# tmdt-buw/VQ-VAE-Transformer-Arc-Welding

Measured on AMD Instinct MI355X. Metric: welding windows/sec (train) VQ-VAE+8-blk Transformer at 1/2/4/8 MI355X, higher is better.
Workload: dtype bf16; 1 GPU; VQ-VAE-Patch reconstruction train step (configs[1]); global_batch=1024, per_gpu_batch=1024, seq_len=200, codebook=512x64, hidden=512, n_resblocks=8, patch=25, parallelism=dp1, optimizer=RAdam(lr 1e-3), operands=bf16 (opt-in), fp32 accumulation and master weights

## Files before the change

### include/arcweld_amd.h

```cpp
#ifndef ARCWELD_AMD_H
#define ARCWELD_AMD_H

#include <stdint.h>

#ifdef __cplusplus
extern "C" {
#endif

enum { AW_OK = 0, AW_ERR_ARG = -1, AW_ERR_LAUNCH = -2 };
enum { AW_F32 = 0, AW_BF16 = 1 };
enum { AW_ACT_GELU_ERF = 0, AW_ACT_GELU_TANH = 1, AW_ACT_DERIV = 2 };

const char* aw_last_error(void);
int aw_version(void);

typedef struct {
  int M, N, K;
  int a_dtype;
  const void* A; int64_t lda; int a_trans;
  const void* B; int64_t ldb; int b_trans;
  int conv_cin, conv_seg, conv_dir, conv_operand;
  float alpha, beta;
  const float* bias;
  int act;
  const float* pre; int64_t ld_pre;
  const float* resid; int64_t ld_resid;
  float drop_p; uint64_t drop_seed;
  void* C; int64_t ldc; int c_dtype;
  void* C2; int64_t ldc2; int c2_mode; int c2_dtype;
  float drop2_p; uint64_t drop2_seed;
  double* colstats; int stats_mod;
  float* a_rowsum;
  int bias_mod;
  int accumulate, col_mod, col_mul, col_off;
  const uint64_t* seed_ptr;
  int pre_dtype;
  int store_policy;
  int resid_dtype;
} aw_gemm_args;
#define AW_STORE_NT 0
#define AW_STORE_WT 1

int aw_gemm(const aw_gemm_args* args, void* stream);
int64_t aw_gemm_workspace(const aw_gemm_args* args);
int aw_gemm_ws(const aw_gemm_args* args, float* ws, int64_t ws_elems, void* stream);
#define AW_GEMM_MAX_GROUPS 16
int aw_gemm_grouped(const aw_gemm_args* args, int n, void* stream);
int aw_gemm_set_tile(int bm);
int aw_gemm_describe(const aw_gemm_args* args, int* layout, uint32_t* epi, int* tile_rows, int* specialised,
                     int* ragged, int* splits);
int aw_gemm_set_wgrad_policy(int mode);
#define AW_WGRAD_BATCH_MAX 32
int64_t aw_wgrad_batch_workspace(const aw_gemm_args* args, int n);
int aw_wgrad_batch(const aw_gemm_args* args, int n, void* ws, int64_t ws_bytes, void* stream);
int aw_wgrad_set_spin_limit(int polls);

#define AW_RES_CHAIN_MAX 16
typedef struct {
  int64_t N;
  int H, R;
  int taps, seg;
  const void* a0;
  const void* x0;
  const void* w1[AW_RES_CHAIN_MAX];
  const void* w2[AW_RES_CHAIN_MAX];
  const float* b1[AW_RES_CHAIN_MAX];
  const float* b2[AW_RES_CHAIN_MAX];
  void* dgelu_h[AW_RES_CHAIN_MAX];
  void* a1[AW_RES_CHAIN_MAX];
  void* dgelu_x[AW_RES_CHAIN_MAX];
  void* a[AW_RES_CHAIN_MAX];
  float drop_p;
  uint64_t drop_seed[AW_RES_CHAIN_MAX];
  const uint64_t* seed_ptr;
  int store_policy;
  uint64_t* drop_masks;
} aw_res_chain_fwd_args;
typedef struct {
  int64_t N;
  int H, R;
  int taps, seg;
  const void* gx;
  const void* gxo;
  const void* x0;
  const void* w1t[AW_RES_CHAIN_MAX];
  const void* w2t[AW_RES_CHAIN_MAX];
  const void* dgelu_h[AW_RES_CHAIN_MAX];
  const void* dgelu_x[AW_RES_CHAIN_MAX];
  void* gh[AW_RES_CHAIN_MAX];
  void* gxo_out[AW_RES_CHAIN_MAX];
  float drop_p;
  int store_policy;
  const uint64_t* drop_masks;
} aw_res_chain_bwd_args;
int aw_res_chain_fwd(const aw_res_chain_fwd_args* args, void* stream);
int aw_res_chain_bwd(const aw_res_chain_bwd_args* args, void* stream);
int64_t aw_res_dropout_masks_bytes(int64_t N, int R);
int aw_res_dropout_masks(int64_t N, int R, float drop_p, const uint64_t* drop_seed, const uint64_t* seed_ptr,
                         void* masks, void* stream);
#define AW_RES_PACK_MAX 32
int aw_res_pack_weights(const void* const* src, void* const* fwd, void* const* bwd, int n, int taps, void* stream);

int aw_vq_forward(const float* z, const float* E, int64_t N, int K, int D,
                  float* zq, int64_t* idx, float* counts, double* sqerr, void* stream);
int aw_vq_forward_ex(const float* z, const float* E, int64_t N, int K, int D, float* zq, int64_t* idx, float* counts,
                     double* sqerr, void* zq_copy, int copy_dtype, void* stream);
#define AW_VQ_COUNT_GROUPS_MAX 64
int aw_vq_forward_ex2(const float* z, const float* E, int64_t N, int K, int D, float* zq, int64_t* idx, float* counts,
                      int count_groups, double* sqerr, void* zq_copy, int copy_dtype, void* stream);
int aw_vq_finalize(const float* counts, const double* sqerr, int64_t N, int K, int D, float beta,
                   float* loss, float* perplexity, void* stream);
int aw_vq_finalize_ex(const float* counts, int count_groups, const double* sqerr, int64_t N, int K, int D, float beta,
                      float* loss, float* perplexity, void* stream);
int aw_vq_backward(const float* z, const float* E, const int64_t* idx, const float* g_zq, const float* g_loss,
                   int64_t N, int K, int D, float beta, float* dz, float* dE, void* stream);
int aw_vq_backward_ex(const float* z, const float* E, const int64_t* idx, const float* g_zq, const float* g_loss,
                      int64_t N, int K, int D, float beta, float* dz, float* dE, void* dz_copy, int copy_dtype,
                      void* stream);
int aw_vq_cluster_sums(const float* z, const int64_t* idx, int64_t N, int K, int D, float* sums, void* stream);
int aw_kmeans_update(float* means, const float* sums, const float* counts, int K, int D, float* avg, void* stream);
int aw_rvq_ema_update(float* embed, float* embed_avg, float* cluster_size, const float* counts, const float* sums,
                      const float* z, int64_t N, int K, int D, float decay, float eps, float threshold, uint64_t salt,
                      const uint64_t* seed_ptr, float* ws, void* stream);
int aw_rvq_residual(const float* r, const float* zq, int64_t n, float* out, int first, float* r_next, void* stream);
int aw_rvq_backward(const float* res, const float* q, const float* g_zq, const float* g_loss, int nq, int64_t N,
                    int D, float commitment, float* dz, void* stream);

int aw_vq_onehot(const int64_t* idx, int64_t N, int K, float* onehot, void* stream);
int aw_vq_gather(const float* E, const int64_t* idx, int64_t N, int D, float* out, void* stream);

int aw_patchify(const float* x, int64_t B, int L, int C, int P, void* patches, int64_t ldp, int dtype,
                void* stream);
int aw_weight_relayout(const float* W, int O, int I, int k, int tap, int mode, void* out, int64_t ldo,
                       int dtype, void* stream);
#define AW_RELAYOUT_MAX_JOBS 40
typedef struct {
  const float* W;
  void* out;
  int O, I, k, tap, mode;
  int64_t ldo;
} aw_relayout_job;
int aw_weight_relayout_batch(const aw_relayout_job* jobs, int n, int dtype, void* stream);
int aw_weight_grad_scatter(const float* g, int O, int I, int k, int tap, int mode, int64_t ldg, float* G,
                           void* stream);
int aw_cast(const float* in, int64_t n, void* out, int dtype, void* stream);

int aw_unpatch_head_fwd(const float* y, int64_t R, int H, int Q, const float* stats, const float* w2,
                        const float* b2, float* x_hat, void* stream);
int aw_bn_finalize(const double* colstats, int64_t n, int H, const float* gamma, const float* beta,
                   float* running_mean, float* running_var, int64_t* nbt, float eps, float momentum,
                   int training, float* stats, void* stream);
int aw_unpatch_head_bwd1(const float* y, int64_t R, int H, int Q, const float* stats, const float* w2,
                         const float* g_xhat, double* gsums, float* gw2, float* gb2, float* ggamma, float* gbeta,
                         void* stream);
int aw_unpatch_head_bwd2(const float* y, int64_t R, int H, int Q, const float* stats, const float* w2,
                         const float* g_xhat, const double* gsums, int training, void* g_y, int gy_dtype, float* db_y,
                         void* stream);
int aw_unpatch_head_fwd_ex(const void* y, int y_dtype, int64_t R, int H, int Q, const float* stats, const float* w2,
                           const float* b2, float* x_hat, void* stream);
int aw_unpatch_head_bwd1_ex(const void* y, int y_dtype, int64_t R, int H, int Q, const float* stats, const float* w2,
                            const float* g_xhat, double* gsums, float* gw2, float* gb2, float* ggamma, float* gbeta,
                            void* stream);
int aw_unpatch_head_bwd2_ex(const void* y, int y_dtype, int64_t R, int H, int Q, const float* stats, const float* w2,
                            const float* g_xhat, const double* gsums, int training, void* g_y, int gy_dtype,
                            float* db_y, void* stream);
int aw_unpatch_head_fwd_bwd1(const void* y, int y_dtype, int64_t R, int H, int Q, const float* stats, const float* w2,
                             const float* b2, const float* x, const float* gscale, float* x_hat, float* g_xhat,
                             double* sqerr, double* gsums, float* gw2, float* gb2, float* ggamma, float* gbeta,
                             void* stream);
int aw_bn_group_stats(const float* h, int64_t N, int H, int G, double* sums, void* stream);
int aw_bn_group_finalize(const double* sums, int64_t n, int H, int G, const float* gamma, const float* beta,
                         float* running_mean, float* running_var, int64_t* nbt, float eps, float momentum,
                         int training, float* stats, void* stream);
int aw_bn_apply(const float* h, int64_t N, int H, int G, const float* stats, int mode, const float* resid,
                float drop_p, uint64_t drop_seed, const uint64_t* seed_ptr, float* out, void* op, int op_dtype,
                void* stream);
int aw_bn_bwd_reduce(const float* h, int64_t N, int H, int G, const float* stats, const float* g_in, float drop_p,
                     uint64_t drop_seed, const uint64_t* seed_ptr, double* sums, void* stream);
int aw_bn_bwd_apply(const float* h, int64_t N, int H, int G, const float* stats, const float* g_in, float drop_p,
                    uint64_t drop_seed, const uint64_t* seed_ptr, const double* sums, int64_t n, int training,
                    void* dh, int dh_dtype, float* dgamma, float* dbeta, void* stream);
int aw_mse_fwd(const float* a, const float* b, int64_t n, double* sqerr, void* stream);
int aw_mse_bwd(const float* a, const float* b, int64_t n, const float* g, float* ga, void* stream);

int aw_scalar_add(const float* a, const float* b, float* out, void* stream);
int aw_mse_finalize(const double* sqerr, int64_t numel, float* out, void* stream);
int aw_mse_finalize_add(const double* sqerr, int64_t numel, const float* addend, float* out, float* sum, void* stream);

int aw_radam_step(float* param, float* grad, float* exp_avg, float* exp_avg_sq, const int64_t* seg_off,
                  const int64_t* seg_len, const float* seg_wd, const int* seg_active, int nseg, int64_t total, int64_t step,
                  float lr, float beta1, float beta2, float eps, const float* gscale, const int64_t* step_ptr,
                  int zero_grad, void* stream);
#define AW_OPS_PER_SEG 2
typedef struct {
  void* out;
  int O, I, k, tap, mode, dtype;
  int64_t ldo;
} aw_operand_desc;
int aw_radam_step_ops(float* param, float* grad, float* exp_avg, float* exp_avg_sq, const int64_t* seg_off,
                      const int64_t* seg_len, const float* seg_wd, const int* seg_active, int nseg, int64_t total,
                      int64_t step, float lr, float beta1, float beta2, float eps, const float* gscale,
                      const int64_t* step_ptr, const aw_operand_desc* ops, int zero_grad, void* stream);
int aw_counter_add(int64_t* counter, int64_t v, void* stream);
int aw_counter_add_snapshot(int64_t* counter, int64_t v, int64_t* snapshot, void* stream);
int aw_counter_add_snapshot_zero(int64_t* counter, int64_t v, int64_t* snapshot, double* zero, int64_t nzero,
                                 void* stream);
#define AW_NORM_WS 1024
int aw_grad_norm_clip(const float* grad, const int64_t* seg_off, const int64_t* seg_len, const int* seg_active,
                      int nseg, int64_t total, float max_norm, double* ws, float* out_norm, float* out_coef,
                      void* stream);
int aw_scale(float* x, int64_t n, const float* s, void* stream);

int aw_layernorm_fwd(const float* x, int64_t R, int D, const float* w, const float* b, float eps, void* y,
                     int y_dtype, float* mean, float* rstd, void* stream);
int aw_layernorm_bwd(const float* x, const float* dy, int64_t R, int D, const float* w, const float* mean,
                     const float* rstd, float* dx, int accumulate, float* dw, float* db, void* dx2, int dx2_dtype,
                     float drop_p, uint64_t drop_seed, const uint64_t* seed_ptr, void* stream);
int aw_class_head_fwd(const float* xf, int64_t B, int T, int D, const float* w1, const float* b1, const float* W2,
                      const float* b2, float* s, float* out, void* stream);
int aw_class_head_bwd(const float* xf, const float* s, const float* dout, int64_t B, int T, int D, const float* w1,
                      const float* W2, float* dxf, float* dw1, float* db1, float* dW2, float* db2, void* stream);
int aw_embed_fwd(const int64_t* ids, int64_t B, int T, int D, const float* wtok, const float* pe, float* x,
                 void* stream);
int aw_embed_ln_fwd(const int64_t* ids, int64_t B, int T, int D, const float* wtok, const float* pe, float* x,
                    const float* w, const float* b, float eps, void* y, int y_dtype, float* mean, float* rstd,
                    void* stream);
int aw_embed_bwd(const int64_t* ids, int64_t B, int T, int D, const float* dx, float* dwtok, void* stream);
int aw_embed_bwd_sorted(const int64_t* ids, int64_t B, int T, int D, int V, const float* dx, float* dwtok, int* work,
                        void* stream);
int aw_embed_sort(const int64_t* ids, int64_t R, int V, int* work, void* stream);
int aw_embed_bwd_segsum(const int* work, int V, int D, const float* dx, float* dwtok, void* stream);
int aw_attn_fwd(const void* qkv, int64_t B, int T, int n_head, int d, int dtype, void* y, float* lse,
                void* stream);
int aw_attn_bwd(const void* qkv, const void* y, const void* dy, const float* lse, int64_t B, int T, int n_head,
                int d, int dtype, void* dqkv, float* ws, void* stream);
int aw_attn_fwd_dropout(const void* qkv, int64_t B, int T, int n_head, int d, int dtype, void* y, float* lse,
                        float drop_p, uint64_t drop_seed, const uint64_t* seed_ptr, void* stream);
int aw_attn_bwd_dropout(const void* qkv, const void* y, const void* dy, const float* lse, int64_t B, int T,
                        int n_head, int d, int dtype, void* dqkv, float* ws, float drop_p, uint64_t drop_seed,
                        const uint64_t* seed_ptr, void* stream);
int aw_attn_decode(const void* qkv_new, int64_t B, int n_new, int pos0, int n_head, int d, int dtype,
                   void* kv_cache, int Tmax, void* y, void* stream);
int aw_ce_fwd(const float* logits, int64_t R, int V, int64_t ldl, const int64_t* y, int ignore_index,
              double* loss_sum, double* count, float* lse, void* stream);
int aw_ce_bwd(const float* logits, int64_t R, int V, int64_t ldl, const int64_t* y, int ignore_index,
              const float* lse, const double* count, const float* g, void* dlogits, int64_t ldd, int dtype,
              void* stream);
int aw_ce_finalize(const double* loss_sum, const double* count, float* out, void* stream);

int aw_gru_pack_weights(const float* w_hh, int H, int op_dtype, void* w_fwd, void* w_bwd, void* stream);
int aw_gru_step_fwd(int B, int H, int op_dtype, const void* h_prev_op, const float* h_prev, const void* w_fwd,
                    const float* gi, const float* b_hh, float* h, void* h_op, float* saved, void* stream);
int aw_gru_step_bwd(int B, int H, int op_dtype, const void* dgh_next_op, const float* dh_next,
                    const float* saved_next, const void* w_bwd, const float* dy, const float* saved,
                    const float* h_prev, float* dh, float* dgi, float* dgh, void* dgi_op, void* dgh_op, void* stream);
int aw_gru_bias_grad(const float* dg, int64_t rows, int H, float* db, void* stream);

#ifdef __cplusplus
}
#endif
#endif
```

### vq-vae-transformer-arc-welding_amd/arcweld/_native.py

```python
from __future__ import annotations

import ctypes
import os

import torch

PKG_DIR = os.path.dirname(os.path.dirname(os.path.abspath(__file__)))
LIB_PATH = os.environ.get("ARCWELD_LIB") or os.path.join(PKG_DIR, "lib", "libarcweld_amd.so")
HEADER = os.path.join(os.path.dirname(PKG_DIR), "include", "arcweld_amd.h")

AW_F32, AW_BF16 = 0, 1
AW_ACT_GELU_ERF, AW_ACT_GELU_TANH, AW_ACT_DERIV = 0, 1, 2
AW_STORE_NT, AW_STORE_WT = 0, 1

c_i64 = ctypes.c_int64
c_int = ctypes.c_int
c_f = ctypes.c_float
c_p = ctypes.c_void_p


class GemmArgs(ctypes.Structure):
    _fields_ = [
        ("M", c_int), ("N", c_int), ("K", c_int),
        ("a_dtype", c_int),
        ("A", c_p), ("lda", c_i64), ("a_trans", c_int),
        ("B", c_p), ("ldb", c_i64), ("b_trans", c_int),
        ("conv_cin", c_int), ("conv_seg", c_int), ("conv_dir", c_int), ("conv_operand", c_int),
        ("alpha", c_f), ("beta", c_f),
        ("bias", c_p),
        ("act", c_int),
        ("pre", c_p), ("ld_pre", c_i64),
        ("resid", c_p), ("ld_resid", c_i64),
        ("drop_p", c_f), ("drop_seed", ctypes.c_uint64),
        ("C", c_p), ("ldc", c_i64), ("c_dtype", c_int),
        ("C2", c_p), ("ldc2", c_i64), ("c2_mode", c_int), ("c2_dtype", c_int),
        ("drop2_p", c_f), ("drop2_seed", ctypes.c_uint64),
        ("colstats", c_p), ("stats_mod", c_int),
        ("a_rowsum", c_p),
        ("bias_mod", c_int),
        ("accumulate", c_int), ("col_mod", c_int), ("col_mul", c_int), ("col_off", c_int),
        ("seed_ptr", c_p),
        ("pre_dtype", c_int),
        ("store_policy", c_int),
        ("resid_dtype", c_int),
    ]


class RelayoutJob(ctypes.Structure):
    _fields_ = [("W", c_p), ("out", c_p), ("O", c_int), ("I", c_int), ("k", c_int), ("tap", c_int),
                ("mode", c_int), ("ldo", c_i64)]


class OperandDesc(ctypes.Structure):
    _fields_ = [("out", c_p), ("O", c_int), ("I", c_int), ("k", c_int), ("tap", c_int), ("mode", c_int),
                ("dtype", c_int), ("ldo", c_i64)]


OPS_PER_SEG = 2

RES_CHAIN_MAX = 16
RES_PACK_MAX = 32
_E = RES_CHAIN_MAX


class ResChainFwdArgs(ctypes.Structure):
    _fields_ = [("N", c_i64), ("H", c_int), ("R", c_int), ("taps", c_int), ("seg", c_int), ("a0", c_p), ("x0", c_p),
                ("w1", c_p * _E), ("w2", c_p * _E), ("b1", c_p * _E), ("b2", c_p * _E),
                ("dgelu_h", c_p * _E), ("a1", c_p * _E), ("dgelu_x", c_p * _E), ("a", c_p * _E),
                ("drop_p", c_f), ("drop_seed", ctypes.c_uint64 * _E), ("seed_ptr", c_p), ("store_policy", c_int),
                ("drop_masks", c_p)]


class ResChainBwdArgs(ctypes.Structure):
    _fields_ = [("N", c_i64), ("H", c_int), ("R", c_int), ("taps", c_int), ("seg", c_int), ("gx", c_p), ("gxo", c_p),
                ("x0", c_p), ("w1t", c_p * _E), ("w2t", c_p * _E), ("dgelu_h", c_p * _E), ("dgelu_x", c_p * _E),
                ("gh", c_p * _E), ("gxo_out", c_p * _E),
                ("drop_p", c_f), ("store_policy", c_int), ("drop_masks", c_p)]

SIGNATURES = {
    "aw_version": [],
    "aw_gemm": [ctypes.POINTER(GemmArgs), c_p],
    "aw_gemm_ws": [ctypes.POINTER(GemmArgs), c_p, c_i64, c_p],
    "aw_gemm_workspace": [ctypes.POINTER(GemmArgs)],
    "aw_gemm_grouped": [ctypes.POINTER(GemmArgs), c_int, c_p],
    "aw_gemm_set_tile": [c_int],
    "aw_gemm_describe": [ctypes.POINTER(GemmArgs), ctypes.POINTER(c_int), ctypes.POINTER(ctypes.c_uint32),
                         ctypes.POINTER(c_int), ctypes.POINTER(c_int), ctypes.POINTER(c_int), ctypes.POINTER(c_int)],
    "aw_gemm_set_wgrad_policy": [c_int],
    "aw_wgrad_batch_workspace": [ctypes.POINTER(GemmArgs), c_int],
    "aw_wgrad_batch": [ctypes.POINTER(GemmArgs), c_int, c_p, c_i64, c_p],
    "aw_wgrad_set_spin_limit": [c_int],
    "aw_res_chain_fwd": [ctypes.POINTER(ResChainFwdArgs), c_p],
    "aw_res_chain_bwd": [ctypes.POINTER(ResChainBwdArgs), c_p],
    "aw_res_pack_weights": [ctypes.POINTER(c_p), ctypes.POINTER(c_p), ctypes.POINTER(c_p), c_int, c_int, c_p],
    "aw_res_dropout_masks_bytes": [c_i64, c_int],
    "aw_res_dropout_masks": [c_i64, c_int, c_f, ctypes.POINTER(ctypes.c_uint64), c_p, c_p, c_p],
    "aw_weight_relayout_batch": [ctypes.POINTER(RelayoutJob), c_int, c_int, c_p],
    "aw_vq_forward": [c_p, c_p, c_i64, c_int, c_int, c_p, c_p, c_p, c_p, c_p],
    "aw_vq_forward_ex": [c_p, c_p, c_i64, c_int, c_int, c_p, c_p, c_p, c_p, c_p, c_int, c_p],
    "aw_vq_finalize": [c_p, c_p, c_i64, c_int, c_int, c_f, c_p, c_p, c_p],
    "aw_vq_forward_ex2": [c_p, c_p, c_i64, c_int, c_int, c_p, c_p, c_p, c_int, c_p, c_p, c_int, c_p],
    "aw_vq_finalize_ex": [c_p, c_int, c_p, c_i64, c_int, c_int, c_f, c_p, c_p, c_p],
    "aw_vq_backward": [c_p, c_p, c_p, c_p, c_p, c_i64, c_int, c_int, c_f, c_p, c_p, c_p],
    "aw_vq_backward_ex": [c_p, c_p, c_p, c_p, c_p, c_i64, c_int, c_int, c_f, c_p, c_p, c_p, c_int, c_p],
    "aw_vq_onehot": [c_p, c_i64, c_int, c_p, c_p],
    "aw_vq_gather": [c_p, c_p, c_i64, c_int, c_p, c_p],
    "aw_patchify": [c_p, c_i64, c_int, c_int, c_int, c_p, c_i64, c_int, c_p],
    "aw_weight_relayout": [c_p, c_int, c_int, c_int, c_int, c_int, c_p, c_i64, c_int, c_p],
    "aw_weight_grad_scatter": [c_p, c_int, c_int, c_int, c_int, c_int, c_i64, c_p, c_p],
    "aw_cast": [c_p, c_i64, c_p, c_int, c_p],
    "aw_unpatch_head_fwd": [c_p, c_i64, c_int, c_int, c_p, c_p, c_p, c_p, c_p],
    "aw_bn_finalize": [c_p, c_i64, c_int, c_p, c_p, c_p, c_p, c_p, c_f, c_f, c_int, c_p, c_p],
    "aw_unpatch_head_bwd1": [c_p, c_i64, c_int, c_int, c_p, c_p, c_p, c_p, c_p, c_p, c_p, c_p, c_p],
    "aw_unpatch_head_bwd2": [c_p, c_i64, c_int, c_int, c_p, c_p, c_p, c_p, c_int, c_p, c_int, c_p, c_p],
    "aw_unpatch_head_fwd_ex": [c_p, c_int, c_i64, c_int, c_int, c_p, c_p, c_p, c_p, c_p],
    "aw_unpatch_head_bwd1_ex": [c_p, c_int, c_i64, c_int, c_int, c_p, c_p, c_p, c_p, c_p, c_p, c_p, c_p, c_p],
    "aw_unpatch_head_fwd_bwd1": [c_p, c_int, c_i64, c_int, c_int, c_p, c_p, c_p, c_p, c_p, c_p, c_p, c_p, c_p, c_p,
                                 c_p, c_p, c_p, c_p],
    "aw_unpatch_head_bwd2_ex": [c_p, c_int, c_i64, c_int, c_int, c_p, c_p, c_p, c_p, c_int, c_p, c_int, c_p, c_p],
    "aw_bn_group_stats": [c_p, c_i64, c_int, c_int, c_p, c_p],
    "aw_bn_group_finalize": [c_p, c_i64, c_int, c_int, c_p, c_p, c_p, c_p, c_p, c_f, c_f, c_int, c_p, c_p],
    "aw_bn_apply": [c_p, c_i64, c_int, c_int, c_p, c_int, c_p, c_f, ctypes.c_uint64, c_p, c_p, c_p, c_int, c_p],
    "aw_bn_bwd_reduce": [c_p, c_i64, c_int, c_int, c_p, c_p, c_f, ctypes.c_uint64, c_p, c_p, c_p],
    "aw_bn_bwd_apply": [c_p, c_i64, c_int, c_int, c_p, c_p, c_f, ctypes.c_uint64, c_p, c_p, c_i64, c_int, c_p, c_int,
                        c_p, c_p, c_p],
    "aw_mse_fwd": [c_p, c_p, c_i64, c_p, c_p],
    "aw_mse_bwd": [c_p, c_p, c_i64, c_p, c_p, c_p],
    "aw_scalar_add": [c_p, c_p, c_p, c_p],
    "aw_mse_finalize": [c_p, c_i64, c_p, c_p],
    "aw_mse_finalize_add": [c_p, c_i64, c_p, c_p, c_p, c_p],
    "aw_radam_step": [c_p, c_p, c_p, c_p, c_p, c_p, c_p, c_p, c_int, c_i64, c_i64, c_f, c_f, c_f, c_f, c_p, c_p,
                      c_int, c_p],
    "aw_radam_step_ops": [c_p, c_p, c_p, c_p, c_p, c_p, c_p, c_p, c_int, c_i64, c_i64, c_f, c_f, c_f, c_f, c_p, c_p,
                          c_p, c_int, c_p],
    "aw_counter_add": [c_p, c_i64, c_p],
    "aw_counter_add_snapshot": [c_p, c_i64, c_p, c_p],
    "aw_counter_add_snapshot_zero": [c_p, c_i64, c_p, c_p, c_i64, c_p],
    "aw_grad_norm_clip": [c_p, c_p, c_p, c_p, c_int, c_i64, c_f, c_p, c_p, c_p, c_p],
    "aw_scale": [c_p, c_i64, c_p, c_p],
    "aw_layernorm_fwd": [c_p, c_i64, c_int, c_p, c_p, c_f, c_p, c_int, c_p, c_p, c_p],
    "aw_layernorm_bwd": [c_p, c_p, c_i64, c_int, c_p, c_p, c_p, c_p, c_int, c_p, c_p, c_p, c_int, c_f,
                         ctypes.c_uint64, c_p, c_p],
    "aw_class_head_fwd": [c_p, c_i64, c_int, c_int, c_p, c_p, c_p, c_p, c_p, c_p, c_p],
    "aw_class_head_bwd": [c_p, c_p, c_p, c_i64, c_int, c_int, c_p, c_p, c_p, c_p, c_p, c_p, c_p, c_p],
    "aw_embed_fwd": [c_p, c_i64, c_int, c_int, c_p, c_p, c_p, c_p],
    "aw_embed_ln_fwd": [c_p, c_i64, c_int, c_int, c_p, c_p, c_p, c_p, c_p, c_f, c_p, c_int, c_p, c_p, c_p],
    "aw_embed_bwd": [c_p, c_i64, c_int, c_int, c_p, c_p, c_p],
    "aw_embed_bwd_sorted": [c_p, c_i64, c_int, c_int, c_int, c_p, c_p, c_p, c_p],
    "aw_embed_sort": [c_p, c_i64, c_int, c_p, c_p],
    "aw_embed_bwd_segsum": [c_p, c_int, c_int, c_p, c_p, c_p],
    "aw_attn_fwd": [c_p, c_i64, c_int, c_int, c_int, c_int, c_p, c_p, c_p],
    "aw_attn_bwd": [c_p, c_p, c_p, c_p, c_i64, c_int, c_int, c_int, c_int, c_p, c_p, c_p],
    "aw_attn_fwd_dropout": [c_p, c_i64, c_int, c_int, c_int, c_int, c_p, c_p, c_f, ctypes.c_uint64, c_p, c_p],
    "aw_attn_bwd_dropout": [c_p, c_p, c_p, c_p, c_i64, c_int, c_int, c_int, c_int, c_p, c_p, c_f, ctypes.c_uint64,
                            c_p, c_p],
    "aw_attn_decode": [c_p, c_i64, c_int, c_int, c_int, c_int, c_int, c_p, c_int, c_p, c_p],
    "aw_ce_fwd": [c_p, c_i64, c_int, c_i64, c_p, c_int, c_p, c_p, c_p, c_p],
    "aw_ce_bwd": [c_p, c_i64, c_int, c_i64, c_p, c_int, c_p, c_p, c_p, c_p, c_i64, c_int, c_p],
    "aw_ce_finalize": [c_p, c_p, c_p, c_p],
    "aw_vq_cluster_sums": [c_p, c_p, c_i64, c_int, c_int, c_p, c_p],
    "aw_kmeans_update": [c_p, c_p, c_p, c_int, c_int, c_p, c_p],
    "aw_rvq_ema_update": [c_p, c_p, c_p, c_p, c_p, c_p, c_i64, c_int, c_int, c_f, c_f, c_f, ctypes.c_uint64, c_p, c_p,
                          c_p],
    "aw_rvq_residual": [c_p, c_p, c_i64, c_p, c_int, c_p, c_p],
    "aw_rvq_backward": [c_p, c_p, c_p, c_p, c_int, c_i64, c_int, c_f, c_p, c_p],
    "aw_gru_pack_weights": [c_p, c_int, c_int, c_p, c_p, c_p],
    "aw_gru_step_fwd": [c_int, c_int, c_int, c_p, c_p, c_p, c_p, c_p, c_p, c_p, c_p, c_p],
    "aw_gru_bias_grad": [c_p, c_i64, c_int, c_p, c_p],
    "aw_gru_step_bwd": [c_int, c_int, c_int, c_p, c_p, c_p, c_p, c_p, c_p, c_p, c_p, c_p, c_p, c_p, c_p, c_p],
}

RET_I64 = {"aw_gemm_workspace", "aw_wgrad_batch_workspace", "aw_res_dropout_masks_bytes"}

_lib = None


class NativeError(RuntimeError):
    pass


def load(path: str = LIB_PATH):
    global _lib
    if _lib is not None:
        return _lib
    if not os.path.exists(path):
        raise NativeError(f"HIP library not built: {path} is missing (run `python -c 'import __graft_entry__ as g; "
                          f"g.build()'` or `make -C vq-vae-transformer-arc-welding_amd/csrc`)")
    lib = ctypes.CDLL(path, mode=ctypes.RTLD_GLOBAL)
    lib.aw_last_error.restype = ctypes.c_char_p
    lib.aw_last_error.argtypes = []
    for name, argtypes in SIGNATURES.items():
        fn = getattr(lib, name)
        fn.restype = c_i64 if name in RET_I64 else c_int
        fn.argtypes = argtypes
    _lib = lib
    return lib


def call(name: str, *args) -> None:
    lib = load()
    status = getattr(lib, name)(*args)
    if status != 0:
        raise NativeError(f"{name} failed ({status}): {lib.aw_last_error().decode(errors='replace')}")


def stream_ptr(stream=None) -> int:
    s = stream if stream is not None else torch.cuda.current_stream()
    return s.cuda_stream


def ptr(t):
    if t is None:
        return None
    if not t.is_cuda:
        raise NativeError("arcweld HIP kernels need device tensors (got a CPU tensor); there is no CPU fallback")
    return t.data_ptr()


def dtype_code(dt: torch.dtype) -> int:
    if dt == torch.float32:
        return AW_F32
    if dt == torch.bfloat16:
        return AW_BF16
    raise NativeError(f"unsupported operand dtype {dt}")
```

### vq-vae-transformer-arc-welding_amd/arcweld/kernels.py

```python
from __future__ import annotations

import contextvars
import ctypes

import torch

from . import _native as nat
from ._native import AW_ACT_DERIV, AW_ACT_GELU_ERF, AW_ACT_GELU_TANH, AW_BF16, AW_F32, GemmArgs, call, dtype_code, ptr, stream_ptr

__all__ = ["gemm", "AW_ACT_DERIV", "AW_ACT_GELU_ERF", "AW_ACT_GELU_TANH", "AW_BF16", "AW_F32"]


def _ld(t):
    if t is None:
        return 0
    if t.dim() == 1:
        return t.shape[0]
    if t.stride(-1) != 1:
        raise nat.NativeError("operand rows must be contiguous (stride(-1) == 1)")
    return t.stride(0)


_STORE_POLICY = contextvars.ContextVar("arcweld_store_policy", default=0)


class store_policy:

    def __init__(self, policy):
        self.policy = int(policy)

    def __enter__(self):
        self._tok = _STORE_POLICY.set(self.policy)

    def __exit__(self, *exc):
        _STORE_POLICY.reset(self._tok)
        return False

    def __call__(self, fn):
        import functools

        @functools.wraps(fn)
        def wrapped(*a, **k):
            with store_policy(self.policy):
                return fn(*a, **k)
        return wrapped


PROFILE = None


def _algorithmic_flops(M, N, Kd, conv, flops):
    if flops is not None:
        return float(flops)
    if conv is not None:
        seg = conv[1]
        return 2.0 * M * N * (Kd / 3.0) * (3.0 - 2.0 / seg)
    return 2.0 * M * N * Kd


def _gemm_args(A, B, M, N, K, *, a_trans=False, b_trans=False, conv=None, alpha=1.0, beta=0.0, bias=None,
               act=AW_ACT_GELU_ERF, pre=None, resid=None, drop=(0.0, 0), C=None, C2=None, c2_mode=0, drop2=(0.0, 0),
               colstats=None, stats_mod=0, a_rowsum=None, bias_mod=0, accumulate=False, col_map=(0, 1, 0),
               seed_ptr=None):
    if A.dtype != B.dtype:
        raise nat.NativeError(f"gemm operands must share a dtype ({A.dtype} vs {B.dtype})")
    a = GemmArgs()
    a.M, a.N, a.K = int(M), int(N), int(K)
    a.a_dtype = dtype_code(A.dtype)
    a.A, a.lda, a.a_trans = ptr(A), _ld(A), int(bool(a_trans))
    a.B, a.ldb, a.b_trans = ptr(B), _ld(B), int(bool(b_trans))
    if conv is not None:
        a.conv_cin, a.conv_seg, a.conv_dir, a.conv_operand = (int(v) for v in conv)
    a.alpha, a.beta = float(alpha), float(beta)
    a.bias = ptr(bias)
    a.act = int(act)
    a.store_policy = _STORE_POLICY.get()
    a.pre, a.ld_pre = ptr(pre), _ld(pre)
    if pre is not None:
        if pre.dtype not in (torch.float32, torch.bfloat16):
            raise nat.NativeError("pre must be float32 or bfloat16")
        a.pre_dtype = dtype_code(pre.dtype)
    a.resid, a.ld_resid = ptr(resid), _ld(resid)
    if resid is not None:
        if resid.dtype not in (torch.float32, torch.bfloat16):
            raise nat.NativeError("resid must be float32 or bfloat16")
        a.resid_dtype = dtype_code(resid.dtype)
    a.drop_p, a.drop_seed = float(drop[0]), int(drop[1]) & 0xFFFFFFFFFFFFFFFF
    if C is not None:
        a.C, a.ldc, a.c_dtype = ptr(C), _ld(C), dtype_code(C.dtype)
    if C2 is not None:
        a.C2, a.ldc2, a.c2_dtype = ptr(C2), _ld(C2), dtype_code(C2.dtype)
    a.c2_mode = int(c2_mode)
    a.drop2_p, a.drop2_seed = float(drop2[0]), int(drop2[1]) & 0xFFFFFFFFFFFFFFFF
    if colstats is not None:
        if colstats.dtype != torch.float64:
            raise nat.NativeError("colstats must be float64")
        a.colstats, a.stats_mod = ptr(colstats), int(stats_mod)
    a.a_rowsum = ptr(a_rowsum)
    a.bias_mod = int(bias_mod)
    a.accumulate = int(bool(accumulate))
    a.col_mod, a.col_mul, a.col_off = (int(v) for v in col_map)
    a.seed_ptr = ptr(seed_ptr)
    return a


def _timed(s, fn, flops, tag, name=None, nbytes=None):
    e0, e1 = torch.cuda.Event(enable_timing=True), torch.cuda.Event(enable_timing=True)
    e0.record(s)
    fn(s.cuda_stream)
    e1.record(s)
    PROFILE.append((e0, e1, flops, tag, name or tag, nbytes))


def _gemm_tag(A):
    return "gemm_bf16" if A.dtype == torch.bfloat16 else "gemm_f32"


def gemm(A, B, M, N, K, *, stream=None, flops=None, **kw):
    a = _gemm_args(A, B, M, N, K, **kw)
    lib = nat.load()
    wsn = lib.aw_gemm_workspace(ctypes.byref(a))
    ws = torch.empty(wsn, device=A.device, dtype=torch.float32) if wsn > 0 else None
    if PROFILE is None:
        call("aw_gemm_ws", ctypes.byref(a), ptr(ws), wsn, stream_ptr(stream))
        return kw.get("C")
    s = stream if stream is not None else torch.cuda.current_stream()
    _timed(s, lambda sp: call("aw_gemm_ws", ctypes.byref(a), ptr(ws), wsn, sp),
           _algorithmic_flops(M, N, K, kw.get("conv"), flops), _gemm_tag(A), "gemm_kernel")
    return kw.get("C")


MAX_GROUPS = 16


def gemm_grouped(problems, stream=None):
    for c0 in range(0, len(problems), MAX_GROUPS):
        chunk = problems[c0:c0 + MAX_GROUPS]
        arr = (GemmArgs * len(chunk))(*[_gemm_args(A, B, M, N, K, **kw) for (A, B, M, N, K, kw) in chunk])
        if PROFILE is None:
            call("aw_gemm_grouped", arr, len(chunk), stream_ptr(stream))
            continue
        s = stream if stream is not None else torch.cuda.current_stream()
        fl = sum(_algorithmic_flops(M, N, K, kw.get("conv"), None) for (_, _, M, N, K, kw) in chunk)
        c0_ = chunk[0]
        nm = "wgrad_conv3_kernel" if (c0_[5].get("conv") is not None and c0_[0].dtype == torch.bfloat16) \
            else "gemm_kernel (grouped)"
        _timed(s, lambda sp: call("aw_gemm_grouped", arr, len(chunk), sp), fl, _gemm_tag(chunk[0][0]), nm)


WGRAD_BATCH_MAX = 32


def wgrad_batch_ok(problems):
    import os
    mode = os.environ.get("ARCWELD_WGRAD_BATCH", "auto")
    if mode == "0" or not problems or len(problems) > WGRAD_BATCH_MAX:
        return False
    arr = (GemmArgs * len(problems))(*[_gemm_args(A, B, M, N, K, **kw) for (A, B, M, N, K, kw) in problems])
    if nat.load().aw_wgrad_batch_workspace(arr, len(problems)) <= 0:
        return False
    tiles = sum((M // 256) * (N // 256) for (_, _, M, N, _, _) in problems)
    return mode == "1" or tiles >= 128


def wgrad_batch(problems, stream=None):
    arr = (GemmArgs * len(problems))(*[_gemm_args(A, B, M, N, K, **kw) for (A, B, M, N, K, kw) in problems])
    lib = nat.load()
    wsb = lib.aw_wgrad_batch_workspace(arr, len(problems))
    if wsb < 0:
        raise nat.NativeError(f"aw_wgrad_batch: batch not eligible ({lib.aw_last_error().decode(errors='replace')})")
    ws = torch.empty((wsb + 3) // 4, device=problems[0][0].device, dtype=torch.float32)
    if PROFILE is None:
        call("aw_wgrad_batch", arr, len(problems), ptr(ws), wsb, stream_ptr(stream))
        return
    s = stream if stream is not None else torch.cuda.current_stream()
    fl = sum(_algorithmic_flops(M, N, K, None, None) for (_, _, M, N, K, _) in problems)
    _timed(s, lambda sp: call("aw_wgrad_batch", arr, len(problems), ptr(ws), wsb, sp), fl, _gemm_tag(problems[0][0]),
           "wgrad_tt_kernel")


def wgrad_issue(problems, stream=None):
    if not problems:
        return
    nch = (len(problems) + WGRAD_BATCH_MAX - 1) // WGRAD_BATCH_MAX
    per = (len(problems) + nch - 1) // nch
    chunks = [problems[i:i + per] for i in range(0, len(problems), per)]
    if all(wgrad_batch_ok(c) for c in chunks):
        for c in chunks:
            wgrad_batch(c, stream)
        return
    by_shape = {}
    for pb in problems:
        by_shape.setdefault((pb[2], pb[3]), []).append(pb)
    for grp in by_shape.values():
        gemm_grouped(grp, stream)


RES_CHAIN_MAX = nat.RES_CHAIN_MAX


def res_chain_ok(H, R, T, RT, taps=1, seg=16, which="ENC"):
    import os
    if os.environ.get(f"ARCWELD_{which}_CHAIN", "1") == "0":
        return False
    return (H == 512 and 1 <= R <= RES_CHAIN_MAX and T == torch.bfloat16 and RT == torch.bfloat16
            and (taps == 1 or (taps == 3 and seg == 16)))


def _chain_store_policy():
    import os
    return nat.AW_STORE_WT if os.environ.get("ARCWELD_CHAIN_STORE", "nt") == "wt" else nat.AW_STORE_NT


def _chk_rows(ts, N, H, who):
    for t in ts:
        if t is None:
            continue
        if t.dtype != torch.bfloat16 or t.dim() != 2 or tuple(t.shape) != (N, H) or not t.is_contiguous():
            raise nat.NativeError(f"{who}: activations must be contiguous ({N}, {H}) bfloat16 tensors")


def res_dropout_masks_empty(N, R, device):
    nb = nat.load().aw_res_dropout_masks_bytes(int(N), int(R))
    if nb <= 0:
        raise nat.NativeError("res_dropout_masks: bad N / R")
    return torch.empty(nb, device=device, dtype=torch.uint8)


def res_dropout_masks(N, drop, seed_ptr=None, stream=None):
    p, seeds = float(drop[0]), list(drop[1] or [])
    if p <= 0.0:
        return None
    R = len(seeds)
    out = res_dropout_masks_empty(N, R, torch.cuda.current_device() if seed_ptr is None else seed_ptr.device)
    sd = (ctypes.c_uint64 * R)(*[int(v) & 0xFFFFFFFFFFFFFFFF for v in seeds])
    call("aw_res_dropout_masks", int(N), R, p, sd, ptr(seed_ptr), ptr(out), stream_ptr(stream))
    return out


def _nbytes(ts):
    seen, n = set(), 0
    for t in ts:
        if t is not None and t.data_ptr() not in seen:
            seen.add(t.data_ptr())
            n += t.numel() * t.element_size()
    return n


def _chain_flops(R, N, H, taps, seg):
    if taps == 1:
        return 4.0 * R * N * H * H
    return 4.0 * R * N * H * H * (3 - 2.0 / seg)


def res_chain_fwd(a0, x0, w1, w2, b1, b2, dh, a1, dx, a, drop=(0.0, None), seed_ptr=None, masks=None, taps=1, seg=16,
                  stream=None):
    N, H = a0.shape
    R = len(w1)
    if not (1 <= R <= RES_CHAIN_MAX) or not all(len(v) == R for v in (w2, b1, b2, dh, a1, dx, a)):
        raise nat.NativeError("res_chain_fwd: need R (1..16) entries in every per-block list")
    _chk_rows([a0, x0] + list(dh) + list(a1) + list(dx) + list(a), N, H, "res_chain_fwd")
    g = nat.ResChainFwdArgs()
    g.N, g.H, g.R, g.taps, g.seg = N, H, R, int(taps), int(seg)
    g.a0, g.x0 = ptr(a0), ptr(x0)
    for r in range(R):
        g.w1[r], g.w2[r], g.b1[r], g.b2[r] = ptr(w1[r]), ptr(w2[r]), ptr(b1[r]), ptr(b2[r])
        g.dgelu_h[r], g.a1[r], g.dgelu_x[r], g.a[r] = ptr(dh[r]), ptr(a1[r]), ptr(dx[r]), ptr(a[r])
        g.drop_seed[r] = int(drop[1][r]) & 0xFFFFFFFFFFFFFFFF if drop[0] > 0 else 0
    g.drop_p = float(drop[0])
    g.seed_ptr = ptr(seed_ptr)
    g.store_policy = _chain_store_policy()
    g.drop_masks = ptr(masks)
    _maybe_timed(stream, "gemm_bf16", _chain_flops(R, N, H, taps, seg),
                 lambda sp: call("aw_res_chain_fwd", ctypes.byref(g), sp),
                 lambda: (f"res_chain_fwd_kernel<{int(taps)}>",
                          _nbytes([a0, x0, masks] + list(w1) + list(w2) + list(b1) + list(b2) + list(dh) + list(a1) +
                                  list(dx)[:-1] + list(a))))


def res_chain_bwd(gx, gxo, w1t, w2t, dh, x0, dx, gh, gxo_out, drop_p=0.0, masks=None, taps=1, seg=16, stream=None):
    N, H = gx.shape
    R = len(w1t)
    if not (1 <= R <= RES_CHAIN_MAX) or not all(len(v) == R for v in (w2t, dh, dx, gh, gxo_out)):
        raise nat.NativeError("res_chain_bwd: need R (1..16) entries in every per-block list")
    _chk_rows([gx, gxo, x0] + list(dh) + list(dx[1:]) + list(gh) + list(gxo_out), N, H, "res_chain_bwd")
    g = nat.ResChainBwdArgs()
    g.N, g.H, g.R, g.taps, g.seg = N, H, R, int(taps), int(seg)
    g.gx, g.gxo, g.x0 = ptr(gx), ptr(gxo), ptr(x0)
    for r in range(R):
        g.w1t[r], g.w2t[r], g.dgelu_h[r] = ptr(w1t[r]), ptr(w2t[r]), ptr(dh[r])
        g.dgelu_x[r] = ptr(dx[r]) if r > 0 else None
        g.gh[r], g.gxo_out[r] = ptr(gh[r]), ptr(gxo_out[r])
    g.drop_p = float(drop_p)
    g.store_policy = _chain_store_policy()
    g.drop_masks = ptr(masks)
    _maybe_timed(stream, "gemm_bf16", _chain_flops(R, N, H, taps, seg),
                 lambda sp: call("aw_res_chain_bwd", ctypes.byref(g), sp),
                 lambda: (f"res_chain_bwd_kernel<{int(taps)}>",
                          _nbytes([gx, gxo, x0, masks] + list(w1t) + list(w2t) + list(dh) + list(dx[1:]) + list(gh) +
                                  list(gxo_out))))


def res_pack_weights(src, fwd=None, bwd=None, taps=1, stream=None):
    n = len(src)
    fwd = fwd if fwd is not None else [None] * n
    bwd = bwd if bwd is not None else [None] * n
    if len(fwd) != n or len(bwd) != n:
        raise nat.NativeError("res_pack_weights: list lengths differ")
    for t in list(src) + [t for t in fwd + bwd if t is not None]:
        if t.dtype != torch.bfloat16 or t.numel() != 512 * 512 * taps or not t.is_contiguous():
            raise nat.NativeError(f"res_pack_weights: need contiguous 512 x {512 * taps} bfloat16 tensors")
    for c0 in range(0, n, nat.RES_PACK_MAX):
        sl = slice(c0, c0 + nat.RES_PACK_MAX)
        m = len(src[sl])
        arr = lambda ts: (ctypes.c_void_p * m)(*[ptr(t) for t in ts])
        call("aw_res_pack_weights", arr(src[sl]), arr(fwd[sl]), arr(bwd[sl]), m, int(taps), stream_ptr(stream))


def vq_forward(z2d, E, zq, idx, counts, sqerr, stream=None, zq_copy=None, count_groups=1):
    N, D = z2d.shape
    Kc = E.shape[0]
    assert counts.numel() >= count_groups * Kc, "counts: count_groups x K floats"
    _maybe_timed(stream, "vq_fwd", 2.0 * N * Kc * D, lambda sp: call(
        "aw_vq_forward_ex2", ptr(z2d), ptr(E), N, Kc, D, ptr(zq), ptr(idx), ptr(counts), int(count_groups),
        ptr(sqerr), ptr(zq_copy), dtype_code(zq_copy.dtype) if zq_copy is not None else 0, sp),
        lambda: ("vq_fwd_pinned_kernel" if Kc <= 512 and D in (16, 32, 64) else "vq_fwd_kernel",
                 _nbytes([z2d, E, zq, idx, zq_copy]) + 4 * Kc * count_groups))


def vq_finalize(counts, sqerr, N, K, D, beta, loss, perplexity, stream=None, count_groups=1):
    call("aw_vq_finalize_ex", ptr(counts), int(count_groups), ptr(sqerr), N, K, D, float(beta), ptr(loss),
         ptr(perplexity), stream_ptr(stream))


def vq_backward(z2d, E, idx, g_zq, g_loss, beta, dz, dE, stream=None, dz_copy=None):
    N, D = z2d.shape
    if dz_copy is None:
        call("aw_vq_backward", ptr(z2d), ptr(E), ptr(idx), ptr(g_zq), ptr(g_loss), N, E.shape[0], D, float(beta),
             ptr(dz), ptr(dE), stream_ptr(stream))
    else:
        call("aw_vq_backward_ex", ptr(z2d), ptr(E), ptr(idx), ptr(g_zq), ptr(g_loss), N, E.shape[0], D, float(beta),
             ptr(dz), ptr(dE), ptr(dz_copy), dtype_code(dz_copy.dtype), stream_ptr(stream))


def vq_cluster_sums(z2d, idx, K, sums, stream=None):
    _dense(z2d, "vq_cluster_sums")
    call("aw_vq_cluster_sums", ptr(z2d), ptr(idx), z2d.shape[0], K, z2d.shape[1], ptr(sums), stream_ptr(stream))


def kmeans_update(means, sums, counts, avg=None, stream=None):
    call("aw_kmeans_update", ptr(means), ptr(sums), ptr(counts), means.shape[0], means.shape[1], ptr(avg),
         stream_ptr(stream))


def rvq_ema_update(embed, embed_avg, cluster_size, counts, sums, z2d, decay, eps, threshold, salt, seed_ptr, ws,
                   stream=None):
    K, D = embed.shape
    call("aw_rvq_ema_update", ptr(embed), ptr(embed_avg), ptr(cluster_size), ptr(counts), ptr(sums), ptr(z2d),
         z2d.shape[0], K, D, float(decay), float(eps), float(threshold), int(salt) & 0xFFFFFFFFFFFFFFFF,
         ptr(seed_ptr), ptr(ws), stream_ptr(stream))


def rvq_residual(r, zq, out, first, r_next=None, stream=None):
    call("aw_rvq_residual", ptr(r), ptr(zq), zq.numel(), ptr(out), int(bool(first)), ptr(r_next), stream_ptr(stream))


def rvq_backward(res, q, g_zq, g_loss, dz, commitment=1.0, stream=None):
    nq, N, D = res.shape
    call("aw_rvq_backward", ptr(res), ptr(q), ptr(g_zq), ptr(g_loss), nq, N, D, float(commitment), ptr(dz),
         stream_ptr(stream))


def vq_onehot(idx, K, out, stream=None):
    call("aw_vq_onehot", ptr(idx), idx.numel(), K, ptr(out), stream_ptr(stream))


def vq_gather(E, idx, out, stream=None):
    call("aw_vq_gather", ptr(E), ptr(idx), idx.numel(), E.shape[1], ptr(out), stream_ptr(stream))


def patchify(x, P, out, stream=None):
    B, L, C = x.shape
    call("aw_patchify", ptr(x), B, L, C, P, ptr(out), out.stride(0), dtype_code(out.dtype), stream_ptr(stream))


def weight_relayout(W, O, I, k, tap, mode, out, ldo=0, stream=None):
    _dense(W, "weight_relayout")
    call("aw_weight_relayout", ptr(W), O, I, k, tap, mode, ptr(out), ldo, dtype_code(out.dtype), stream_ptr(stream))


RELAYOUT_MAX_JOBS = 40


def _dense(W, who):
    if not W.is_contiguous():
        raise nat.NativeError(f"{who}: the source weight must be contiguous (got strides {tuple(W.stride())})")


def weight_relayout_batch(jobs, stream=None):
    by_dtype = {}
    for jb in jobs:
        by_dtype.setdefault(jb[6].dtype, []).append(jb)
    for dt, js in by_dtype.items():
        for c0 in range(0, len(js), RELAYOUT_MAX_JOBS):
            chunk = js[c0:c0 + RELAYOUT_MAX_JOBS]
            arr = (nat.RelayoutJob * len(chunk))()
            for r, jb in zip(arr, chunk):
                W, O, I, k, tap, mode, out = jb[:7]
                _dense(W, "weight_relayout_batch")
                r.W, r.out = ptr(W), ptr(out)
                r.O, r.I, r.k, r.tap, r.mode = int(O), int(I), int(k), int(tap), int(mode)
                r.ldo = int(jb[7]) if len(jb) > 7 else 0
            call("aw_weight_relayout_batch", arr, len(chunk), dtype_code(dt), stream_ptr(stream))


def weight_grad_scatter(g, O, I, k, tap, mode, G, stream=None):
    call("aw_weight_grad_scatter", ptr(g), O, I, k, tap, mode, g.stride(0), ptr(G), stream_ptr(stream))


def cast(x, out, stream=None):
    call("aw_cast", ptr(x), x.numel(), ptr(out), dtype_code(out.dtype), stream_ptr(stream))


def bn_finalize(colstats, n, H, gamma, beta, rm, rv, nbt, eps, momentum, training, stats, stream=None):
    call("aw_bn_finalize", ptr(colstats), n, H, ptr(gamma), ptr(beta), ptr(rm), ptr(rv), ptr(nbt), float(eps),
         float(momentum), int(training), ptr(stats), stream_ptr(stream))


def unpatch_head_fwd(y, Q, stats, w2, b2, x_hat, stream=None):
    R, H = y.shape
    call("aw_unpatch_head_fwd_ex", ptr(y), dtype_code(y.dtype), R, H, Q, ptr(stats), ptr(w2), ptr(b2), ptr(x_hat),
         stream_ptr(stream))


def unpatch_head_bwd1(y, Q, stats, w2, g_xhat, gsums, gw2, gb2, ggamma, gbeta, stream=None):
    R, H = y.shape
    call("aw_unpatch_head_bwd1_ex", ptr(y), dtype_code(y.dtype), R, H, Q, ptr(stats), ptr(w2), ptr(g_xhat), ptr(gsums),
         ptr(gw2), ptr(gb2), ptr(ggamma), ptr(gbeta), stream_ptr(stream))


def unpatch_head_bwd2(y, Q, stats, w2, g_xhat, gsums, training, g_y, db_y, stream=None):
    R, H = y.shape
    call("aw_unpatch_head_bwd2_ex", ptr(y), dtype_code(y.dtype), R, H, Q, ptr(stats), ptr(w2), ptr(g_xhat),
         ptr(gsums), int(training), ptr(g_y), dtype_code(g_y.dtype), ptr(db_y), stream_ptr(stream))


def unpatch_head_fwd_bwd1(y, Q, stats, w2, b2, x, gscale, x_hat, g_xhat, sqerr, gsums, gw2, gb2, ggamma, gbeta,
                          stream=None):
    R, H = y.shape
    for nm, t in (("x", x), ("x_hat", x_hat), ("g_xhat", g_xhat)):
        if t.dtype != torch.float32 or not t.is_contiguous() or t.numel() != R * 5:
            raise nat.NativeError(f"unpatch_head_fwd_bwd1: {nm} must be a contiguous float32 tensor of R*5 = {R * 5} "
                                  f"elements (got {tuple(t.shape)} {t.dtype}, contiguous={t.is_contiguous()})")
    call("aw_unpatch_head_fwd_bwd1", ptr(y), dtype_code(y.dtype), R, H, Q, ptr(stats), ptr(w2), ptr(b2), ptr(x),
         ptr(gscale), ptr(x_hat), ptr(g_xhat), ptr(sqerr), ptr(gsums), ptr(gw2), ptr(gb2), ptr(ggamma), ptr(gbeta),
         stream_ptr(stream))


def head_bf16_ok(H):
    return 64 <= H <= 2048 and H & (H - 1) == 0


def mse_fwd(a, b, sqerr, stream=None):
    call("aw_mse_fwd", ptr(a), ptr(b), a.numel(), ptr(sqerr), stream_ptr(stream))


def mse_bwd(a, b, g, ga, stream=None):
    call("aw_mse_bwd", ptr(a), ptr(b), a.numel(), ptr(g), ptr(ga), stream_ptr(stream))


def scalar_add(a, b, out, stream=None):
    call("aw_scalar_add", ptr(a), ptr(b), ptr(out), stream_ptr(stream))


def mse_finalize(sqerr, numel, out, stream=None):
    call("aw_mse_finalize", ptr(sqerr), int(numel), ptr(out), stream_ptr(stream))


def mse_finalize_add(sqerr, numel, addend, out, total, stream=None):
    call("aw_mse_finalize_add", ptr(sqerr), int(numel), ptr(addend), ptr(out), ptr(total), stream_ptr(stream))


def radam_step(param, grad, m, v, seg_off, seg_len, seg_wd, seg_active, nseg, total, step, lr, beta1, beta2, eps,
               gscale=None, stream=None, step_ptr=None, ops=None, zero_grad=False):
    args = (ptr(param), ptr(grad), ptr(m), ptr(v), ptr(seg_off), ptr(seg_len), ptr(seg_wd), ptr(seg_active), int(nseg),
            int(total), int(step), float(lr), float(beta1), float(beta2), float(eps), ptr(gscale), ptr(step_ptr))
    if ops is None:
        call("aw_radam_step", *args, int(bool(zero_grad)), stream_ptr(stream))
    else:
        call("aw_radam_step_ops", *args, ptr(ops), int(bool(zero_grad)), stream_ptr(stream))


def counter_add_snapshot(counter, snapshot, v=1, stream=None, zero=None):
    if zero is None:
        call("aw_counter_add_snapshot", ptr(counter), int(v), ptr(snapshot), stream_ptr(stream))
        return
    if zero.dtype != torch.float64 or not zero.is_contiguous():
        raise nat.NativeError("counter_add_snapshot: zero must be a contiguous float64 tensor")
    call("aw_counter_add_snapshot_zero", ptr(counter), int(v), ptr(snapshot), ptr(zero), zero.numel(),
         stream_ptr(stream))


def counter_add(counter, v=1, stream=None):
    call("aw_counter_add", ptr(counter), int(v), stream_ptr(stream))


NORM_WS = 1024


def grad_norm_clip(grad, seg_off, seg_len, seg_active, nseg, max_norm, ws, out_norm, out_coef, stream=None):
    if ws.numel() < NORM_WS or ws.dtype != torch.float64:
        raise nat.NativeError(f"grad_norm_clip: ws must hold {NORM_WS} float64")
    call("aw_grad_norm_clip", ptr(grad), ptr(seg_off), ptr(seg_len), ptr(seg_active), int(nseg), grad.numel(),
         float(max_norm), ptr(ws), ptr(out_norm), ptr(out_coef), stream_ptr(stream))


def scale_(x, s, stream=None):
    call("aw_scale", ptr(x), x.numel(), ptr(s), stream_ptr(stream))


def layernorm_fwd(x, w, b, eps, y, mean, rstd, stream=None):
    R, D = x.shape
    call("aw_layernorm_fwd", ptr(x), R, D, ptr(w), ptr(b), float(eps), ptr(y), dtype_code(y.dtype), ptr(mean),
         ptr(rstd), stream_ptr(stream))


def layernorm_bwd(x, dy, w, mean, rstd, dx, accumulate, dw, db, dx2=None, drop=(0.0, 0), stream=None,
                  seed_ptr=None):
    R, D = x.shape
    call("aw_layernorm_bwd", ptr(x), ptr(dy), R, D, ptr(w), ptr(mean), ptr(rstd), ptr(dx), int(accumulate), ptr(dw),
         ptr(db), ptr(dx2), dtype_code(dx2.dtype) if dx2 is not None else AW_F32, float(drop[0]),
         int(drop[1]) & 0xFFFFFFFFFFFFFFFF, ptr(seed_ptr), stream_ptr(stream))


def class_head_fwd(xf, B, T, w1, b1, W2, b2, s, out, stream=None):
    call("aw_class_head_fwd", ptr(xf), B, T, xf.shape[-1], ptr(w1), ptr(b1), ptr(W2), ptr(b2), ptr(s), ptr(out),
         stream_ptr(stream))


def class_head_bwd(xf, s, dout, B, T, w1, W2, dxf, dw1, db1, dW2, db2, stream=None):
    call("aw_class_head_bwd", ptr(xf), ptr(s), ptr(dout), B, T, xf.shape[-1], ptr(w1), ptr(W2), ptr(dxf), ptr(dw1),
         ptr(db1), ptr(dW2), ptr(db2), stream_ptr(stream))


def embed_fwd(ids, wtok, pe, x, stream=None):
    B, T = ids.shape
    call("aw_embed_fwd", ptr(ids), B, T, wtok.shape[1], ptr(wtok), ptr(pe), ptr(x), stream_ptr(stream))


def embed_ln_fwd(ids, wtok, pe, x, w, b, eps, y, mean, rstd, stream=None):
    B, T = ids.shape
    call("aw_embed_ln_fwd", ptr(ids), B, T, wtok.shape[1], ptr(wtok), ptr(pe), ptr(x), ptr(w), ptr(b), float(eps),
         ptr(y), dtype_code(y.dtype), ptr(mean), ptr(rstd), stream_ptr(stream))


def embed_bwd(ids, dx, dwtok, stream=None, sort=True):
    B, T = ids.shape
    if not sort:
        call("aw_embed_bwd", ptr(ids), B, T, dwtok.shape[1], ptr(dx), ptr(dwtok), stream_ptr(stream))
        return
    V = dwtok.shape[0]
    work = torch.empty(V + 1 + B * T, device=dx.device, dtype=torch.int32)
    call("aw_embed_bwd_sorted", ptr(ids), B, T, dwtok.shape[1], V, ptr(dx), ptr(dwtok), ptr(work),
         stream_ptr(stream))


EMBED_SORT_MAX_V = 15360


def embed_sort(ids, V, work, stream=None):
    call("aw_embed_sort", ptr(ids), ids.numel(), V, ptr(work), stream_ptr(stream))


def embed_bwd_segsum(work, dx, dwtok, stream=None):
    call("aw_embed_bwd_segsum", ptr(work), dwtok.shape[0], dwtok.shape[1], ptr(dx), ptr(dwtok), stream_ptr(stream))


def attn_flops(B, T, n_head, d):
    return 4.0 * B * n_head * (T * (T + 1) / 2) * (d // n_head)


def _maybe_timed(stream, tag, flops, fn, info=None):
    if PROFILE is None:
        fn(stream_ptr(stream))
        return
    s = stream if stream is not None else torch.cuda.current_stream()
    _timed(s, fn, flops, tag, *(info() if info is not None else ()))


def attn_fwd(qkv, B, T, n_head, d, y, lse, drop=(0.0, 0), seed_ptr=None, stream=None):
    if drop[0] > 0:
        _maybe_timed(stream, "attn_fwd", attn_flops(B, T, n_head, d), lambda sp: call(
            "aw_attn_fwd_dropout", ptr(qkv), B, T, n_head, d, dtype_code(qkv.dtype), ptr(y), ptr(lse),
            float(drop[0]), int(drop[1]) & 0xFFFFFFFFFFFFFFFF, ptr(seed_ptr), sp))
        return
    _maybe_timed(stream, "attn_fwd", attn_flops(B, T, n_head, d), lambda sp: call(
        "aw_attn_fwd", ptr(qkv), B, T, n_head, d, dtype_code(qkv.dtype), ptr(y), ptr(lse), sp))


def attn_bwd(qkv, y, dy, lse, B, T, n_head, d, dqkv, ws, drop=(0.0, 0), seed_ptr=None, stream=None):
    fl = 2.0 * attn_flops(B, T, n_head, d)
    if drop[0] > 0:
        _maybe_timed(stream, "attn_bwd", fl, lambda sp: call(
            "aw_attn_bwd_dropout", ptr(qkv), ptr(y), ptr(dy), ptr(lse), B, T, n_head, d, dtype_code(qkv.dtype),
            ptr(dqkv), ptr(ws), float(drop[0]), int(drop[1]) & 0xFFFFFFFFFFFFFFFF, ptr(seed_ptr), sp))
        return
    _maybe_timed(stream, "attn_bwd", fl, lambda sp: call(
        "aw_attn_bwd", ptr(qkv), ptr(y), ptr(dy), ptr(lse), B, T, n_head, d, dtype_code(qkv.dtype), ptr(dqkv),
        ptr(ws), sp))


def bn_group_stats(h, G, sums, stream=None):
    N, H = h.shape
    call("aw_bn_group_stats", ptr(h), N, H, int(G), ptr(sums), stream_ptr(stream))


def bn_group_finalize(sums, n, H, G, bn, training, stats, stream=None):
    mom = bn.momentum if bn.momentum is not None else 0.1
    call("aw_bn_group_finalize", ptr(sums) if training else None, int(n), int(H), int(G), ptr(bn.weight),
         ptr(bn.bias), ptr(bn.running_mean), ptr(bn.running_var), ptr(bn.num_batches_tracked) if training else None,
         float(bn.eps), float(mom), int(bool(training)), ptr(stats), stream_ptr(stream))


def bn_apply(h, G, stats, mode, out, op=None, resid=None, drop=(0.0, 0), seed_ptr=None, stream=None):
    N, H = h.shape
    call("aw_bn_apply", ptr(h), N, H, int(G), ptr(stats), int(mode), ptr(resid), float(drop[0]), int(drop[1]),
         ptr(seed_ptr), ptr(out), ptr(op), dtype_code(op.dtype) if op is not None else AW_F32, stream_ptr(stream))


def bn_bwd_reduce(h, G, stats, g_in, sums, drop=(0.0, 0), seed_ptr=None, stream=None):
    N, H = h.shape
    call("aw_bn_bwd_reduce", ptr(h), N, H, int(G), ptr(stats), ptr(g_in), float(drop[0]), int(drop[1]),
         ptr(seed_ptr), ptr(sums), stream_ptr(stream))


def bn_bwd_apply(h, G, stats, g_in, sums, n, training, dh, dgamma=None, dbeta=None, drop=(0.0, 0), seed_ptr=None,
                 stream=None):
    N, H = h.shape
    call("aw_bn_bwd_apply", ptr(h), N, H, int(G), ptr(stats), ptr(g_in), float(drop[0]), int(drop[1]),
         ptr(seed_ptr), ptr(sums), int(n), int(bool(training)), ptr(dh), dtype_code(dh.dtype), ptr(dgamma),
         ptr(dbeta), stream_ptr(stream))


def attn_decode(qkv_new, B, n_new, pos0, n_head, d, kv_cache, y, stream=None):
    if kv_cache.dtype != qkv_new.dtype or y.dtype != qkv_new.dtype or kv_cache.shape[-1] != 2 * d:
        raise nat.NativeError("attn_decode: qkv, cache and y share a dtype; cache rows are [K | V] (2d)")
    call("aw_attn_decode", ptr(qkv_new), B, n_new, pos0, n_head, d, dtype_code(qkv_new.dtype), ptr(kv_cache),
         kv_cache.shape[1], ptr(y), stream_ptr(stream))


def ce_fwd(logits, V, y, ignore_index, loss_sum, count, lse, stream=None):
    R = y.numel()
    call("aw_ce_fwd", ptr(logits), R, V, logits.stride(0), ptr(y), int(ignore_index), ptr(loss_sum), ptr(count),
         ptr(lse), stream_ptr(stream))


def ce_bwd(logits, V, y, ignore_index, lse, count, g, dlogits, stream=None):
    R = y.numel()
    call("aw_ce_bwd", ptr(logits), R, V, logits.stride(0), ptr(y), int(ignore_index), ptr(lse), ptr(count), ptr(g),
         ptr(dlogits), dlogits.stride(0), dtype_code(dlogits.dtype), stream_ptr(stream))


def ce_finalize(loss_sum, count, out, stream=None):
    call("aw_ce_finalize", ptr(loss_sum), ptr(count), ptr(out), stream_ptr(stream))


def gru_padded(H):
    return (int(H) + 31) // 32 * 32


def _chk_gru(name, t, shape, dtype):
    if t is None:
        return
    if t.dtype != dtype or tuple(t.shape) != tuple(shape) or not t.is_contiguous():
        raise nat.NativeError(f"gru: {name} must be a contiguous {dtype} tensor of shape {tuple(shape)}, got "
                              f"{t.dtype} {tuple(t.shape)}")


def gru_pack_weights(w_hh, H, w_fwd=None, w_bwd=None, stream=None):
    Hp = gru_padded(H)
    T = (w_fwd if w_fwd is not None else w_bwd).dtype
    _chk_gru("w_hh", w_hh, (3 * H, H), torch.float32)
    _chk_gru("w_fwd", w_fwd, (3, Hp, Hp), T)
    _chk_gru("w_bwd", w_bwd, (Hp, 3 * Hp), T)
    call("aw_gru_pack_weights", ptr(w_hh), int(H), dtype_code(T), ptr(w_fwd), ptr(w_bwd), stream_ptr(stream))


def gru_step_fwd(H, T, gi, b_hh, h, saved, w_fwd=None, h_prev_op=None, h_prev=None, h_op=None, stream=None):
    B, Hp = gi.shape[0], gru_padded(H)
    _chk_gru("gi", gi, (B, 3 * Hp), torch.float32)
    _chk_gru("b_hh", b_hh, (3 * H,), torch.float32)
    _chk_gru("h", h, (B, Hp), torch.float32)
    _chk_gru("saved", saved, (B, 4 * Hp), torch.float32)
    _chk_gru("h_prev_op", h_prev_op, (B, Hp), T)
    _chk_gru("h_prev", h_prev, (B, Hp), torch.float32)
    _chk_gru("h_op", h_op, (B, Hp), torch.bfloat16)
    _chk_gru("w_fwd", w_fwd, (3, Hp, Hp), T)
    call("aw_gru_step_fwd", B, int(H), dtype_code(T), ptr(h_prev_op), ptr(h_prev), ptr(w_fwd), ptr(gi), ptr(b_hh),
         ptr(h), ptr(h_op), ptr(saved), stream_ptr(stream))


def gru_step_bwd(H, T, saved, dh, dgi, dgh, w_bwd=None, dgh_next_op=None, dh_next=None, saved_next=None, dy=None,
                 h_prev=None, dgi_op=None, dgh_op=None, stream=None):
    B, Hp = saved.shape[0], gru_padded(H)
    f32 = torch.float32
    _chk_gru("saved", saved, (B, 4 * Hp), f32)
    _chk_gru("saved_next", saved_next, (B, 4 * Hp), f32)
    for name, t in (("dh", dh), ("dh_next", dh_next), ("dy", dy), ("h_prev", h_prev)):
        _chk_gru(name, t, (B, Hp), f32)
    for name, t in (("dgi", dgi), ("dgh", dgh)):
        _chk_gru(name, t, (B, 3 * Hp), f32)
    for name, t in (("dgi_op", dgi_op), ("dgh_op", dgh_op)):
        _chk_gru(name, t, (B, 3 * Hp), torch.bfloat16)
    _chk_gru("dgh_next_op", dgh_next_op, (B, 3 * Hp), T)
    _chk_gru("w_bwd", w_bwd, (Hp, 3 * Hp), T)
    call("aw_gru_step_bwd", B, int(H), dtype_code(T), ptr(dgh_next_op), ptr(dh_next), ptr(saved_next), ptr(w_bwd),
         ptr(dy), ptr(saved), ptr(h_prev), ptr(dh), ptr(dgi), ptr(dgh), ptr(dgi_op), ptr(dgh_op), stream_ptr(stream))


def gru_bias_grad(dg, H, db, stream=None):
    rows = dg.shape[0]
    _chk_gru("dg", dg, (rows, 3 * gru_padded(H)), torch.float32)
    _chk_gru("db", db, (3 * H,), torch.float32)
    call("aw_gru_bias_grad", ptr(dg), rows, int(H), ptr(db), stream_ptr(stream))
```

### vq-vae-transformer-arc-welding_amd/arcweld/resstack.py

```python
from __future__ import annotations

import torch

from . import kernels as K

F32 = torch.float32


def _centre_job(w, out):
    O, I = w.shape[0], w.shape[1]
    c = w[:, :, 1]
    if w.is_contiguous():
        return (w, O, I, 3, 1, 0, out)
    if not c.is_contiguous():
        raise ValueError("encoder conv weight: unsupported layout")
    return (c, O, I, 1, 0, 0, out)


def _centre_grad(g):
    O, I = g.shape[0], g.shape[1]
    if g.is_contiguous():
        return g.view(O, 3 * I), (0, 3, 1)
    c = g[:, :, 1]
    if not c.is_contiguous():
        raise ValueError("encoder conv gradient: unsupported layout")
    return c, (0, 1, 0)


def _conv3_job(w, mode, out):
    from .operands import OperandJob
    return OperandJob("", w, w.shape[0], w.shape[1], 3, 0, mode, out).relayout_job()


def _conv3_grad(g):
    O, I = g.shape[0], g.shape[1]
    if g.is_contiguous():
        return g.view(O, 3 * I), (I, 3, 0)
    st = g.permute(0, 2, 1)
    if not st.is_contiguous():
        raise ValueError("decoder conv gradient: unsupported layout")
    return st.reshape(O, 3 * I), (0, 1, 0)


class Geometry:

    def __init__(self, taps, H, S):
        self.taps, self.H, self.S, self.Kd = taps, H, S, taps * H
        conv = lambda d, operand: dict(conv=(H, S, d, operand)) if taps == 3 else {}
        self.fwd, self.dgrad, self.wgrad = conv(1, 0), conv(-1, 0), conv(1, 1)
        self.G = S if taps == 1 else 1
        self.grad_target = _centre_grad if taps == 1 else _conv3_grad

    def fwd_job(self, w, out):
        return _centre_job(w, out) if self.taps == 1 else _conv3_job(w, 1, out)

    def dgrad_job(self, w, out):
        return _conv3_job(w, 2, out)

    def wgrad_problem(self, A, B, gw, gb):
        Cw, cm = self.grad_target(gw)
        return (A, B, self.H, self.Kd, A.shape[0], dict(a_trans=True, b_trans=True, C=Cw, accumulate=True, col_map=cm,
                                                        a_rowsum=gb, **self.wgrad))


class Saved:

    def __init__(self, geo, route, T, p_drop, seeds, ctr, training, x0, a0):
        self.geo = geo
        self.route, self.T, self.p_drop, self.seeds, self.ctr, self.training = route, T, p_drop, seeds, ctr, training
        self.xs, self.a0s, self.hs, self.a1s, self.bs, self.ws = [x0], [a0], [], [], [], []
        self.masks = self.pk_bwd = None


def _bn_stats(h, G, bn, training):
    N, H = h.shape
    sums = None
    if training and N // G <= 1:
        raise ValueError(f"Expected more than 1 value per channel when training, got input size "
                         f"torch.Size([{N // G}, {H}])")
    if training:
        sums = torch.zeros(2, G, H, device=h.device, dtype=torch.float64)
        K.bn_group_stats(h, G, sums)
    st = torch.empty(4, G, H, device=h.device)
    K.bn_group_finalize(sums, N // G, H, G, bn, training, st)
    return st


def _bn_block_fwd(geo, a0, x, w1, w2, b1, b2, bns, training, p_drop, seed, ctr, T, last):
    N, H = x.shape
    G = geo.G
    bn1, bn2 = bns
    e = lambda *s, dt=F32: torch.empty(*s, device=x.device, dtype=dt)
    h1 = e(N, H)
    K.gemm(a0, w1, N, H, geo.Kd, bias=b1, C=h1, **geo.fwd)
    st1 = _bn_stats(h1, G, bn1, training)
    hn1, a1 = e(N, H), e(N, H, dt=T)
    K.bn_apply(h1, G, st1, 0, hn1, op=a1)
    h2 = e(N, H)
    K.gemm(a1, w2, N, H, geo.Kd, bias=b2, C=h2, **geo.fwd)
    st2 = _bn_stats(h2, G, bn2, training)
    y, an = e(N, H), e(N, H, dt=T)
    K.bn_apply(h2, G, st2, 2 if last else 1, y, op=an, resid=x, drop=(p_drop, seed), seed_ptr=ctr)
    return y, an, dict(h1=h1, hn1=hn1, a1=a1, h2=h2, st1=st1, st2=st2)


def _bn_block_bwd(sv, r, gy, w1d, w2d, grads, bns, slot, wgrads, need_copy):
    N, H = gy.shape
    geo = sv.geo
    G, T, training = geo.G, sv.T, sv.training
    bs, drop = sv.bs[r], dict(drop=(sv.p_drop, sv.seeds[r]), seed_ptr=sv.ctr)
    bn1, bn2 = bns
    dev = gy.device
    e = lambda *s, dt=F32: torch.empty(*s, device=dev, dtype=dt)
    n = N // G
    sums2 = torch.zeros(2, G, H, device=dev, dtype=torch.float64)
    K.bn_bwd_reduce(bs["h2"], G, bs["st2"], gy, sums2, **drop)
    dh2 = e(N, H, dt=T)
    K.bn_bwd_apply(bs["h2"], G, bs["st2"], gy, sums2, n, training, dh2, slot(bn2.weight), slot(bn2.bias), **drop)
    t1 = e(N, H)
    K.gemm(dh2, w2d, N, H, geo.Kd, b_trans=True, pre=bs["hn1"], C=t1, **geo.dgrad)
    wgrads.append(geo.wgrad_problem(dh2, bs["a1"], *grads(r, 1)))
    sums1 = torch.zeros(2, G, H, device=dev, dtype=torch.float64)
    K.bn_bwd_reduce(bs["h1"], G, bs["st1"], t1, sums1)
    dh1 = e(N, H, dt=T)
    K.bn_bwd_apply(bs["h1"], G, bs["st1"], t1, sums1, n, training, dh1, slot(bn1.weight), slot(bn1.bias))
    gx = e(N, H)
    gxo = e(N, H, dt=T) if need_copy else None
    K.gemm(dh1, w1d, N, H, geo.Kd, b_trans=True, pre=sv.xs[r], resid=gy, C=gx, C2=gxo, c2_mode=2 if need_copy else 0,
           **geo.dgrad)
    wgrads.append(geo.wgrad_problem(dh1, sv.a0s[r], *grads(r, 0)))
    return gx, gxo


def _chain_fwd(sv, weights, biases, RT, save):
    geo = sv.geo
    R, H, taps, T = len(biases), geo.H, geo.taps, sv.T
    x0, a0 = sv.xs[0], sv.a0s[0]
    N, dev = a0.shape[0], a0.device
    e = lambda dt: torch.empty(N, H, device=dev, dtype=dt)
    sv.hs = [e(T) if save else None for _ in range(R)]
    sv.a1s = [e(T) if save else None for _ in range(R)]
    sv.xs += [e(RT) if save and r < R - 1 else None for r in range(R)]
    sv.a0s += [e(T) for _ in range(R)]
    wsrc = [w for r in range(R) for w in weights[r]]
    pk = [torch.empty(H, geo.Kd, device=dev, dtype=T) for _ in wsrc]
    K.res_pack_weights(wsrc, pk, None, taps=taps)
    if save:
        sv.pk_bwd = wsrc
        if sv.p_drop > 0 and R > 1:
            sv.masks = K.res_dropout_masks_empty(N, R, dev)
    K.res_chain_fwd(a0, x0, pk[0::2], pk[1::2], [b1 for b1, _ in biases], [b2 for _, b2 in biases], sv.hs, sv.a1s,
                    sv.xs[1:], sv.a0s[1:], drop=(sv.p_drop, sv.seeds), seed_ptr=sv.ctr, masks=sv.masks, taps=taps,
                    seg=geo.S)


def _chain_bwd(sv, gx, gxo, grads):
    N, H = gx.shape
    geo = sv.geo
    R, taps, dev, T = len(sv.hs), geo.taps, gx.device, gxo.dtype
    gh = [torch.empty(N, H, device=dev, dtype=T) for _ in range(R)]
    go = [torch.empty(N, H, device=dev, dtype=T) for _ in range(R)]
    pk_bwd = [torch.empty(H, geo.Kd, device=dev, dtype=T) for _ in sv.pk_bwd]
    K.res_pack_weights(sv.pk_bwd, None, pk_bwd, taps=taps)
    K.res_chain_bwd(gx, gxo, pk_bwd[0::2], pk_bwd[1::2], sv.hs, sv.xs[0], [None] + list(sv.xs[1:R]), gh, go,
                    drop_p=sv.p_drop, masks=sv.masks, taps=taps, seg=geo.S)
    sv.pk_bwd = sv.masks = None
    wgrads = []
    for r in reversed(range(R)):
        gin = gxo if r == R - 1 else go[r + 1]
        wgrads.append(geo.wgrad_problem(gin, sv.a1s[r], *grads(r, 1)))
        wgrads.append(geo.wgrad_problem(gh[r], sv.a0s[r], *grads(r, 0)))
    return go[0], wgrads


def forward(geo, x0, a0, weights, biases, bns=None, *, T, RT, p_drop=0.0, seeds=None, ctr=None, training=False,
            chain=False, last_operand_only=True, in_place=False, save=True):
    R, H, Kd = len(biases), geo.H, geo.Kd
    N, dev = a0.shape[0], a0.device
    seeds = [0] * R if seeds is None else seeds
    route = "bn" if bns is not None else "chain" if chain else "conv"
    sv = Saved(geo, route, T, p_drop, seeds, ctr, training, x0, a0)
    e = lambda dt: torch.empty(N, H, device=dev, dtype=dt)
    if route == "chain":
        _chain_fwd(sv, weights, biases, RT, save)
        return sv.xs[R], sv.a0s[R], sv
    x, a, h, a1 = x0, a0, None, None
    for r in range(R):
        (w1, w2), (b1, b2) = weights[r], biases[r]
        last = last_operand_only and r == R - 1
        if route == "bn":
            xn, an, bs = _bn_block_fwd(geo, a, x, w1, w2, b1, b2, bns[r], training, p_drop, seeds[r], ctr, T, last)
        else:
            if h is None or not in_place:
                h, a1 = e(T), e(T)
            K.gemm(a, w1, N, H, Kd, bias=b1, C=h, C2=a1, c2_mode=1, **geo.fwd)
            xn = None if last else x if in_place else e(RT)
            an = a if in_place else e(T)
            out = dict(C=an) if last else dict(C=xn, C2=an, c2_mode=1)
            K.gemm(a1, w2, N, H, Kd, bias=b2, drop=(p_drop, seeds[r]), seed_ptr=ctr, resid=x, **out, **geo.fwd)
            bs = None
        if save:
            sv.xs.append(xn)
            sv.a0s.append(an)
            sv.hs.append(h)
            sv.a1s.append(a1)
            sv.bs.append(bs)
            sv.ws.append((w1, w2))
        x, a = xn, an
    return x, a, sv


def backward(sv, gy, go, dweights, grads, bns=None, slot=None, r0_copy=True):
    if sv.route == "chain":
        gxo, wgrads = _chain_bwd(sv, gy, go, grads)
        return gxo, gxo, wgrads
    N, H = gy.shape
    geo, RT, T, p = sv.geo, gy.dtype, sv.T, sv.p_drop
    e = lambda dt: torch.empty(N, H, device=gy.device, dtype=dt)
    wgrads = []
    for r in reversed(range(len(sv.hs))):
        W1d, W2d = dweights[r]
        if sv.route == "bn":
            gy, go = _bn_block_bwd(sv, r, gy, W1d, W2d, grads, bns[r], slot, wgrads, r0_copy and r == 0)
            continue
        gh = e(T)
        K.gemm(go, W2d, N, H, geo.Kd, b_trans=True, pre=sv.hs[r], C=gh, **geo.dgrad)
        wgrads.append(geo.wgrad_problem(go, sv.a1s[r], *grads(r, 1)))
        gyn = e(RT)
        gon = e(T) if r > 0 or r0_copy else None
        K.gemm(gh, W1d, N, H, geo.Kd, b_trans=True, pre=sv.xs[r], resid=gy, C=gyn, C2=gon,
               c2_mode=3 if r > 0 else 2 if r0_copy else 0, drop2=(p, sv.seeds[r - 1] if r > 0 else 0),
               seed_ptr=sv.ctr, **geo.dgrad)
        wgrads.append(geo.wgrad_problem(gh, sv.a0s[r], *grads(r, 0)))
        gy, go = gyn, gon
    return gy, go, wgrads
```

### vq-vae-transformer-arc-welding_amd/arcweld/vqvae.py

```python
from __future__ import annotations

import os
import weakref

import torch

from . import _native as nat
from . import kernels as K
from . import operands
from . import resstack
from .precision import operand_dtype

F32 = torch.float32


def _mix(seed: int, salt: int) -> int:
    z = (seed * 0x9E3779B97F4A7C15 + salt * 0xBF58476D1CE4E5B9 + 0x94D049BB133111EB) & 0xFFFFFFFFFFFFFFFF
    z ^= z >> 31
    z = (z * 0xD6E8FEB86659FD93) & 0xFFFFFFFFFFFFFFFF
    return z ^ (z >> 32)


def rng_snapshot(m, dev, p_drop, zero=None):
    if p_drop <= 0.0:
        if zero is not None:
            zero.zero_()
        return None
    ctr = getattr(m, "_rng_counter", None)
    if ctr is None or ctr.device != dev:
        ctr = torch.zeros(1, dtype=torch.int64, device=dev)
        m._rng_counter = ctr
    snap = torch.empty(1, dtype=torch.int64, device=dev)
    K.counter_add_snapshot(ctr, snap, zero=zero)
    return snap


VQ_COUNT_GROUPS = 8


def accumulators(m, dev, K, H, zero=True):
    key = (dev, K, H)
    st = m.__dict__.get("_acc_block")
    if st is None or st[0] != key:
        st = (key, torch.empty(2 + 4 * H + (VQ_COUNT_GROUPS * K + 1) // 2, dtype=torch.float64, device=dev))
        m.__dict__["_acc_block"] = st
    buf = st[1]
    if zero:
        buf.zero_()
    return dict(block=buf, vq_sq=buf[0:1], mse_sq=buf[1:2], colstats=buf[2:2 + 2 * H], head_gsums=buf[2 + 2 * H:2 + 4 * H],
                counts=buf[2 + 4 * H:].view(torch.float32)[:VQ_COUNT_GROUPS * K])


def resid_dtype(m, T):
    if T == F32 or m.batch_norm or os.environ.get("ARCWELD_RESID_F32", "0") == "1":
        return F32
    return T


class VQVAEShapes:
    def __init__(self, m, B):
        self.B = B
        self.H, self.D, self.K = m.hidden_dim, m.embedding_dim, m.num_embeddings
        self.R = m.n_resblocks
        self.P, self.L, self.C = m.patch_size, m.seq_len, m.input_dim
        self.S = self.L * self.C // self.P
        self.N = B * self.S
        self.k1 = m.reverse_patch_embed.k1
        self.Q = self.S * self.k1
        self.ldp = (self.P + 7) // 8 * 8


def _params(m):
    enc = [(blk.block[1], blk.block[4]) for blk in m.encoder[0].shared_conv]
    dec = [(blk.block[1], blk.block[4]) for blk in m.decoder[1].shared_conv]
    enc_bn = [(blk.block[2], blk.block[5]) for blk in m.encoder[0].shared_conv] if m.batch_norm else None
    dec_bn = [(blk.block[2], blk.block[5]) for blk in m.decoder[1].shared_conv] if m.batch_norm else None
    rp = m.reverse_patch_embed.proj
    E = None if getattr(m, "use_improved_vq", False) else m.vector_quantization.embedding.weight
    return dict(pe=m.patch_embed.proj, enc=enc, sep=m.encoder[1].shared_conv, E=E,
                dec0=m.decoder[0], dec=dec, t1=rp[0], bn=rp[1], t2=rp[3], enc_bn=enc_bn, dec_bn=dec_bn)


class Saved:
    pass


def _operand_jobs(m, T):
    from .operands import OperandJob as J
    sh = VQVAEShapes(m, 1)
    H, D, R, P, k1 = sh.H, sh.D, sh.R, sh.P, sh.k1
    pr = _params(m)
    dev = pr["pe"].weight.device
    e = lambda *s: torch.empty(*s, device=dev, dtype=T)
    jobs = [J("Wp", pr["pe"].weight, H, 1, P, 0, 4, torch.zeros(H, sh.ldp, device=dev, dtype=T),
              sh.ldp)]
    centre = lambda w: resstack._centre_job(w, None)[:6]
    for r, (c1, c2) in enumerate(pr["enc"]):
        for nm, c in (("1", c1), ("2", c2)):
            jobs.append(J(f"enc{r}_{nm}", c.weight, H, H, 1, 0, 0, e(H, H), derive=centre))
    jobs.append(J("Ws", pr["sep"].weight, D, H, 1, 0, 0, e(D, H)))
    jobs.append(J("Wd0", pr["dec0"].weight, H, D, 1, 0, 0, e(H, D)))
    for r, (c1, c2) in enumerate(pr["dec"]):
        for nm, c in (("1", c1), ("2", c2)):
            jobs.append(J(f"dec{r}_{nm}", c.weight, H, H, 3, 0, 1, e(H, 3 * H)))
            jobs.append(J(f"dgw{r}_{nm}", c.weight, H, H, 3, 0, 2, e(3 * H, H)))
    jobs.append(J("Wt1", pr["t1"].weight, H, H, k1, 0, 3, e(k1 * H, H)))
    return jobs


def operand_set(m, T=None):
    T = operand_dtype(T)
    return operands.peek(m, ("vqvae", T), lambda: _operand_jobs(m, T))


@K.store_policy(nat.AW_STORE_WT)
def forward(m, x, training: bool, need_backward: bool, dtype=None, seed: int = 0, head=True):
    T = operand_dtype(dtype)
    if x.dtype != F32 or x.dim() != 3:
        raise ValueError("VQVAEPatch expects float32 windows of shape (B, seq_len, input_dim)")
    x = x.contiguous()
    sh = VQVAEShapes(m, x.shape[0])
    H, D, N, S, R, P, k1 = sh.H, sh.D, sh.N, sh.S, sh.R, sh.P, sh.k1
    if x.shape[1] != sh.L or x.shape[2] != sh.C:
        raise ValueError(f"expected windows (B, {sh.L}, {sh.C}), got {tuple(x.shape)}")
    pr = _params(m)
    dev = x.device
    p_drop = float(m.dropout_p) if training else 0.0
    e = lambda *s, dt=F32: torch.empty(*s, device=dev, dtype=dt)
    sv = Saved()
    sv.sh, sv.T, sv.p_drop, sv.training = sh, T, p_drop, training
    RT = sv.RT = resid_dtype(m, T)
    acc = accumulators(m, dev, sh.K, H, zero=False)
    sv.ctr = rng_snapshot(m, dev, p_drop, zero=acc["block"])
    sv.acc = acc
    owner = m.__dict__.get("_acc_owner")
    owned = owner is not None and owner() is not None
    sv.head_gsums = acc["head_gsums"] if not owned else torch.zeros(2 * H, device=dev, dtype=torch.float64)
    if need_backward and not owned:
        m.__dict__["_acc_owner"] = weakref.ref(sv)

    ops = operands.get(m, ("vqvae", T), lambda: _operand_jobs(m, T))
    Wp, Ws, Wd0, Wt1 = ops["Wp"], ops["Ws"], ops["Wd0"], ops["Wt1"]
    enc_w = [(ops[f"enc{r}_1"], ops[f"enc{r}_2"]) for r in range(R)]
    dec_w = [(ops[f"dec{r}_1"], ops[f"dec{r}_2"]) for r in range(R)]
    sv.ops = ops

    patches = e(N, sh.ldp, dt=T)
    K.patchify(x, P, patches)
    x0, a0 = e(N, H, dt=RT), e(N, H, dt=T)
    K.gemm(patches, Wp, N, H, sh.ldp, bias=pr["pe"].bias, C=x0, C2=a0, c2_mode=1, flops=2 * N * H * P)

    stack = dict(T=T, RT=RT, p_drop=p_drop, ctr=sv.ctr, training=training, save=need_backward)
    _, xR_T, sv.enc = resstack.forward(resstack.Geometry(1, H, S), x0, a0, enc_w, _biases(pr["enc"]), pr["enc_bn"],
                                       seeds=[_mix(seed, 100 + r) for r in range(R)],
                                       chain=K.res_chain_ok(H, R, T, RT), **stack)
    if R == 0:
        xR_T = _operand(x0, T)

    z = e(N, D)
    K.gemm(xR_T, Ws, N, D, H, bias=pr["sep"].bias, C=z)

    Kc = sh.K
    if pr["E"] is None:
        rvq = m.vector_quantization.vq
        zq, idx2, losses, sv.rvq = rvq.quantize_rows(z, training, save=need_backward)
        idx = idx2[:, 0] if rvq.num_quantizers == 1 else idx2
        emb_loss = losses.view(()) if rvq.num_quantizers == 1 else losses.sum()
        perplexity = None
    else:
        zq = e(N, D)
        idx = e(N, dt=torch.int64)
        counts, sq = acc["counts"], acc["vq_sq"]
        zq_T = None if T == F32 else e(N, D, dt=T)
        K.vq_forward(z, pr["E"], zq, idx, counts, sq, zq_copy=zq_T, count_groups=VQ_COUNT_GROUPS)
        emb_loss, perplexity = e(()), e(())
        K.vq_finalize(counts, sq, N, Kc, D, m.vector_quantization.beta, emb_loss, perplexity,
                      count_groups=VQ_COUNT_GROUPS)
    if pr["E"] is None or T == F32:
        zq_T = zq if T == F32 else _cast(zq, T)

    y0, ya0 = e(N, H, dt=RT), e(N, H, dt=T)
    K.gemm(zq_T, Wd0, N, H, D, bias=pr["dec0"].bias, C=y0, C2=ya0, c2_mode=1)
    _, yR_T, sv.dec = resstack.forward(resstack.Geometry(3, H, S), y0, ya0, dec_w, _biases(pr["dec"]), pr["dec_bn"],
                                       seeds=[_mix(seed, 200 + r) for r in range(R)],
                                       chain=K.res_chain_ok(H, R, T, RT, 3, S, "DEC"), **stack)
    if R == 0:
        yR_T = _operand(y0, T)

    bn = pr["bn"]
    bf_y = T != F32 and K.head_bf16_ok(H) and os.environ.get("ARCWELD_HEAD_BF16", "1") == "1"
    Y = e(N, k1 * H, dt=T if bf_y else F32)
    colstats = acc["colstats"] if training else None
    K.gemm(yR_T, Wt1, N, k1 * H, H, bias=pr["t1"].bias, bias_mod=H, C=Y, colstats=colstats, stats_mod=H)
    stats = e(4 * H)
    K.bn_finalize(colstats, N * k1, H, bn.weight, bn.bias, bn.running_mean, bn.running_var,
                  bn.num_batches_tracked if training else None, bn.eps,
                  bn.momentum if bn.momentum is not None else 0.1, training, stats)
    x_hat = e(sh.B, sh.L, sh.C)
    Y2 = Y.view(N * k1, H)
    sv.head_fused = not head and need_backward and fused_head_ok(H)
    if not sv.head_fused:
        K.unpatch_head_fwd(Y2, sh.Q, stats, pr["t2"].weight.view(H, 5), pr["t2"].bias, x_hat)

    if not need_backward:
        return emb_loss, x_hat, perplexity, idx, None
    sv.patches, sv.xR_T, sv.z, sv.idx, sv.zq_T, sv.yR_T = patches, xR_T, z, idx, zq_T, yR_T
    sv.Y2, sv.stats = Y2, stats
    sv.Ws, sv.Wd0, sv.Wt1 = Ws, Wd0, Wt1
    return emb_loss, x_hat, perplexity, idx, sv


def fused_head_ok(H):
    return H == 512


def head_train(m, sv, x, gscale, x_hat, sqerr, slot):
    sh, H = sv.sh, sv.sh.H
    pr = _params(m)
    bn = pr["bn"]
    g_xhat = torch.empty_like(x_hat)
    K.unpatch_head_fwd_bwd1(sv.Y2, sh.Q, sv.stats, pr["t2"].weight.view(H, 5), pr["t2"].bias, x, gscale, x_hat,
                            g_xhat, sqerr, sv.head_gsums, slot(pr["t2"].weight).view(H, 5), slot(pr["t2"].bias),
                            slot(bn.weight), slot(bn.bias))
    sv.head_pass1_done = True
    return g_xhat


@torch.no_grad()
def encode(m, x, dtype=F32):
    T = F32 if dtype is None else operand_dtype(dtype)
    if x.dtype != F32 or x.dim() != 3:
        raise ValueError("expected float32 windows of shape (W, seq_len, input_dim)")
    x = x.contiguous()
    sh = VQVAEShapes(m, x.shape[0])
    H, D, N, R, P = sh.H, sh.D, sh.N, sh.R, sh.P
    if x.shape[1] != sh.L or x.shape[2] != sh.C:
        raise ValueError(f"expected windows (W, {sh.L}, {sh.C}), got {tuple(x.shape)}")
    pr = _params(m)
    e = lambda *s, dt=F32: torch.empty(*s, device=x.device, dtype=dt)
    Wp = e(H, sh.ldp, dt=T)
    K.weight_relayout(pr["pe"].weight, H, 1, P, 0, 4, Wp, ldo=sh.ldp)
    patches = e(N, sh.ldp, dt=T)
    K.patchify(x, P, patches)
    xr, a = e(N, H), e(N, H, dt=T)
    K.gemm(patches, Wp, N, H, sh.ldp, bias=pr["pe"].bias, C=xr, C2=a, c2_mode=1, flops=2 * N * H * P)
    ew = [(e(H, H, dt=T), e(H, H, dt=T)) for _ in range(R)]
    Ws = e(D, H, dt=T)
    geo = resstack.Geometry(1, H, sh.S)
    K.weight_relayout_batch([geo.fwd_job(c.weight, w) for cs, ws in zip(pr["enc"], ew) for c, w in zip(cs, ws)]
                            + [(pr["sep"].weight, D, H, 1, 0, 0, Ws)])
    _, xR_T, _ = resstack.forward(geo, xr, a, ew, _biases(pr["enc"]), pr["enc_bn"], T=T, RT=F32, training=m.training,
                                  in_place=True, save=False)
    if R == 0:
        xR_T = _operand(xr, T)
    z = e(N, D)
    K.gemm(xR_T, Ws, N, D, H, bias=pr["sep"].bias, C=z)
    if pr["E"] is None:
        rvq = m.vector_quantization.vq
        if rvq.num_quantizers != 1:
            raise ValueError("tokenization needs a single quantizer (ResidualVQ num_quantizers == 1)")
        _, idx2, _, _ = rvq.quantize_rows(z, False)
        return idx2[:, 0].contiguous(), z
    zq, idx = e(N, D), e(N, dt=torch.int64)
    counts = torch.zeros(sh.K, device=x.device)
    sq = torch.zeros(1, device=x.device, dtype=torch.float64)
    K.vq_forward(z, pr["E"], zq, idx, counts, sq)
    return idx, z


def _cast(t, T):
    out = torch.empty(t.shape, device=t.device, dtype=T)
    K.cast(t, out)
    return out


def _operand(x, T):
    return x if x.dtype == T else _cast(x, T)


def _biases(convs):
    return [(c1.bias, c2.bias) for c1, c2 in convs]


def _grads(convs, slot):
    return lambda r, i: (slot(convs[r][i].weight), slot(convs[r][i].bias))


@K.store_policy(nat.AW_STORE_WT)
def backward(m, sv, g_emb, g_xhat, slot, mid_hook=None):
    sh, T, p_drop = sv.sh, sv.T, sv.p_drop
    H, D, N, S, R, P, k1 = sh.H, sh.D, sh.N, sh.S, sh.R, sh.P, sh.k1
    pr = _params(m)
    dev = g_xhat.device
    e = lambda *s, dt=F32: torch.empty(*s, device=dev, dtype=dt)
    g_xhat = g_xhat.contiguous()
    bn = pr["bn"]

    gsums = sv.head_gsums
    owner = m.__dict__.get("_acc_owner")
    if owner is not None and owner() is sv:
        m.__dict__["_acc_owner"] = None
    if not getattr(sv, "head_pass1_done", False):
        K.unpatch_head_bwd1(sv.Y2, sh.Q, sv.stats, pr["t2"].weight.view(H, 5), g_xhat, gsums,
                            slot(pr["t2"].weight).view(H, 5), slot(pr["t2"].bias), slot(bn.weight), slot(bn.bias))
    gY = e(N * k1, H, dt=T)
    K.unpatch_head_bwd2(sv.Y2, sh.Q, sv.stats, pr["t2"].weight.view(H, 5), g_xhat, gsums, sv.training, gY,
                        slot(pr["t1"].bias))
    gY2 = gY.view(N, k1 * H)
    K.gemm(sv.yR_T, gY2, H, k1 * H, N, a_trans=True, b_trans=True, C=slot(pr["t1"].weight).view(H, H * k1),
           accumulate=True, col_map=(H, k1, 0))
    RT = sv.RT
    gy, go = e(N, H, dt=RT), e(N, H, dt=T)
    bnm = m.batch_norm and R > 0
    K.gemm(gY2, sv.Wt1, N, H, k1 * H, b_trans=True, C=gy, C2=None if bnm else go, c2_mode=0 if bnm else
           (3 if R > 0 else 2), drop2=(p_drop, sv.dec.seeds[-1] if R > 0 else 0), seed_ptr=sv.ctr)

    dgw = [(sv.ops[f"dgw{r}_1"], sv.ops[f"dgw{r}_2"]) for r in range(R)]
    gy, go, wgrads = resstack.backward(sv.dec, gy, go, dgw, _grads(pr["dec"], slot), pr["dec_bn"], slot)
    K.gemm_grouped(wgrads)

    K.gemm(go, sv.zq_T, H, D, N, a_trans=True, b_trans=True, C=slot(pr["dec0"].weight).view(H, D), accumulate=True,
           a_rowsum=slot(pr["dec0"].bias))
    gzq = e(N, D)
    K.gemm(go, sv.Wd0, N, D, H, b_trans=True, C=gzq)

    dz = e(N, D)
    dz_T = dz if T == F32 else None
    if pr["E"] is None:
        res, qs = sv.rvq
        nq = res.shape[0]
        K.rvq_backward(res, qs, gzq, g_emb if nq == 1 else g_emb.expand(nq).contiguous(), dz)
    else:
        dz_T = dz if T == F32 else e(N, D, dt=T)
        K.vq_backward(sv.z, pr["E"], sv.idx, gzq, g_emb, m.vector_quantization.beta, dz, slot(pr["E"]),
                      dz_copy=None if T == F32 else dz_T)
    if mid_hook is not None:
        with K.store_policy(nat.AW_STORE_NT):
            mid_hook()
    if dz_T is None:
        dz_T = _cast(dz, T)

    K.gemm(dz_T, sv.xR_T, D, H, N, a_trans=True, b_trans=True, C=slot(pr["sep"].weight).view(D, H), accumulate=True,
           a_rowsum=slot(pr["sep"].bias))
    gx, gxo = e(N, H, dt=RT), e(N, H, dt=T)
    K.gemm(dz_T, sv.Ws, N, H, D, b_trans=True, C=gx, C2=None if bnm else gxo, c2_mode=0 if bnm else
           (3 if R > 0 else 2), drop2=(p_drop, sv.enc.seeds[-1] if R > 0 else 0), seed_ptr=sv.ctr)

    gx, gxo, wgrads = resstack.backward(sv.enc, gx, gxo, sv.enc.ws, _grads(pr["enc"], slot), pr["enc_bn"], slot)
    K.wgrad_issue(wgrads)

    K.gemm(gxo, sv.patches, H, P, N, a_trans=True, b_trans=True, C=slot(pr["pe"].weight).view(H, P),
           accumulate=True, a_rowsum=slot(pr["pe"].bias))


class VQVAEPatchFunction(torch.autograd.Function):

    @staticmethod
    def forward(ctx, m, x, seed, *params):
        training = m.training
        need = torch.is_grad_enabled() or any(p.requires_grad for p in params)
        emb, x_hat, perp, idx, sv = forward(m, x, training, need_backward=True, seed=seed)
        ctx.m, ctx.sv, ctx.params = m, sv, params
        if perp is not None:
            ctx.mark_non_differentiable(perp)
        m._last_indices = idx
        return emb, x_hat, perp

    @staticmethod
    def backward(ctx, g_emb, g_xhat, g_perp):
        m, sv = ctx.m, ctx.sv
        sink = getattr(m, "_grad_sink", None)
        grads = {}

        def slot(p):
            if sink is not None and p in sink:
                return sink[p]
            g = grads.get(p)
            if g is None:
                g = torch.zeros_like(p, dtype=F32)
                grads[p] = g
            return g

        if g_emb is None:
            g_emb = torch.zeros(1, device=g_xhat.device)
        if g_xhat is None:
            g_xhat = torch.zeros(sv.sh.B, sv.sh.L, sv.sh.C, device=g_emb.device)
        backward(m, sv, g_emb.reshape(1).contiguous(), g_xhat, slot)
        ctx.sv = None
        return (None, None, None) + tuple(grads.get(p) for p in ctx.params)
```

### vq-vae-transformer-arc-welding_amd/csrc/gemm_core.h

```cpp
#pragma once
#include "common.h"

#pragma clang diagnostic ignored "-Winline-asm"

namespace awg {

constexpr int BN = 128;
constexpr int ROWB = 128;
constexpr int CPITCH = BN + 4;

template <int BMT> struct Cfg;
#ifndef AW_W8
#define AW_W8 1
#endif
#if AW_W8
template <> struct Cfg<128> { static constexpr int NTH = 512, NSTAGE = 2, MINB = 4; };
#else
template <> struct Cfg<128> { static constexpr int NTH = 256, NSTAGE = 2, MINB = 2; };
#endif
template <> struct Cfg<256> { static constexpr int NTH = 512, NSTAGE = 3, MINB = 1; };
template <int BMT> constexpr int stage_bytes() { return (BMT + BN) * ROWB; }
template <int BMT> constexpr int smem_bytes() {
  return Cfg<BMT>::NSTAGE * stage_bytes<BMT>() > BMT * CPITCH * 4 ? Cfg<BMT>::NSTAGE * stage_bytes<BMT>()
                                                                   : BMT * CPITCH * 4;
}

template <typename T> struct TT;
template <> struct TT<bf16> {
  static constexpr int EPC = 8, BK = 64;
  __device__ static constexpr int rot(int k) { return 32 * ((k & 3) + 4 * ((k >> 3) & 1)); }
};
template <> struct TT<float> {
  static constexpr int EPC = 4, BK = 32;
  __device__ static constexpr int rot(int k) { return 64 * ((k >> 2) & 1); }
};

__device__ __forceinline__ int nt_off(int row, int chunk) { return row * ROWB + ((chunk ^ ((row >> 1) & 7)) << 4); }
template <typename T, int MPB>
__device__ __forceinline__ int tr_off(int krow, int byte_in_row) {
  return krow * MPB + ((byte_in_row + TT<T>::rot(krow)) & (MPB - 1));
}

struct GemmP {
  aw_gemm_args a;
  int tiles_n, nblocks, splits, ksplit;
  int vec;
  int a_bytes, b_bytes;
  float* ws;
  int ngroups, tiles_per_group;
  int bm;
  const void* gA[AW_GEMM_MAX_GROUPS];
  const void* gB[AW_GEMM_MAX_GROUPS];
  void* gC[AW_GEMM_MAX_GROUPS];
  float* gRow[AW_GEMM_MAX_GROUPS];
};

enum { CONV_NONE = 0, CONV_ROWSHIFT = 1, CONV_KSHIFT = 2 };

enum EpiBits : uint32_t {
  EP_BIAS = 1u << 0, EP_BIASMOD = 1u << 1, EP_PRE = 1u << 2, EP_TANH = 1u << 3, EP_DROP = 1u << 4,
  EP_RESID = 1u << 5, EP_BETA = 1u << 6, EP_C = 1u << 7, EP_CBF = 1u << 8, EP_C2ACT = 1u << 9,
  EP_C2COPY = 1u << 10, EP_C2DROP = 1u << 11, EP_C2BF = 1u << 12, EP_STATS = 1u << 13, EP_ACCUM = 1u << 14,
  EP_PREBF = 1u << 15, EP_RESIDBF = 1u << 16, EP_DERIV = 1u << 17, EP_C2DACT = 1u << 18, EP_GENERIC = 1u << 31
};

#ifdef AW_GEMM_STAMPS
static __device__ uint64_t g_gemm_stamps[8192 * 8];
#define AW_STAMP(i) do { if (threadIdx.x == 0 && blockIdx.y == 0 && blockIdx.x < 8192) \
    g_gemm_stamps[blockIdx.x * 8 + (i)] = __builtin_amdgcn_s_memrealtime(); } while (0)
#define AW_STAMP_EXPORT(name)                                                                                   \
  extern "C" int name(uint64_t* out, int n) {                                                                  \
    if (hipMemcpyFromSymbol(out, HIP_SYMBOL(awg::g_gemm_stamps), (size_t)n * 8) != hipSuccess) return -1;     \
    static uint64_t zeros[8192 * 8];                                                                            \
    return hipMemcpyToSymbol(HIP_SYMBOL(awg::g_gemm_stamps), zeros, sizeof(zeros)) == hipSuccess ? n : -1;    \
  }
#else
#define AW_STAMP(i) do { } while (0)
#define AW_STAMP_EXPORT(name)
#endif

constexpr int OOB = 0x7FFFFFF0;
typedef int v4i32 __attribute__((ext_vector_type(4)));

template <typename T, bool TR, int CONV, bool RAGGED, int ROWS, int NTH>
struct Stager {
  static constexpr int EPC = TT<T>::EPC, BK = TT<T>::BK;
  static constexpr int CPR = ROWS / EPC;
  static constexpr int CPK = BK / EPC;
  static constexpr int MPB = ROWS * (int)sizeof(T);
  static constexpr int NCH = ROWS * 8 / NTH;
  const T* base;
  int64_t ld;
  int rows_total, row0, kend, cin, seg, dir;
  __amdgpu_buffer_rsrc_t rsrc;
  v4i32 desc;
  int wpos[NCH];
  int tapoff[NCH];
  int colin[NCH];

  __device__ __forceinline__ static int tr_logical_m(int c, bool dma) {
    if (!dma) return (c % CPR) * EPC;
    const int pb = (c % CPR) * 16;
    return ((pb - TT<T>::rot(c / CPR)) & (MPB - 1)) / (int)sizeof(T);
  }

  __device__ __forceinline__ void init(int kbeg, int tid, int nbytes, bool dma) {
    rsrc = __builtin_amdgcn_make_buffer_rsrc((void*)base, (short)0, nbytes, 0x00020000);
    const uint64_t b = (uint64_t)(uintptr_t)base;
    desc = v4i32{(int)__builtin_amdgcn_readfirstlane((uint32_t)b),
                 (int)__builtin_amdgcn_readfirstlane((uint32_t)(b >> 32) & 0xFFFFu),
                 (int)__builtin_amdgcn_readfirstlane((uint32_t)nbytes), 0x00020000};
#pragma unroll
    for (int i = 0; i < NCH; ++i) {
      const int c = tid + i * NTH;
      if constexpr (CONV == CONV_ROWSHIFT) {
        wpos[i] = (row0 + c / CPK) % seg;
      } else if constexpr (CONV == CONV_KSHIFT) {
        const int m = row0 + tr_logical_m(c, dma);
        const int j = m / cin;
        tapoff[i] = j - 1;
        colin[i] = m - j * cin;
        wpos[i] = (kbeg + c / CPR) % seg;
      }
    }
  }

  __device__ __forceinline__ uint4 bload(int off) const {
    auto r = __builtin_amdgcn_raw_buffer_load_b128(rsrc, off, 0, 0);
    uint4 u;
    memcpy(&u, &r, 16);
    return u;
  }

  __device__ __forceinline__ int64_t src_nt(int i, int jrow, int row, int k, bool& ok) const {
    ok = row < rows_total && k < kend;
    int src = row, kk = k;
    if constexpr (CONV == CONV_ROWSHIFT) {
      kk = k - jrow * cin;
      const int sft = dir * (jrow - 1);
      ok = ok && (wpos[i] + sft >= 0) && (wpos[i] + sft < seg);
      src = row + sft;
    }
    return (int64_t)src * ld + kk;
  }
  __device__ __forceinline__ int64_t src_tr(int i, int k, int m, bool& ok) {
    ok = k < kend && m < rows_total;
    int srck = k, mm = m;
    if constexpr (CONV == CONV_KSHIFT) {
      mm = colin[i];
      const int sft = tapoff[i];
      ok = ok && (wpos[i] + sft >= 0) && (wpos[i] + sft < seg);
      srck = k + sft;
      wpos[i] += BK % seg;
      if (wpos[i] >= seg) wpos[i] -= seg;
    }
    return (int64_t)srck * ld + mm;
  }

  __device__ __forceinline__ void load(int k0, int tid, uint4 (&v)[NCH]) {
    const int jrow = (CONV == CONV_ROWSHIFT) ? k0 / cin : 0;
#pragma unroll
    for (int i = 0; i < NCH; ++i) {
      const int c = tid + i * NTH;
      bool ok;
      if constexpr (!TR) {
        const int k = k0 + (c % CPK) * EPC;
        const int64_t e = src_nt(i, jrow, row0 + c / CPK, k, ok);
        if constexpr (RAGGED) {
          if (ok && k + EPC > kend) {
            T tmp[EPC];
#pragma unroll
            for (int q = 0; q < EPC; ++q) tmp[q] = (k + q < kend) ? base[e + q] : from_f32<T>(0.f);
            memcpy(&v[i], tmp, 16);
            continue;
          }
        }
        v[i] = bload(ok ? (int)(e * (int)sizeof(T)) : OOB);
      } else {
        const int m = row0 + (c % CPR) * EPC;
        const int64_t e = src_tr(i, k0 + c / CPR, m, ok);
        if constexpr (RAGGED) {
          if (ok && m + EPC > rows_total) {
            T tmp[EPC];
#pragma unroll
            for (int q = 0; q < EPC; ++q) tmp[q] = (m + q < rows_total) ? base[e + q] : from_f32<T>(0.f);
            memcpy(&v[i], tmp, 16);
            continue;
          }
        }
        v[i] = bload(ok ? (int)(e * (int)sizeof(T)) : OOB);
      }
    }
  }

  __device__ __forceinline__ void store(char* lds, int tid, const uint4 (&v)[NCH]) const {
#pragma unroll
    for (int i = 0; i < NCH; ++i) {
      const int c = tid + i * NTH;
      if constexpr (!TR)
        *reinterpret_cast<uint4*>(lds + nt_off(c / CPK, c % CPK)) = v[i];
      else
        *reinterpret_cast<uint4*>(lds + tr_off<T, MPB>(c / CPR, (c % CPR) * 16)) = v[i];
    }
  }

  int doff[NCH];
  int rbase[NCH];
  int dpos[NCH];
  bool rok[NCH];
  uint32_t lds0;
  int dj, dkc;
  static constexpr uint32_t OOB_F = 0x80000000u;

  __device__ __forceinline__ void retap() {
    const int sft = dir * (dj - 1);
#pragma unroll
    for (int i = 0; i < NCH; ++i) {
      const bool ok = rok[i] && (unsigned)(wpos[i] + sft) < (unsigned)seg;
      doff[i] = ok ? rbase[i] + (int)((int64_t)sft * ld * (int)sizeof(T)) : (int)OOB_F;
    }
  }

  __device__ __forceinline__ void dma_init(int tid, uint32_t img_lds, int kbeg) {
    lds0 = img_lds + __builtin_amdgcn_readfirstlane((uint32_t)(tid & ~63)) * 16u;
#pragma unroll
    for (int i = 0; i < NCH; ++i) {
      const int c = tid + i * NTH;
      if constexpr (!TR) {
        const int r = c / CPK;
        const int lc = (c % CPK) ^ ((r >> 1) & 7);
        const int row = row0 + r;
        rok[i] = row < rows_total;
        dpos[i] = lc * EPC;
        rbase[i] = rok[i] ? (int)(((int64_t)row * ld + lc * EPC) * (int)sizeof(T)) : 0;
        doff[i] = rok[i] ? rbase[i] : (int)OOB_F;
      } else {
        const int kr = c / CPR;
        const int m = row0 + tr_logical_m(c, true);
        rok[i] = m < rows_total;
        dpos[i] = kr;
        if constexpr (CONV == CONV_KSHIFT)
          doff[i] = (int)(((int64_t)(kr + tapoff[i]) * ld + colin[i]) * (int)sizeof(T));
        else
          doff[i] = rok[i] ? (int)(((int64_t)kr * ld + m) * (int)sizeof(T)) : (int)OOB_F;
      }
    }
    if constexpr (CONV == CONV_ROWSHIFT) {
      dj = kbeg / cin;
      dkc = kbeg - dj * cin;
      retap();
    }
  }

  __device__ __forceinline__ void dma(int k0, uint32_t stage_off) {
    int delta;
    if constexpr (!TR)
      delta = (CONV == CONV_ROWSHIFT ? dkc : k0) * (int)sizeof(T);
    else
      delta = (int)((int64_t)k0 * ld * (int)sizeof(T));
    const bool full = k0 + BK <= kend;
#pragma unroll
    for (int i = 0; i < NCH; ++i) {
      int off;
      if constexpr (CONV == CONV_KSHIFT) {
        bool ok = rok[i] & (k0 + dpos[i] < kend);
        ok = ok & ((unsigned)(wpos[i] + tapoff[i]) < (unsigned)seg);
        wpos[i] += BK % seg;
        if (wpos[i] >= seg) wpos[i] -= seg;
        off = ok ? doff[i] + delta : OOB;
      } else {
        off = doff[i] + delta;
        if (!full) off = (k0 + dpos[i] < kend) ? off : OOB;
      }
      const uint32_t m0 = lds0 + stage_off + (uint32_t)(i * NTH * 16);
      asm volatile("s_mov_b32 m0, %0\n\tbuffer_load_dwordx4 %1, %2, 0 offen lds" ::"s"(m0), "v"(off), "s"(desc)
                   : "memory", "m0");
    }
    if constexpr (CONV == CONV_ROWSHIFT) {
      dkc += BK;
      if (dkc >= cin) {
        dkc = 0;
        ++dj;
        retap();
      }
    }
  }
};

typedef short v4i16 __attribute__((ext_vector_type(4)));
typedef __attribute__((address_space(3))) v4i16 lds_v4i16;

template <typename T, bool TR, int MPB>
__device__ __forceinline__ uint4 frag(const char* lds, int rbase, int lane, int u) {
  const int g = lane >> 4, i = lane & 15;
  if constexpr (!TR) {
    return *reinterpret_cast<const uint4*>(lds + nt_off(rbase + i, 4 * u + g));
  } else if constexpr (sizeof(T) == 2) {
    const int q = i >> 2, p = i & 3;
    const int k0 = 32 * u + 8 * g + q;
    const v4i16 lo = __builtin_amdgcn_ds_read_tr16_b64_v4i16(
        (lds_v4i16*)(uintptr_t)(lds + tr_off<T, MPB>(k0, 2 * (rbase + 4 * p))));
    const v4i16 hi = __builtin_amdgcn_ds_read_tr16_b64_v4i16(
        (lds_v4i16*)(uintptr_t)(lds + tr_off<T, MPB>(k0 + 4, 2 * (rbase + 4 * p))));
    uint4 out;
    memcpy(&out, &lo, 8);
    memcpy(reinterpret_cast<char*>(&out) + 8, &hi, 8);
    return out;
  } else {
    float f[4];
#pragma unroll
    for (int s = 0; s < 4; ++s)
      f[s] = *reinterpret_cast<const float*>(lds + tr_off<T, MPB>(16 * u + 4 * g + s, 4 * (rbase + i)));
    uint4 out;
    memcpy(&out, f, 16);
    return out;
  }
}

template <typename T> struct Mfma;
template <> struct Mfma<bf16> {
  __device__ __forceinline__ static void run(f32x4& acc, const uint4& a, const uint4& b) {
    acc = __builtin_amdgcn_mfma_f32_16x16x32_bf16(__builtin_bit_cast(bf16x8, a), __builtin_bit_cast(bf16x8, b), acc,
                                                  0, 0, 0);
  }
};
template <> struct Mfma<float> {
  __device__ __forceinline__ static void run(f32x4& acc, const uint4& a, const uint4& b) {
    f32x4 av, bv;
    memcpy(&av, &a, 16);
    memcpy(&bv, &b, 16);
#pragma unroll
    for (int s = 0; s < 4; ++s) acc = __builtin_amdgcn_mfma_f32_16x16x4f32(av[s], bv[s], acc, 0, 0, 0);
  }
};

#ifndef AW_GEMM_NT
#define AW_GEMM_NT 1
#endif
__device__ __forceinline__ void store4(void* base, bool is_bf16, int64_t e, const float (&v)[4], bool wt) {
  if (is_bf16) {
    bf16 h[4] = {(bf16)v[0], (bf16)v[1], (bf16)v[2], (bf16)v[3]};
    u32x2 u;
    memcpy(&u, h, 8);
    u32x2* d = reinterpret_cast<u32x2*>(reinterpret_cast<bf16*>(base) + e);
    if (wt) aw_st_wt(d, u);
    else if (AW_GEMM_NT) __builtin_nontemporal_store(u, d);
    else *d = u;
  } else {
    f32x4 u = {v[0], v[1], v[2], v[3]};
    f32x4* d = reinterpret_cast<f32x4*>(reinterpret_cast<float*>(base) + e);
    if (wt) aw_st_wt(d, u);
    else if (AW_GEMM_NT) __builtin_nontemporal_store(u, d);
    else *d = u;
  }
}

__device__ __forceinline__ int xcd_remap(int bid, int nblocks) {
  const int q = nblocks / 8, r = nblocks % 8;
  const int xcd = bid % 8, slot = bid / 8;
  return (xcd < r ? xcd * (q + 1) : r * (q + 1) + (xcd - r) * q) + slot;
}

template <typename T>
__device__ __forceinline__ float frag_sum(const uint4& v) {
  const uint32_t w[4] = {v.x, v.y, v.z, v.w};
  if constexpr (sizeof(T) == 2) {
    const bf16x8 h = __builtin_bit_cast(bf16x8, v);
    float s0 = 0.f, s1 = 0.f;
#pragma unroll
    for (int i = 0; i < 4; ++i) {
      s0 += (float)h[2 * i];
      s1 += (float)h[2 * i + 1];
    }
    return s0 + s1;
  } else {
    return (__uint_as_float(w[0]) + __uint_as_float(w[1])) + (__uint_as_float(w[2]) + __uint_as_float(w[3]));
  }
}

template <int N> __device__ __forceinline__ void wait_vmcnt() { asm volatile("s_waitcnt vmcnt(%0)" ::"n"(N) : "memory"); }

template <typename T, bool ATR, bool BTR, int ACONV, int BCONV, bool RAGGED, uint32_t EPI, int BMT>
__global__ __launch_bounds__(Cfg<BMT>::NTH, RAGGED ? 1 : Cfg<BMT>::MINB) void gemm_kernel(GemmP P) {
  constexpr int NTH = Cfg<BMT>::NTH;
  constexpr int BK = TT<T>::BK;
  constexpr int A_IMG = BMT * ROWB;
  constexpr int STAGE = stage_bytes<BMT>();
  static_assert(!(RAGGED && BMT != 128), "ragged shapes use the 128-row register-staged tile");
  using SA = Stager<T, ATR, ACONV, RAGGED, BMT, NTH>;
  using SB = Stager<T, BTR, BCONV, RAGGED, BN, NTH>;
  const aw_gemm_args& p = P.a;
  __shared__ __attribute__((aligned(16))) char smem[smem_bytes<BMT>()];

  AW_STAMP(0);
  const int tid = threadIdx.x;
  const int lane = tid & 63, wid = tid >> 6;
  const int wm = wid >> 1, wn = wid & 1;
  constexpr int WR = BMT / (NTH / 128);
  constexpr int FM = WR / 16;
  int tile = xcd_remap(blockIdx.x, P.nblocks);
  const void* Aptr = p.A;
  const void* Bptr = p.B;
  void* Cptr = p.C;
  float* rowptr = p.a_rowsum;
  if (P.ngroups > 1) {
    const int g = tile / P.tiles_per_group;
    tile -= g * P.tiles_per_group;
    Aptr = P.gA[g];
    Bptr = P.gB[g];
    Cptr = P.gC[g];
    rowptr = P.gRow[g];
  }
  const int tm = tile / P.tiles_n, tn = tile % P.tiles_n;
  const int m0 = tm * BMT, n0 = tn * BN;
  const int M = p.M, N = p.N;
  const int kbeg = blockIdx.y * P.ksplit;
  const int kend = min(p.K, kbeg + P.ksplit);

  SA sa{reinterpret_cast<const T*>(Aptr), p.lda, M, m0, kend, p.conv_cin, p.conv_seg, p.conv_dir};
  SB sb{reinterpret_cast<const T*>(Bptr), p.ldb, N, n0, kend, p.conv_cin, p.conv_seg, 1};
  constexpr bool use_dma = !RAGGED;
  sa.init(kbeg, tid, P.a_bytes, use_dma);
  sb.init(kbeg, tid, P.b_bytes, use_dma);
  if constexpr (use_dma) {
    const uint32_t smem_lds = (uint32_t)(uintptr_t)(__attribute__((address_space(3))) char*)smem;
    sa.dma_init(tid, smem_lds, kbeg);
    sb.dma_init(tid, smem_lds + A_IMG, kbeg);
  }
  const bool do_rowsum = rowptr != nullptr && tn == 0;

  f32x4 acc[FM][4];
#pragma unroll
  for (int i = 0; i < FM; ++i)
#pragma unroll
    for (int j = 0; j < 4; ++j) acc[i][j] = f32x4{0.f, 0.f, 0.f, 0.f};
  constexpr bool ROWSUM_OK = (EPI & EP_GENERIC) || (EPI & EP_ACCUM);
  const bool wave_rowsum = ROWSUM_OK && do_rowsum && wn == 0;
  float rowacc[FM] = {};

  auto compute = [&](const char* a_l) {
    const char* b_l = a_l + A_IMG;
#pragma unroll
    for (int u = 0; u < 2; ++u) {
      uint4 af[FM], bfr[4];
#pragma unroll
      for (int f = 0; f < FM; ++f) af[f] = frag<T, ATR, BMT * (int)sizeof(T)>(a_l, wm * WR + f * 16, lane, u);
#pragma unroll
      for (int f = 0; f < 4; ++f) bfr[f] = frag<T, BTR, BN * (int)sizeof(T)>(b_l, wn * 64 + f * 16, lane, u);
#pragma unroll
      for (int i = 0; i < FM; ++i)
#pragma unroll
        for (int j = 0; j < 4; ++j) Mfma<T>::run(acc[i][j], af[i], bfr[j]);
      if (wave_rowsum) {
#pragma unroll
        for (int f = 0; f < FM; ++f) rowacc[f] += frag_sum<T>(af[f]);
      }
    }
  };

  const int nk = kend > kbeg ? (kend - kbeg + BK - 1) / BK : 0;
  if constexpr (use_dma && Cfg<BMT>::NSTAGE == 2) {
    char* L0 = smem;
    char* L1 = smem + STAGE;
    sa.dma(kbeg, 0u);
    sb.dma(kbeg, 0u);
    wait_vmcnt<0>();
    __syncthreads();
    AW_STAMP(1);
    for (int kt = 0; kt < nk; ++kt) {
      char* cur = (kt & 1) ? L1 : L0;
      const uint32_t nxt = (kt & 1) ? 0u : (uint32_t)STAGE;
      if (kt + 1 < nk) {
        sa.dma(kbeg + (kt + 1) * BK, nxt);
        sb.dma(kbeg + (kt + 1) * BK, nxt);
      }
      compute(cur);
      wait_vmcnt<0>();
      __syncthreads();
    }
  } else if constexpr (use_dma) {
    constexpr int PER_STEP = SA::NCH + SB::NCH;
    const int grp = wid >> 2;
    auto stage_of = [](int t) { return (uint32_t)((t % 3) * STAGE); };
    sa.dma(kbeg, 0u);
    sb.dma(kbeg, 0u);
    if (nk > 1) {
      sa.dma(kbeg + BK, stage_of(1));
      sb.dma(kbeg + BK, stage_of(1));
      wait_vmcnt<PER_STEP>();
    } else {
      wait_vmcnt<0>();
    }
    __builtin_amdgcn_sched_barrier(0);
    __builtin_amdgcn_s_barrier();
    __builtin_amdgcn_sched_barrier(0);
    if (grp == 1) __builtin_amdgcn_s_barrier();
    AW_STAMP(1);
    uint4 af[2][FM], bfr[2][4];
    for (int kt = 0; kt < nk; ++kt) {
      const char* a_l = smem + stage_of(kt);
      const char* b_l = a_l + A_IMG;
#pragma unroll
      for (int u = 0; u < 2; ++u) {
#pragma unroll
        for (int f = 0; f < FM; ++f) af[u][f] = frag<T, ATR, BMT * (int)sizeof(T)>(a_l, wm * WR + f * 16, lane, u);
#pragma unroll
        for (int f = 0; f < 4; ++f) bfr[u][f] = frag<T, BTR, BN * (int)sizeof(T)>(b_l, wn * 64 + f * 16, lane, u);
      }
      if (kt + 2 < nk) {
        sa.dma(kbeg + (kt + 2) * BK, stage_of(kt + 2));
        sb.dma(kbeg + (kt + 2) * BK, stage_of(kt + 2));
        wait_vmcnt<PER_STEP>();
      } else {
        wait_vmcnt<0>();
      }
      asm volatile("s_waitcnt lgkmcnt(0)" ::: "memory");
      __builtin_amdgcn_sched_barrier(0);
      __builtin_amdgcn_s_barrier();
      __builtin_amdgcn_sched_barrier(0);
      __builtin_amdgcn_s_setprio(1);
#pragma unroll
      for (int u = 0; u < 2; ++u)
#pragma unroll
        for (int i = 0; i < FM; ++i)
#pragma unroll
          for (int j = 0; j < 4; ++j) Mfma<T>::run(acc[i][j], af[u][i], bfr[u][j]);
      __builtin_amdgcn_s_setprio(0);
      if (wave_rowsum) {
#pragma unroll
        for (int u = 0; u < 2; ++u)
#pragma unroll
          for (int f = 0; f < FM; ++f) rowacc[f] += frag_sum<T>(af[u][f]);
      }
      __builtin_amdgcn_sched_barrier(0);
      __builtin_amdgcn_s_barrier();
      __builtin_amdgcn_sched_barrier(0);
    }
    if (grp == 0) __builtin_amdgcn_s_barrier();
  } else {
    char* L0 = smem;
    char* L1 = smem + STAGE;
    uint4 ra0[SA::NCH], rb0[SB::NCH], ra1[SA::NCH], rb1[SB::NCH];
    sa.load(kbeg, tid, ra0);
    sb.load(kbeg, tid, rb0);
    sa.load(kbeg + BK, tid, ra1);
    sb.load(kbeg + BK, tid, rb1);
    sa.store(L0, tid, ra0);
    sb.store(L0 + A_IMG, tid, rb0);
    __syncthreads();
    AW_STAMP(1);
    for (int kt = 0; kt < nk; kt += 2) {
      sa.load(kbeg + (kt + 2) * BK, tid, ra0);
      sb.load(kbeg + (kt + 2) * BK, tid, rb0);
      compute(L0);
      sa.store(L1, tid, ra1);
      sb.store(L1 + A_IMG, tid, rb1);
      __syncthreads();
      if (kt + 1 >= nk) break;
      sa.load(kbeg + (kt + 3) * BK, tid, ra1);
      sb.load(kbeg + (kt + 3) * BK, tid, rb1);
      compute(L1);
      sa.store(L0, tid, ra0);
      sb.store(L0 + A_IMG, tid, rb0);
      __syncthreads();
    }
  }

  AW_STAMP(2);
  if (wave_rowsum) {
#pragma unroll
    for (int f = 0; f < FM; ++f) {
      float v = rowacc[f];
      v += __shfl_xor(v, 16, 64);
      v += __shfl_xor(v, 32, 64);
      const int r = m0 + wm * WR + f * 16 + lane;
      if (lane < 16 && r < M) atomicAdd(rowptr + r, v);
    }
  }

#define EPF(bit, rt) ((EPI & EP_GENERIC) ? (rt) : ((EPI & (bit)) != 0))
  constexpr bool GEN = (EPI & EP_GENERIC) != 0;
  constexpr int NR = NTH / 32;
  float* Cs = reinterpret_cast<float*>(smem);
  {
    const int cq = lane & 15, rq = (lane >> 4) * 4;
#pragma unroll
    for (int i = 0; i < FM; ++i)
#pragma unroll
      for (int j = 0; j < 4; ++j)
#pragma unroll
        for (int r = 0; r < 4; ++r)
          Cs[(wm * WR + i * 16 + rq + r) * CPITCH + wn * 64 + j * 16 + cq] = acc[i][j][r];
  }
  __syncthreads();
  AW_STAMP(3);
  const int rows_here = min(BMT, M - m0);
  if (EPF(EP_ACCUM, P.splits > 1 || p.accumulate)) {
    if (P.splits > 1 && P.ws) {
      const int lc = tid & 127, col = n0 + lc;
      if (col >= N) return;
      float* slab = P.ws + (int64_t)blockIdx.y * M * N;
      for (int lr = tid >> 7; lr < rows_here; lr += NTH / 128)
        slab[(int64_t)(m0 + lr) * N + col] = Cs[lr * CPITCH + lc];
      return;
    }
    const int lc = tid & 127, col = n0 + lc;
    if (col >= N) return;
    const int64_t oc = p.col_mod > 0 ? (int64_t)(col % p.col_mod) * p.col_mul + col / p.col_mod + p.col_off
                                     : (int64_t)col * (p.col_mul > 0 ? p.col_mul : 1) + p.col_off;
    float* C = reinterpret_cast<float*>(Cptr);
    for (int lr = tid >> 7; lr < rows_here; lr += NTH / 128)
      atomicAdd(C + (int64_t)(m0 + lr) * p.ldc + oc, p.alpha * Cs[lr * CPITCH + lc]);
    return;
  }
  if constexpr (!GEN && (EPI & EP_ACCUM)) return;
  else {
  const bool f_bias = EPF(EP_BIAS, p.bias != nullptr);
  const bool f_bmod = EPF(EP_BIASMOD, p.bias_mod > 0);
  const bool f_pre = EPF(EP_PRE, p.pre != nullptr);
  const bool f_prebf = EPF(EP_PREBF, p.pre_dtype == AW_BF16);
  const bool f_tanh = EPF(EP_TANH, p.act == AW_ACT_GELU_TANH);
  const bool f_deriv = EPF(EP_DERIV, p.act == AW_ACT_DERIV);
  const bool f_drop = EPF(EP_DROP, p.drop_p > 0.f);
  const bool f_resid = EPF(EP_RESID, p.resid != nullptr);
  const bool f_residbf = EPF(EP_RESIDBF, p.resid_dtype == AW_BF16);
  const bool f_beta = EPF(EP_BETA, p.beta != 0.f);
  const bool f_c = EPF(EP_C, Cptr != nullptr);
  const bool f_cbf = EPF(EP_CBF, p.c_dtype == AW_BF16);
  const int c2m = GEN ? p.c2_mode
                      : ((EPI & EP_C2ACT) ? 1 : (EPI & EP_C2COPY) ? 2 : (EPI & EP_C2DROP) ? 3 : (EPI & EP_C2DACT) ? 4 : 0);
  const bool f_c2bf = EPF(EP_C2BF, p.c2_dtype == AW_BF16);
  const bool f_stats = EPF(EP_STATS, p.colstats != nullptr);
  const float alpha = GEN ? p.alpha : 1.f;
  const bool wt = p.store_policy == AW_STORE_WT;
  constexpr bool FASTGELU = sizeof(T) == 2;
  const uint64_t dseed = f_drop ? aw_seed_mix(p.drop_seed, p.seed_ptr) : 0ull;
  const uint64_t dseed2 = c2m == 3 ? aw_seed_mix(p.drop2_seed, p.seed_ptr) : 0ull;
  const int c4 = (tid & 31) * 4, r0 = tid >> 5;
  const int col = n0 + c4;
  const bool vec = GEN ? (P.vec && col + 4 <= N) : (col < N);
  float bias[4], csum[4] = {0.f, 0.f, 0.f, 0.f}, csq[4] = {0.f, 0.f, 0.f, 0.f};
#pragma unroll
  for (int e = 0; e < 4; ++e) {
    const int c = col + e;
    bias[e] = (f_bias && c < N) ? p.bias[f_bmod ? c % p.bias_mod : c] : 0.f;
  }
  if (col < N) {
    for (int lr0 = r0; lr0 < rows_here; lr0 += 4 * NR) {
      float4 pre4[4], res4[4], old4[4];
#pragma unroll
      for (int u = 0; u < 4; ++u) {
        const int lr = lr0 + NR * u;
        if (lr >= rows_here) break;
        const int64_t row = m0 + lr;
        if (vec) {
          if (f_pre) {
            if (f_prebf) {
              const uint2 h = *reinterpret_cast<const uint2*>(reinterpret_cast<const bf16*>(p.pre) + row * p.ld_pre + col);
              pre4[u] = make_float4(__uint_as_float(h.x << 16), __uint_as_float(h.x & 0xFFFF0000u),
                                    __uint_as_float(h.y << 16), __uint_as_float(h.y & 0xFFFF0000u));
            } else {
              pre4[u] = *reinterpret_cast<const float4*>(p.pre + row * p.ld_pre + col);
            }
          }
          if (f_resid) {
            if (f_residbf) {
              const uint2 h = *reinterpret_cast<const uint2*>(reinterpret_cast<const bf16*>(p.resid) + row * p.ld_resid + col);
              res4[u] = make_float4(__uint_as_float(h.x << 16), __uint_as_float(h.x & 0xFFFF0000u),
                                    __uint_as_float(h.y << 16), __uint_as_float(h.y & 0xFFFF0000u));
            } else {
              res4[u] = *reinterpret_cast<const float4*>(p.resid + row * p.ld_resid + col);
            }
          }
          if (f_beta) old4[u] = *reinterpret_cast<const float4*>(reinterpret_cast<const float*>(Cptr) + row * p.ldc + col);
        } else if constexpr (GEN) {
          float a[4] = {0.f, 0.f, 0.f, 0.f}, b[4] = {0.f, 0.f, 0.f, 0.f}, c[4] = {0.f, 0.f, 0.f, 0.f};
#pragma unroll
          for (int e = 0; e < 4; ++e) {
            if (col + e >= N) break;
            if (f_pre) a[e] = load_as_f32(p.pre, p.pre_dtype, row * p.ld_pre + col + e);
            if (f_resid) b[e] = load_as_f32(p.resid, p.resid_dtype, row * p.ld_resid + col + e);
            if (f_beta) c[e] = reinterpret_cast<const float*>(Cptr)[row * p.ldc + col + e];
          }
          pre4[u] = make_float4(a[0], a[1], a[2], a[3]);
          res4[u] = make_float4(b[0], b[1], b[2], b[3]);
          old4[u] = make_float4(c[0], c[1], c[2], c[3]);
        }
      }
#pragma unroll
      for (int u = 0; u < 4; ++u) {
        const int lr = lr0 + NR * u;
        if (lr >= rows_here) break;
        const int64_t row = m0 + lr;
        const float4 a4 = *reinterpret_cast<const float4*>(Cs + lr * CPITCH + c4);
        const float av[4] = {a4.x, a4.y, a4.z, a4.w};
        const float pv[4] = {pre4[u].x, pre4[u].y, pre4[u].z, pre4[u].w};
        const float rv[4] = {res4[u].x, res4[u].y, res4[u].z, res4[u].w};
        const float ov[4] = {old4[u].x, old4[u].y, old4[u].z, old4[u].w};
        const uint64_t e0 = (uint64_t)row * N + col;
        float ds[4] = {1.f, 1.f, 1.f, 1.f}, ds2[4] = {1.f, 1.f, 1.f, 1.f};
        if (f_drop) aw_dropout_scale4(dseed, e0, p.drop_p, ds);
        if (c2m == 3) aw_dropout_scale4(dseed2, e0, p.drop2_p, ds2);
        float v[4], w[4], ag[4];
        if (FASTGELU && f_pre && !f_tanh && !f_deriv) aw_gelu_grad4(pv, ag);
#pragma unroll
        for (int e = 0; e < 4; ++e) {
          float x = alpha * av[e] + bias[e];
          float m = 1.f;
          bool has_m = false;
          if (f_pre) {
            const float a = f_deriv ? pv[e] : f_tanh ? gelu_tanh_grad(pv[e]) : (FASTGELU ? ag[e] : gelu_erf_grad(pv[e]));
            if (f_drop) x *= a;
            else m = a, has_m = true;
          }
          if (f_drop) m = ds[e], has_m = true;
          x = aw_epi_mad(x, m, has_m, f_resid ? rv[e] : 0.f, f_resid);
          if (f_beta) x += p.beta * ov[e];
          v[e] = x;
          float y = x;
          if (c2m == 1 && (f_tanh || !FASTGELU)) y = f_tanh ? gelu_tanh(x) : gelu_erf(x);
          else if (c2m == 3) y = x * ds2[e];
          w[e] = y;
          if (f_stats && col + e < N) {
            csum[e] += x;
            csq[e] += x * x;
          }
        }
        if (FASTGELU && c2m == 1 && !f_tanh) aw_gelu4(v, w);
        if (c2m == 4 && f_tanh && FASTGELU) {
#pragma unroll
          for (int e = 0; e < 4; e += 2) {
            f32x2 g, dg;
            gelu_tanh_and_grad2((f32x2){v[e], v[e + 1]}, g, dg);
            v[e] = g.x, v[e + 1] = g.y, w[e] = dg.x, w[e + 1] = dg.y;
          }
        } else if (c2m == 4) {
#pragma unroll
          for (int e = 0; e < 4; ++e) {
            float g, dg;
            if (f_tanh) {
              gelu_tanh_and_grad(v[e], g, dg);
            } else {
              float ex;
              const float phi = FASTGELU ? aw_phi_e(v[e], ex) : 0.f;
              g = FASTGELU ? v[e] * phi : gelu_erf(v[e]);
              dg = FASTGELU ? fmaf(v[e] * AW_INV_SQRT2PI, ex, phi) : gelu_erf_grad(v[e]);
            }
            v[e] = g;
            w[e] = dg;
          }
        }
        if (vec) {
          if (f_c) store4(Cptr, f_cbf, row * p.ldc + col, v, wt);
          if (c2m) store4(p.C2, f_c2bf, row * p.ldc2 + col, w, wt);
        } else if constexpr (GEN) {
#pragma unroll
          for (int e = 0; e < 4; ++e) {
            if (col + e >= N) break;
            if (f_c) store_from_f32(Cptr, p.c_dtype, row * p.ldc + col + e, v[e]);
            if (c2m) store_from_f32(p.C2, p.c2_dtype, row * p.ldc2 + col + e, w[e]);
          }
        }
      }
    }
  }
  AW_STAMP(4);
  if (f_stats) {
    __syncthreads();
    float* red = Cs;
#pragma unroll
    for (int e = 0; e < 4; ++e) {
      red[(r0 * 2 + 0) * 128 + c4 + e] = csum[e];
      red[(r0 * 2 + 1) * 128 + c4 + e] = csq[e];
    }
    __syncthreads();
    if (tid < 128 && n0 + tid < N) {
      float a = 0.f, b = 0.f;
#pragma unroll
      for (int g = 0; g < NR; ++g) {
        a += red[(g * 2 + 0) * 128 + tid];
        b += red[(g * 2 + 1) * 128 + tid];
      }
      const int sl = (n0 + tid) % p.stats_mod;
      atomicAdd(p.colstats + sl, (double)a);
      atomicAdd(p.colstats + p.stats_mod + sl, (double)b);
    }
  }
  }
#undef EPF
}

enum Layout { L_NN = 0, L_NN_CONV = 1, L_NT = 2, L_NT_CONV = 3, L_TN = 4, L_TT = 5, L_TT_KCONV = 6 };

template <Layout LY> struct LayoutArgs;
template <> struct LayoutArgs<L_NN> { static constexpr bool ATR = false, BTR = false; static constexpr int AC = CONV_NONE, BC = CONV_NONE; };
template <> struct LayoutArgs<L_NN_CONV> { static constexpr bool ATR = false, BTR = false; static constexpr int AC = CONV_ROWSHIFT, BC = CONV_NONE; };
template <> struct LayoutArgs<L_NT> { static constexpr bool ATR = false, BTR = true; static constexpr int AC = CONV_NONE, BC = CONV_NONE; };
template <> struct LayoutArgs<L_NT_CONV> { static constexpr bool ATR = false, BTR = true; static constexpr int AC = CONV_ROWSHIFT, BC = CONV_NONE; };
template <> struct LayoutArgs<L_TN> { static constexpr bool ATR = true, BTR = false; static constexpr int AC = CONV_NONE, BC = CONV_NONE; };
template <> struct LayoutArgs<L_TT> { static constexpr bool ATR = true, BTR = true; static constexpr int AC = CONV_NONE, BC = CONV_NONE; };
template <> struct LayoutArgs<L_TT_KCONV> { static constexpr bool ATR = true, BTR = true; static constexpr int AC = CONV_NONE, BC = CONV_KSHIFT; };

template <typename T, Layout LY, bool RAGGED, uint32_t EPI, int BMT>
inline void launch_kernel(const GemmP& P, hipStream_t s) {
  using LA = LayoutArgs<LY>;
  hipLaunchKernelGGL((gemm_kernel<T, LA::ATR, LA::BTR, LA::AC, LA::BC, RAGGED, EPI, BMT>), dim3(P.nblocks, P.splits),
                     dim3(Cfg<BMT>::NTH), 0, s, P);
}

template <typename T, Layout LY, uint32_t EPI>
inline void launch_tiled(const GemmP& P, hipStream_t s) {
  if constexpr (sizeof(T) == 2 && (EPI == EP_GENERIC || EPI == EP_ACCUM)) {
    if (P.bm == 256) {
      launch_kernel<T, LY, false, EPI, 256>(P, s);
      return;
    }
  }
  launch_kernel<T, LY, false, EPI, 128>(P, s);
}

bool launch_fast_fwd(const GemmP& P, hipStream_t s, bool is_bf16, Layout ly, uint32_t code, bool launch);
bool launch_fast_bwd(const GemmP& P, hipStream_t s, bool is_bf16, Layout ly, uint32_t code, bool launch);
bool launch_fast_256(const GemmP& P, hipStream_t s, Layout ly, uint32_t code, bool launch);
bool wgrad_conv3_try(const aw_gemm_args* args, int n, hipStream_t s);


}
```

### vq-vae-transformer-arc-welding_amd/csrc/reschain.hip

```cpp
#include "common.h"

#include <type_traits>

#pragma clang diagnostic ignored "-Winline-asm"


namespace {

constexpr int EC_H = 512;
constexpr int EC_ROWS = 64;
constexpr int EC_NTH = 512;
constexpr int EC_ROWB = EC_H * 2;
constexpr int EC_SCR = 2048;
constexpr int EC_SEG = 16;

template <int TAPS> struct EcGeo {
  static constexpr int KS = 16 * TAPS;
  static constexpr int JS = (TAPS == 1 ? 16 : 17) * EC_ROWB;
  static constexpr int R0 = TAPS == 1 ? 0 : EC_ROWB;
  static constexpr int IMG = (TAPS == 1 ? 64 : 69) * EC_ROWB;
  static constexpr int SCR = 2 * IMG;
  static constexpr int FLAGS = SCR + 8 * EC_SCR;
  static constexpr int BIAS = FLAGS + 64;
  static constexpr int LDS = BIAS + 8 * 256;
  static constexpr uint32_t WBYTES = (uint32_t)EC_H * EC_H * 2 * TAPS;
  static constexpr int WWAVE = 4 * KS * 1024;
  static constexpr uint64_t KEYS = TAPS == 1 ? 0xfe76dc54ba329810ull : 0xf53ac739685ace10ull;
  __device__ static int key(int u) { return u < 0 ? 15 : u > 15 ? 0 : (int)((KEYS >> (4 * u)) & 15); }
};
static_assert(EcGeo<3>::LDS <= 160 * 1024, "decoder chain LDS");

typedef __amdgpu_buffer_rsrc_t rsrc_t;
__device__ __forceinline__ rsrc_t ec_rsrc(const void* p, uint32_t nbytes) {
  return __builtin_amdgcn_make_buffer_rsrc((void*)p, (short)0, p ? nbytes : 0u, 0x00020000);
}
__device__ __forceinline__ u32x2 ec_load8(rsrc_t r, uint32_t voff, int soff) {
  return __builtin_amdgcn_raw_buffer_load_b64(r, voff, soff, 0);
}
template <bool WT> __device__ __forceinline__ void ec_store16(rsrc_t r, uint32_t voff, int soff, uint4 v) {
  aw_v4i32 u;
  memcpy(&u, &v, 16);
  __builtin_amdgcn_raw_buffer_store_b128(u, r, voff, soff, WT ? 16 : 2);
  asm volatile("s_nop 1" ::"v"(u));
}
__device__ __forceinline__ void ec_store8(rsrc_t r, uint32_t voff, u32x2 v) {
  __builtin_amdgcn_raw_buffer_store_b64(v, r, voff, 0, 2);
}
typedef __attribute__((ext_vector_type(2))) __bf16 bf16x2;
__device__ __forceinline__ u32x2 ec_pack(const float (&v)[4]) {
  const bf16x2 lo = __builtin_convertvector((f32x2){v[0], v[1]}, bf16x2);
  const bf16x2 hi = __builtin_convertvector((f32x2){v[2], v[3]}, bf16x2);
  return u32x2{__builtin_bit_cast(uint32_t, lo), __builtin_bit_cast(uint32_t, hi)};
}
__device__ __forceinline__ void ec_unpack(u32x2 u, float (&v)[4]) {
  v[0] = __uint_as_float(u.x << 16);
  v[1] = __uint_as_float(u.x & 0xFFFF0000u);
  v[2] = __uint_as_float(u.y << 16);
  v[3] = __uint_as_float(u.y & 0xFFFF0000u);
}
__device__ __forceinline__ uint4 ec_wload(rsrc_t r, int voff, int soff) {
  const auto v = __builtin_amdgcn_raw_buffer_load_b128(r, voff, soff, 0);
  uint4 u;
  memcpy(&u, &v, 16);
  return u;
}
__device__ __forceinline__ void ec_lds_w8(char* smem, int off, u32x2 v) { *reinterpret_cast<u32x2*>(smem + off) = v; }
__device__ __forceinline__ uint4 ec_lds_r16(const char* smem, int off) {
  return *reinterpret_cast<const uint4*>(smem + off);
}

template <class G> __device__ __forceinline__ int ec_off(int tok, int chunk) {
  return G::R0 + (tok >> 4) * G::JS + (tok & 15) * EC_ROWB + ((chunk ^ G::key(tok & 15)) << 4);
}

template <class G>
__device__ __forceinline__ void ec_load_image(char* img, const void* src, int64_t row0, uint32_t nbytes, int tid) {
  const rsrc_t rs = ec_rsrc(src, nbytes);
#pragma unroll
  for (int q = 0; q < (EC_ROWS * EC_ROWB / 16) / EC_NTH; ++q) {
    const int c = tid + q * EC_NTH, tok = c >> 6, ch = c & 63;
    const uint32_t off = (uint32_t)((row0 + tok) * EC_ROWB + ch * 16);
    const auto v = __builtin_amdgcn_raw_buffer_load_b128(rs, off, 0, 0);
    uint4 u;
    memcpy(&u, &v, 16);
    *reinterpret_cast<uint4*>(img + ec_off<G>(tok, ch)) = u;
  }
  if constexpr (G::R0 != 0) {
    for (int c = tid; c < 2 * 5 * 64; c += EC_NTH) {
      const int im = c / 320, row = (c % 320) >> 6, ch = c & 63;
      *reinterpret_cast<uint4*>(img + im * G::IMG + row * G::JS + ch * 16) = uint4{0u, 0u, 0u, 0u};
    }
  }
}

typedef __attribute__((address_space(3))) volatile int lds_vint;
template <class G> __device__ __forceinline__ lds_vint* ec_flag(char* smem, int wv) {
  return (lds_vint*)(smem + G::FLAGS) + wv;
}
template <class G> __device__ __forceinline__ void ec_wait(char* smem, int wv, int target) {
  while (__builtin_amdgcn_readfirstlane(*ec_flag<G>(smem, wv)) < target) __builtin_amdgcn_s_sleep(1);
  asm volatile("" ::: "memory");
}
template <class G> __device__ __forceinline__ void ec_publish(char* smem, int w, int lane, int count) {
  asm volatile("s_waitcnt lgkmcnt(0)" ::: "memory");
  if (lane == 0) *ec_flag<G>(smem, w) = count;
}

__device__ __forceinline__ void ec_frag_fence(int) { __builtin_amdgcn_sched_barrier(0); }

__device__ __forceinline__ void ec_gelu_grad4(const float (&v)[4], float (&y)[4]) {
#pragma unroll
  for (int e = 0; e < 4; ++e) y[e] = gelu_erf_grad_fast(v[e]);
}
__device__ __forceinline__ void ec_gelu_and_grad4(const float (&v)[4], float (&y)[4], float (&d)[4]) {
#pragma unroll
  for (int e = 0; e < 4; ++e) {
    float ex;
    const float phi = aw_phi_e(v[e], ex);
    y[e] = v[e] * phi;
    d[e] = fmaf(v[e] * AW_INV_SQRT2PI, ex, phi);
  }
}

template <class G> __device__ __forceinline__ constexpr int ec_woff(int i, int s) { return (i * G::KS + s) * 1024; }

__device__ __forceinline__ size_t ec_keep_idx(int r, int tid) {
  return ((size_t)r * gridDim.x + blockIdx.x) * EC_NTH + tid;
}
__device__ __forceinline__ u32x2 ec_keep(const uint64_t* masks, int r, int tid) {
  return __builtin_bit_cast(u32x2, masks[ec_keep_idx(r, tid)]);
}
__device__ __forceinline__ uint32_t ec_keep_bits(uint64_t seed, uint64_t grp0, int f, uint32_t thr) {
  uint32_t lo = (uint32_t)grp0, hi = (uint32_t)(grp0 >> 32);
  asm volatile("" : "+v"(lo), "+v"(hi));
  const uint64_t h = aw_hash_group(seed, (((uint64_t)hi << 32) | lo) + 2048u * (f & 3) + 4u * (f >> 2));
  uint32_t k = 0;
#pragma unroll
  for (int e = 0; e < 4; ++e) k |= (((uint32_t)(h >> (16 * e)) & 0xFFFFu) >= thr ? 1u : 0u) << (4 * (f & 7) + e);
  return k;
}
__device__ __forceinline__ void ec_scales(u32x2 keep, int i, int j, float k, float (&ds)[4]) {
  const int f = 4 * i + j;
  const uint32_t b = ((f >> 3) ? keep.y : keep.x) >> (4 * (f & 7));
#pragma unroll
  for (int e = 0; e < 4; ++e) ds[e] = (b >> e) & 1u ? k : 0.f;
}

template <class G, typename Tail, typename Step>
__device__ __forceinline__ void ec_conv(f32x4 (&acc)[4][4], uint4 (&wf)[2][4], char* smem, const int (&rb)[G::KS / 16],
                                        int io, rsrc_t rc, rsrc_t rn, bool has_next, int wl, int w, int target,
                                        Tail tail, Step step) {
  constexpr int T = G::KS / 16;
#pragma unroll
  for (int i = 0; i < 4; ++i)
#pragma unroll
    for (int j = 0; j < 4; ++j) acc[i][j] = f32x4{0.f, 0.f, 0.f, 0.f};
  int rbi[T];
#pragma unroll
  for (int t = 0; t < T; ++t) rbi[t] = rb[t] + io;
#pragma unroll
  for (int s = 0; s < G::KS; ++s) {
    const int t = s >> 4, kk = s & 15;
    if (t == 0 && (kk & 1) == 0 && (kk >> 1) != w) ec_wait<G>(smem, kk >> 1, target);
    uint4 bf[4];
#pragma unroll
    for (int j = 0; j < 4; ++j) bf[j] = ec_lds_r16(smem, (rbi[t] ^ (64 * (kk & 3))) + (kk >> 2) * 256 + j * G::JS);
#pragma unroll
    for (int i = 0; i < 4; ++i)
#pragma unroll
      for (int j = 0; j < 4; ++j)
        acc[i][j] = __builtin_amdgcn_mfma_f32_16x16x32_bf16(__builtin_bit_cast(bf16x8, wf[s & 1][i]),
                                                            __builtin_bit_cast(bf16x8, bf[j]), acc[i][j], 0, 0, 0);
    if (s + 2 < G::KS) {
#pragma unroll
      for (int i = 0; i < 4; ++i) wf[s & 1][i] = ec_wload(rc, wl, ec_woff<G>(i, s + 2));
    } else if (has_next) {
#pragma unroll
      for (int i = 0; i < 4; ++i) wf[s & 1][i] = ec_wload(rn, wl, ec_woff<G>(i, s + 2 - G::KS));
    }
    step(s);
    if (s == G::KS - 1) tail();
    __builtin_amdgcn_sched_barrier(0);
  }
}

template <class G, int DIR> struct EcLane {
  static constexpr int T = G::KS / 16;
  int lane, li, g, w;
  int wl;
  int rb[T];
  int wb0;
  __device__ __forceinline__ EcLane(int tid) {
    lane = tid & 63;
    w = tid >> 6, g = lane >> 4, li = lane & 15;
    wl = w * G::WWAVE + lane * 16;
#pragma unroll
    for (int t = 0; t < T; ++t) {
      const int tp = li + (T == 1 ? 0 : DIR * (t - 1)), key = G::key(tp);
      rb[t] = G::R0 + tp * EC_ROWB + ((4 * (key >> 2) + (g ^ (key & 3))) << 4);
    }
    wb0 = G::R0 + li * EC_ROWB + (((8 * w + (g >> 1)) ^ G::key(li)) << 4) + (g & 1) * 8;
  }
  __device__ __forceinline__ int wb(int i) const { return wb0 ^ (32 * i); }
};
template <class G> struct EcStore {
  int ir[2];
  int sw[4];
  int sr;
  __device__ __forceinline__ int srq(int q) const { return q ? (sr ^ 64) + 1024 : sr; }
  uint32_t gs;
  __device__ __forceinline__ EcStore(int tid, int64_t row0) {
    const int lane = tid & 63, w = tid >> 6, g = lane >> 4, li = lane & 15;
    const int t8 = lane >> 3, c8 = lane & 7;
#pragma unroll
    for (int p = 0; p < 2; ++p) ir[p] = G::R0 + (8 * p + t8) * EC_ROWB + (((8 * w + c8) ^ G::key(8 * p + t8)) << 4);
    const int sbase = G::SCR + w * EC_SCR;
#pragma unroll
    for (int i = 0; i < 4; ++i) sw[i] = sbase + li * 128 + (((2 * i + (g >> 1)) ^ (li >> 1)) << 4) + (g & 1) * 8;
    sr = sbase + t8 * 128 + ((c8 ^ (t8 >> 1)) << 4);
    gs = (uint32_t)(((row0 + t8) * EC_H + 64 * w + 8 * c8) * 2);
  }
};

__device__ __forceinline__ void ec_load_frags(u32x2 (&d)[4][4], rsrc_t r, uint32_t go) {
#pragma unroll
  for (int i = 0; i < 4; ++i)
#pragma unroll
    for (int j = 0; j < 4; ++j) d[i][j] = ec_load8(r, go, 16384 * j + 32 * i);
}
__device__ __forceinline__ uint32_t ec_frag_off(int64_t row0, int li, int w, int g) {
  return (uint32_t)(((row0 + li) * EC_H + 64 * w + 4 * g) * 2);
}
template <class G, bool WT>
__device__ __forceinline__ void ec_store_slice(const char* smem, int img, const EcStore<G>& S, rsrc_t r) {
  const int b0 = img + S.ir[0], b1 = img + S.ir[1];
#pragma unroll
  for (int q = 0; q < 8; ++q)
    ec_store16<WT>(r, S.gs, 8192 * q, ec_lds_r16(smem, ((q & 1) ? b1 : b0) + G::JS * (q >> 1)));
}
template <class G, bool WT>
__device__ __forceinline__ void ec_store_scratch(const char* smem, int j, const EcStore<G>& S, rsrc_t r) {
#pragma unroll
  for (int q = 0; q < 2; ++q) ec_store16<WT>(r, S.gs, 8192 * (2 * j + q), ec_lds_r16(smem, S.srq(q)));
}

template <class G> __device__ __forceinline__ void ec_init(char* smem, int tid) {
  if (tid < 8) *ec_flag<G>(smem, tid) = 0;
}

template <int TAPS, bool DROP, bool WT>
__global__ __launch_bounds__(EC_NTH) void res_chain_fwd_kernel(aw_res_chain_fwd_args P) {
  using G = EcGeo<TAPS>;
  __shared__ __attribute__((aligned(16))) char smem[G::LDS];
  const int tid = threadIdx.x;
  const int64_t row0 = (int64_t)blockIdx.x * EC_ROWS;
  const EcLane<G, 1> L(tid);
  const uint32_t nbytes = (uint32_t)(P.N * EC_ROWB);
  const int R = P.R, NC = 2 * R;

  ec_init<G>(smem, tid);
  ec_load_image<G>(smem, P.a0, row0, nbytes, tid);
  u32x2 xr[4][4];
  ec_load_frags(xr, ec_rsrc(P.x0, nbytes), ec_frag_off(row0, L.li, L.w, L.g));
  uint4 wf[2][4];
  {
    const rsrc_t r0 = ec_rsrc(P.w1[0], G::WBYTES);
#pragma unroll
    for (int i = 0; i < 4; ++i) {
      wf[0][i] = ec_wload(r0, L.wl, ec_woff<G>(i, 0));
      wf[1][i] = ec_wload(r0, L.wl, ec_woff<G>(i, 1));
    }
  }
  const rsrc_t rmask = ec_rsrc(DROP ? P.drop_masks : nullptr, (uint32_t)(R * gridDim.x * EC_NTH * 8));
  const uint32_t thr = aw_drop_threshold(P.drop_p);
  const uint64_t grp0 = (uint64_t)(row0 + L.li) * (EC_H / 4) + 16 * L.w + L.g;
  asm volatile("s_waitcnt lgkmcnt(0)" ::: "memory");
  __syncthreads();

  for (int c = 0; c < NC; ++c) {
    const int r = c >> 1;
    const bool second = (c & 1) != 0;
    const rsrc_t rc = ec_rsrc(second ? P.w2[r] : P.w1[r], G::WBYTES);
    const bool has_next = c + 1 < NC;
    const rsrc_t rn = ec_rsrc(has_next ? (second ? P.w1[r + 1] : P.w2[r]) : nullptr, G::WBYTES);
    const int io = (c & 1) * G::IMG, no = ((c + 1) & 1) * G::IMG;
    f32x4 acc[4][4];
    const float bias_l = (second ? P.b2[r] : P.b1[r])[64 * L.w + L.lane];
    const uint64_t seed = DROP && second ? aw_seed_mix(P.drop_seed[r], P.seed_ptr) : 0;
    uint32_t kb[2] = {0u, 0u};
    auto hash = [&](int s) {
      if (DROP && second && s < 16) kb[s >> 3] |= ec_keep_bits(seed, grp0, s, thr);
    };
    auto park = [&] {
      *reinterpret_cast<float*>(smem + G::BIAS + 256 * L.w + 4 * L.lane) = bias_l;
      if (DROP && second) ec_store8(rmask, (uint32_t)(ec_keep_idx(r, tid) * 8), u32x2{kb[0], kb[1]});
    };
    ec_conv<G>(acc, wf, smem, L.rb, io, rc, rn, has_next, L.wl, L.w, c, park, hash);
    const u32x2 keep = {kb[0], kb[1]};
    int nwb[4];
#pragma unroll
    for (int i = 0; i < 4; ++i) nwb[i] = L.wb(i) + no;

    auto bias = [&](int i, float (&bv)[4]) {
      const float4 b4 = *reinterpret_cast<const float4*>(smem + G::BIAS + 256 * L.w + 64 * i + 16 * L.g);
      bv[0] = b4.x, bv[1] = b4.y, bv[2] = b4.z, bv[3] = b4.w;
    };
    const EcStore<G> S(tid, row0);
    if (!second) {
      const rsrc_t rh = ec_rsrc(P.dgelu_h[r], nbytes);
#pragma unroll
      for (int j = 0; j < 4; ++j) {
#pragma unroll
        for (int i = 0; i < 4; ++i) {
          float v[4], y[4], d[4], bv[4];
          bias(i, bv);
#pragma unroll
          for (int e = 0; e < 4; ++e) v[e] = acc[i][j][e] + bv[e];
          ec_gelu_and_grad4(v, y, d);
          ec_lds_w8(smem, nwb[i] + G::JS * j, ec_pack(y));
          ec_lds_w8(smem, S.sw[i], ec_pack(d));
          ec_frag_fence(4 * j + i);
        }
        ec_store_scratch<G, WT>(smem, j, S, rh);
        __builtin_amdgcn_sched_barrier(0);
      }
      ec_publish<G>(smem, L.w, L.lane, c + 1);
      ec_store_slice<G, WT>(smem, no, S, ec_rsrc(P.a1[r], nbytes));
    } else {
      const bool last = r == R - 1;
      const float dk = DROP ? 1.f / (1.f - P.drop_p) : 1.f;
      auto resid = [&](int i, int j, float (&v)[4]) {
        float ds[4] = {1.f, 1.f, 1.f, 1.f}, xv[4], bv[4];
        bias(i, bv);
        if constexpr (DROP) ec_scales(keep, i, j, dk, ds);
        ec_unpack(xr[i][j], xv);
#pragma unroll
        for (int e = 0; e < 4; ++e) v[e] = aw_epi_mad(acc[i][j][e] + bv[e], ds[e], DROP, xv[e], true);
        xr[i][j] = ec_pack(v);
      };
      if (!last) {
        const rsrc_t rx = ec_rsrc(P.dgelu_x[r], nbytes);
#pragma unroll
        for (int j = 0; j < 4; ++j) {
#pragma unroll
          for (int i = 0; i < 4; ++i) {
            float v[4], y[4], d[4];
            resid(i, j, v);
            ec_gelu_and_grad4(v, y, d);
            ec_lds_w8(smem, nwb[i] + G::JS * j, ec_pack(y));
            ec_lds_w8(smem, S.sw[i], ec_pack(d));
            ec_frag_fence(4 * j + i);
          }
          ec_store_scratch<G, WT>(smem, j, S, rx);
          __builtin_amdgcn_sched_barrier(0);
        }
        ec_publish<G>(smem, L.w, L.lane, c + 1);
      } else {
#pragma unroll
        for (int i = 0; i < 4; ++i)
#pragma unroll
          for (int j = 0; j < 4; ++j) {
            float v[4];
            resid(i, j, v);
            ec_lds_w8(smem, nwb[i] + G::JS * j, xr[i][j]);
            ec_frag_fence(4 * i + j);
          }
      }
      ec_store_slice<G, WT>(smem, no, S, ec_rsrc(P.a[r], nbytes));
    }
  }
}

template <int TAPS, bool DROP, bool WT>
__global__ __launch_bounds__(EC_NTH) void res_chain_bwd_kernel(aw_res_chain_bwd_args P) {
  using G = EcGeo<TAPS>;
  __shared__ __attribute__((aligned(16))) char smem[G::LDS];
  const int tid = threadIdx.x;
  const int64_t row0 = (int64_t)blockIdx.x * EC_ROWS;
  const EcLane<G, -1> L(tid);
  const uint32_t nbytes = (uint32_t)(P.N * EC_ROWB);
  const int R = P.R, NC = 2 * R;
  const uint32_t fo = ec_frag_off(row0, L.li, L.w, L.g);

  ec_init<G>(smem, tid);
  ec_load_image<G>(smem, P.gxo, row0, nbytes, tid);
  u32x2 gr[4][4];
  ec_load_frags(gr, ec_rsrc(P.gx, nbytes), fo);
  uint4 wf[2][4];
  {
    const rsrc_t r0 = ec_rsrc(P.w2t[R - 1], G::WBYTES);
#pragma unroll
    for (int i = 0; i < 4; ++i) {
      wf[0][i] = ec_wload(r0, L.wl, ec_woff<G>(i, 0));
      wf[1][i] = ec_wload(r0, L.wl, ec_woff<G>(i, 1));
    }
  }
  asm volatile("s_waitcnt lgkmcnt(0)" ::: "memory");
  __syncthreads();

  for (int c = 0; c < NC; ++c) {
    const int r = R - 1 - (c >> 1);
    const bool second = (c & 1) != 0;
    const rsrc_t rc = ec_rsrc(second ? P.w1t[r] : P.w2t[r], G::WBYTES);
    const bool has_next = c + 1 < NC;
    const rsrc_t rn = ec_rsrc(has_next ? (second ? P.w2t[r - 1] : P.w1t[r]) : nullptr, G::WBYTES);
    const int io = (c & 1) * G::IMG, no = ((c + 1) & 1) * G::IMG;
    f32x4 acc[4][4];
    uint4 pl[8];
    u32x2 keep = {0u, 0u};
    auto load_pre = [&] {
      const rsrc_t rp = ec_rsrc(second ? (r > 0 ? P.dgelu_x[r] : P.x0) : P.dgelu_h[r], nbytes);
      const uint32_t gs = (uint32_t)(((row0 + (L.lane >> 3)) * EC_H + 64 * L.w + 8 * (L.lane & 7)) * 2);
#pragma unroll
      for (int q = 0; q < 8; ++q) {
        const auto v = __builtin_amdgcn_raw_buffer_load_b128(rp, gs, 8192 * q, 0);
        memcpy(&pl[q], &v, 16);
      }
      if (DROP && second && r > 0) keep = ec_keep(P.drop_masks, r - 1, tid);
    };
    ec_conv<G>(acc, wf, smem, L.rb, io, rc, rn, has_next, L.wl, L.w, c, load_pre, [](int) {});
    int nwb[4];
#pragma unroll
    for (int i = 0; i < 4; ++i) nwb[i] = L.wb(i) + no;
    const EcStore<G> S(tid, row0);
    auto stage_pre = [&](int j) {
      *reinterpret_cast<uint4*>(smem + S.srq(0)) = pl[2 * j];
      *reinterpret_cast<uint4*>(smem + S.srq(1)) = pl[2 * j + 1];
    };
    auto pre_frag = [&](int i, float (&pv)[4]) { ec_unpack(*reinterpret_cast<const u32x2*>(smem + S.sw[i]), pv); };

    if (!second) {
#pragma unroll
      for (int j = 0; j < 4; ++j) {
        stage_pre(j);
#pragma unroll
        for (int i = 0; i < 4; ++i) {
          float ag[4], v[4];
          pre_frag(i, ag);
#pragma unroll
          for (int e = 0; e < 4; ++e) v[e] = aw_epi_mad(acc[i][j][e], ag[e], true, 0.f, false);
          ec_lds_w8(smem, nwb[i] + G::JS * j, ec_pack(v));
          ec_frag_fence(4 * j + i);
        }
      }
      ec_publish<G>(smem, L.w, L.lane, c + 1);
      ec_store_slice<G, WT>(smem, no, S, ec_rsrc(P.gh[r], nbytes));
    } else {
      auto grad = [&](int i, int j, float (&v)[4], auto raw) {
        float pv[4], gv[4], ag[4];
        pre_frag(i, pv);
        ec_unpack(gr[i][j], gv);
        if constexpr (decltype(raw)::value) {
          ec_gelu_grad4(pv, ag);
        } else {
#pragma unroll
          for (int e = 0; e < 4; ++e) ag[e] = pv[e];
        }
#pragma unroll
        for (int e = 0; e < 4; ++e) v[e] = aw_epi_mad(acc[i][j][e], ag[e], true, gv[e], true);
        gr[i][j] = ec_pack(v);
      };
      if (r > 0) {
        const float dk = DROP ? 1.f / (1.f - P.drop_p) : 1.f;
#pragma unroll
        for (int j = 0; j < 4; ++j) {
          stage_pre(j);
#pragma unroll
          for (int i = 0; i < 4; ++i) {
            float v[4], ds[4] = {1.f, 1.f, 1.f, 1.f}, o[4];
            grad(i, j, v, std::false_type{});
            if constexpr (DROP) ec_scales(keep, i, j, dk, ds);
#pragma unroll
            for (int e = 0; e < 4; ++e) o[e] = v[e] * ds[e];
            ec_lds_w8(smem, nwb[i] + G::JS * j, ec_pack(o));
            ec_frag_fence(4 * j + i);
          }
        }
        ec_publish<G>(smem, L.w, L.lane, c + 1);
      } else {
#pragma unroll
        for (int j = 0; j < 4; ++j) {
          stage_pre(j);
#pragma unroll
          for (int i = 0; i < 4; ++i) {
            float v[4];
            grad(i, j, v, std::true_type{});
            ec_lds_w8(smem, nwb[i] + G::JS * j, gr[i][j]);
            ec_frag_fence(4 * j + i);
          }
        }
      }
      ec_store_slice<G, WT>(smem, no, S, ec_rsrc(P.gxo_out[r], nbytes));
    }
  }
}

struct PackJobs {
  const void* src[AW_RES_PACK_MAX];
  void* fwd[AW_RES_PACK_MAX];
  void* bwd[AW_RES_PACK_MAX];
};

constexpr int PK_PITCH1 = 128 + 16;
template <int TAPS>
__global__ __launch_bounds__(256) void res_pack_kernel(PackJobs J) {
  constexpr int RB = EC_ROWB * TAPS, PITCH0 = RB + 16, KB = 16 * TAPS;
  constexpr int SZ = 16 * PITCH0 > EC_H * PK_PITCH1 ? 16 * PITCH0 : EC_H * PK_PITCH1;
  __shared__ __attribute__((aligned(16))) char t[SZ];
  const int x = blockIdx.x, job = blockIdx.y, tid = threadIdx.x;
  const char* __restrict__ W = reinterpret_cast<const char*>(J.src[job]);
  if (blockIdx.z == 0) {
    uint4* __restrict__ out = reinterpret_cast<uint4*>(J.fwd[job]);
    if (!out) return;
    for (int mb = x; mb < EC_H / 16; mb += gridDim.x) {
#pragma unroll
      for (int q = 0; q < 4 * TAPS; ++q) {
        const int c = tid + 256 * q, row = c / (64 * TAPS), kc = c % (64 * TAPS);
        *reinterpret_cast<uint4*>(t + row * PITCH0 + kc * 16) =
            *reinterpret_cast<const uint4*>(W + (size_t)(16 * mb + row) * RB + kc * 16);
      }
      __syncthreads();
#pragma unroll
      for (int q = 0; q < 4 * TAPS; ++q) {
        const int o = tid + 256 * q, st = o >> 6, l = o & 63;
        out[(size_t)mb * 64 * KB + o] = *reinterpret_cast<const uint4*>(t + (l & 15) * PITCH0 + (4 * st + (l >> 4)) * 16);
      }
      __syncthreads();
    }
  } else {
    uint4* __restrict__ out = reinterpret_cast<uint4*>(J.bwd[job]);
    if (!out) return;
    const int tap = x >> 3, b = x & 7;
#pragma unroll
    for (int q = 0; q < 16; ++q) {
      const int c = tid + 256 * q, o = c >> 3, kc = c & 7;
      *reinterpret_cast<uint4*>(t + o * PK_PITCH1 + kc * 16) =
          *reinterpret_cast<const uint4*>(W + (size_t)o * RB + tap * EC_ROWB + 128 * b + kc * 16);
    }
    __syncthreads();
#pragma unroll 4
    for (int q = 0; q < 16; ++q) {
      const int o = tid + 256 * q, mb = o >> 10, st = (o >> 6) & 15, l = o & 63, li = l & 15, g = l >> 4;
      uint16_t e[8];
#pragma unroll
      for (int k = 0; k < 8; ++k)
        e[k] = *reinterpret_cast<const uint16_t*>(t + (32 * st + 8 * g + k) * PK_PITCH1 + (16 * mb + li) * 2);
      uint4 v;
      memcpy(&v, e, 16);
      out[((size_t)(4 * b + mb) * KB + 16 * tap + st) * 64 + l] = v;
    }
  }
}

struct MaskSeeds {
  uint64_t seed[AW_RES_CHAIN_MAX];
};
__global__ __launch_bounds__(EC_NTH) void res_mask_kernel(MaskSeeds S, const uint64_t* seed_ptr, uint32_t thr,
                                                          u32x2* __restrict__ out) {
  const int tid = threadIdx.x, r = blockIdx.y;
  const int lane = tid & 63, w = tid >> 6, g = lane >> 4, li = lane & 15;
  const uint64_t seed = aw_seed_mix(S.seed[r], seed_ptr);
  const uint64_t grp0 = (((uint64_t)blockIdx.x * EC_ROWS + li) * EC_H >> 2) + 16 * w + g;
  uint32_t k[2] = {0u, 0u};
#pragma unroll
  for (int f = 0; f < 16; ++f) k[f >> 3] |= ec_keep_bits(seed, grp0, f, thr);
  out[((size_t)r * gridDim.x + blockIdx.x) * EC_NTH + tid] = u32x2{k[0], k[1]};
}

bool aligned16(const void* p) { return ((uintptr_t)p & 15) == 0; }

template <int TAPS>
void launch_fwd(const aw_res_chain_fwd_args* a, bool drop, bool wt, dim3 grid, hipStream_t s) {
  if (drop && wt) hipLaunchKernelGGL((res_chain_fwd_kernel<TAPS, true, true>), grid, dim3(EC_NTH), 0, s, *a);
  else if (drop) hipLaunchKernelGGL((res_chain_fwd_kernel<TAPS, true, false>), grid, dim3(EC_NTH), 0, s, *a);
  else if (wt) hipLaunchKernelGGL((res_chain_fwd_kernel<TAPS, false, true>), grid, dim3(EC_NTH), 0, s, *a);
  else hipLaunchKernelGGL((res_chain_fwd_kernel<TAPS, false, false>), grid, dim3(EC_NTH), 0, s, *a);
}
template <int TAPS>
void launch_bwd(const aw_res_chain_bwd_args* a, bool drop, bool wt, dim3 grid, hipStream_t s) {
  if (drop && wt) hipLaunchKernelGGL((res_chain_bwd_kernel<TAPS, true, true>), grid, dim3(EC_NTH), 0, s, *a);
  else if (drop) hipLaunchKernelGGL((res_chain_bwd_kernel<TAPS, true, false>), grid, dim3(EC_NTH), 0, s, *a);
  else if (wt) hipLaunchKernelGGL((res_chain_bwd_kernel<TAPS, false, true>), grid, dim3(EC_NTH), 0, s, *a);
  else hipLaunchKernelGGL((res_chain_bwd_kernel<TAPS, false, false>), grid, dim3(EC_NTH), 0, s, *a);
}

}

#define CHAIN_SHAPE_CHECKS(who)                                                                                       \
  AW_REQUIRE(a, who ": null args");                                                                                   \
  AW_REQUIRE(a->H == EC_H, who ": H must be %d (got %d)", EC_H, a->H);                                                \
  AW_REQUIRE(a->R >= 1 && a->R <= AW_RES_CHAIN_MAX, who ": R must be 1..%d", AW_RES_CHAIN_MAX);                       \
  AW_REQUIRE(a->N >= 1 && (a->N + EC_ROWS) * EC_ROWB < (1ll << 31), who ": N out of range");                          \
  AW_REQUIRE(a->taps == 1 || (a->taps == 3 && a->seg == EC_SEG && a->N % EC_SEG == 0),                                \
             who ": taps must be 1, or 3 with seg == %d and N %% %d == 0 (taps %d, seg %d)", EC_SEG, EC_SEG, a->taps, \
             a->seg);                                                                                                 \
  AW_REQUIRE(a->drop_p >= 0.f && a->drop_p < 1.f, who ": drop_p out of [0, 1)")

extern "C" int aw_res_chain_fwd(const aw_res_chain_fwd_args* a, void* stream) {
  CHAIN_SHAPE_CHECKS("aw_res_chain_fwd");
  AW_REQUIRE(a->a0 && a->x0 && aligned16(a->a0) && aligned16(a->x0), "aw_res_chain_fwd: a0 / x0 missing or unaligned");
  for (int r = 0; r < a->R; ++r) {
    AW_REQUIRE(a->w1[r] && a->w2[r] && a->b1[r] && a->b2[r] && aligned16(a->w1[r]) && aligned16(a->w2[r]) &&
               aligned16(a->b1[r]) && aligned16(a->b2[r]), "aw_res_chain_fwd: block %d weights missing or unaligned", r);
    AW_REQUIRE(a->a[r] && aligned16(a->a[r]), "aw_res_chain_fwd: block %d output a missing or unaligned", r);
    AW_REQUIRE(aligned16(a->dgelu_h[r]) && aligned16(a->a1[r]) && aligned16(a->dgelu_x[r]),
               "aw_res_chain_fwd: block %d saved outputs unaligned", r);
  }
  AW_REQUIRE(aligned16(a->drop_masks), "aw_res_chain_fwd: drop_masks unaligned");
  hipStream_t s = (hipStream_t)stream;
  const dim3 grid((unsigned)((a->N + EC_ROWS - 1) / EC_ROWS));
  const bool drop = a->drop_p > 0.f, wt = a->store_policy == AW_STORE_WT;
  if (a->taps == 3) launch_fwd<3>(a, drop, wt, grid, s);
  else launch_fwd<1>(a, drop, wt, grid, s);
  return aw::check_launch("aw_res_chain_fwd");
}

extern "C" int aw_res_chain_bwd(const aw_res_chain_bwd_args* a, void* stream) {
  CHAIN_SHAPE_CHECKS("aw_res_chain_bwd");
  AW_REQUIRE(a->gx && a->gxo && a->x0 && aligned16(a->gx) && aligned16(a->gxo) && aligned16(a->x0),
             "aw_res_chain_bwd: gx / gxo / x0 missing or unaligned");
  for (int r = 0; r < a->R; ++r) {
    AW_REQUIRE(a->w1t[r] && a->w2t[r] && aligned16(a->w1t[r]) && aligned16(a->w2t[r]),
               "aw_res_chain_bwd: block %d weights missing or unaligned", r);
    AW_REQUIRE(a->dgelu_h[r] && aligned16(a->dgelu_h[r]) && (r == 0 || (a->dgelu_x[r] && aligned16(a->dgelu_x[r]))),
               "aw_res_chain_bwd: block %d saved GELU' missing or unaligned", r);
    AW_REQUIRE(a->gh[r] && a->gxo_out[r] && aligned16(a->gh[r]) && aligned16(a->gxo_out[r]),
               "aw_res_chain_bwd: block %d outputs missing or unaligned", r);
  }
  AW_REQUIRE(a->drop_p == 0.f || a->R == 1 || (a->drop_masks && aligned16(a->drop_masks)),
             "aw_res_chain_bwd: drop_p > 0 needs drop_masks");
  hipStream_t s = (hipStream_t)stream;
  const dim3 grid((unsigned)((a->N + EC_ROWS - 1) / EC_ROWS));
  const bool drop = a->drop_p > 0.f && a->R > 1, wt = a->store_policy == AW_STORE_WT;
  if (a->taps == 3) launch_bwd<3>(a, drop, wt, grid, s);
  else launch_bwd<1>(a, drop, wt, grid, s);
  return aw::check_launch("aw_res_chain_bwd");
}

extern "C" int aw_res_pack_weights(const void* const* src, void* const* fwd, void* const* bwd, int n, int taps,
                                   void* stream) {
  AW_REQUIRE(src && fwd && bwd && n >= 0 && n <= AW_RES_PACK_MAX && (taps == 1 || taps == 3),
             "aw_res_pack_weights: bad args (n must be 0..%d, taps 1 or 3)", AW_RES_PACK_MAX);
  if (n == 0) return AW_OK;
  PackJobs J{};
  for (int i = 0; i < n; ++i) {
    AW_REQUIRE(src[i] && aligned16(src[i]) && aligned16(fwd[i]) && aligned16(bwd[i]) && (fwd[i] || bwd[i]) &&
                   src[i] != fwd[i] && src[i] != bwd[i], "aw_res_pack_weights: job %d: missing, aliased or unaligned", i);
    J.src[i] = src[i];
    J.fwd[i] = fwd[i];
    J.bwd[i] = bwd[i];
  }
  const dim3 grid(8 * taps, n, 2);
  if (taps == 3) hipLaunchKernelGGL(res_pack_kernel<3>, grid, dim3(256), 0, (hipStream_t)stream, J);
  else hipLaunchKernelGGL(res_pack_kernel<1>, grid, dim3(256), 0, (hipStream_t)stream, J);
  return aw::check_launch("aw_res_pack_weights");
}

extern "C" int64_t aw_res_dropout_masks_bytes(int64_t N, int R) {
  if (N < 1 || R < 1 || R > AW_RES_CHAIN_MAX) return -1;
  return (int64_t)R * ((N + EC_ROWS - 1) / EC_ROWS) * EC_NTH * 8;
}

extern "C" int aw_res_dropout_masks(int64_t N, int R, float drop_p, const uint64_t* drop_seed, const uint64_t* seed_ptr,
                                    void* masks, void* stream) {
  AW_REQUIRE(N >= 1 && R >= 1 && R <= AW_RES_CHAIN_MAX && drop_seed && masks && aligned16(masks) && drop_p > 0.f &&
                 drop_p < 1.f, "aw_res_dropout_masks: bad args");
  MaskSeeds S{};
  for (int r = 0; r < R; ++r) S.seed[r] = drop_seed[r];
  hipLaunchKernelGGL(res_mask_kernel, dim3((unsigned)((N + EC_ROWS - 1) / EC_ROWS), R), dim3(EC_NTH), 0,
                     (hipStream_t)stream, S, seed_ptr, aw_drop_threshold(drop_p), (u32x2*)masks);
  return aw::check_launch("aw_res_dropout_masks");
}
```

Baseline: 432,700 windows/s.

## Fuse the ConvTranspose head GEMM as a tail into the decoder residual chain kernel

The decoder's persistent residual-chain kernel gains a tail stage that multiplies the final activation tile by the k1 ConvT weight slices, adds the bias, writes the bf16 Y output, and accumulates per-column BN statistics in double via atomics. The separate head GEMM is skipped when the tail is enabled, which is the default. Weight packing is extended so one-tap tail matrices can be packed in the same launch as the chain weights. The aim is to avoid writing and re-reading the last residual output and to save a kernel launch. In exchange the kernel needs more LDS and becomes more complex, and the column-statistic accumulation in the GEMM epilogue also moves to double.

```diff
diff --git a/include/arcweld_amd.h b/include/arcweld_amd.h
--- a/include/arcweld_amd.h
+++ b/include/arcweld_amd.h
@@ -56,6 +56,7 @@
 int aw_wgrad_set_spin_limit(int polls);
 
 #define AW_RES_CHAIN_MAX 16
+#define AW_RES_TAIL_MAX 8
 typedef struct {
   int64_t N;
   int H, R;
@@ -75,6 +76,11 @@
   const uint64_t* seed_ptr;
   int store_policy;
   uint64_t* drop_masks;
+  int tail_k1;
+  const void* tail_w[AW_RES_TAIL_MAX];
+  const float* tail_bias;
+  void* tail_y;
+  double* tail_colstats;
 } aw_res_chain_fwd_args;
 typedef struct {
   int64_t N;
@@ -100,6 +106,8 @@
                          void* masks, void* stream);
 #define AW_RES_PACK_MAX 32
 int aw_res_pack_weights(const void* const* src, void* const* fwd, void* const* bwd, int n, int taps, void* stream);
+int aw_res_pack_weights_mixed(const void* const* src, void* const* fwd, void* const* bwd, const int* job_taps, int n,
+                              int taps, void* stream);
 
 int aw_vq_forward(const float* z, const float* E, int64_t N, int K, int D,
                   float* zq, int64_t* idx, float* counts, double* sqerr, void* stream);
diff --git a/vq-vae-transformer-arc-welding_amd/arcweld/_native.py b/vq-vae-transformer-arc-welding_amd/arcweld/_native.py
--- a/vq-vae-transformer-arc-welding_amd/arcweld/_native.py
+++ b/vq-vae-transformer-arc-welding_amd/arcweld/_native.py
@@ -60,6 +60,7 @@
 
 RES_CHAIN_MAX = 16
 RES_PACK_MAX = 32
+RES_TAIL_MAX = 8
 _E = RES_CHAIN_MAX
 
 
@@ -68,7 +69,9 @@
                 ("w1", c_p * _E), ("w2", c_p * _E), ("b1", c_p * _E), ("b2", c_p * _E),
                 ("dgelu_h", c_p * _E), ("a1", c_p * _E), ("dgelu_x", c_p * _E), ("a", c_p * _E),
                 ("drop_p", c_f), ("drop_seed", ctypes.c_uint64 * _E), ("seed_ptr", c_p), ("store_policy", c_int),
-                ("drop_masks", c_p)]
+                ("drop_masks", c_p),
+                ("tail_k1", c_int), ("tail_w", c_p * RES_TAIL_MAX), ("tail_bias", c_p), ("tail_y", c_p),
+                ("tail_colstats", c_p)]
 
 
 class ResChainBwdArgs(ctypes.Structure):
@@ -93,6 +96,8 @@
     "aw_res_chain_fwd": [ctypes.POINTER(ResChainFwdArgs), c_p],
     "aw_res_chain_bwd": [ctypes.POINTER(ResChainBwdArgs), c_p],
     "aw_res_pack_weights": [ctypes.POINTER(c_p), ctypes.POINTER(c_p), ctypes.POINTER(c_p), c_int, c_int, c_p],
+    "aw_res_pack_weights_mixed": [ctypes.POINTER(c_p), ctypes.POINTER(c_p), ctypes.POINTER(c_p),
+                                  ctypes.POINTER(c_int), c_int, c_int, c_p],
     "aw_res_dropout_masks_bytes": [c_i64, c_int],
     "aw_res_dropout_masks": [c_i64, c_int, c_f, ctypes.POINTER(ctypes.c_uint64), c_p, c_p, c_p],
     "aw_weight_relayout_batch": [ctypes.POINTER(RelayoutJob), c_int, c_int, c_p],
diff --git a/vq-vae-transformer-arc-welding_amd/arcweld/kernels.py b/vq-vae-transformer-arc-welding_amd/arcweld/kernels.py
--- a/vq-vae-transformer-arc-welding_amd/arcweld/kernels.py
+++ b/vq-vae-transformer-arc-welding_amd/arcweld/kernels.py
@@ -253,8 +253,13 @@
     return 4.0 * R * N * H * H * (3 - 2.0 / seg)
 
 
+def convt_tail_ok():
+    import os
+    return os.environ.get("ARCWELD_CONVT_TAIL", "1") != "0"
+
+
 def res_chain_fwd(a0, x0, w1, w2, b1, b2, dh, a1, dx, a, drop=(0.0, None), seed_ptr=None, masks=None, taps=1, seg=16,
-                  stream=None):
+                  stream=None, tail=None):
     N, H = a0.shape
     R = len(w1)
     if not (1 <= R <= RES_CHAIN_MAX) or not all(len(v) == R for v in (w2, b1, b2, dh, a1, dx, a)):
@@ -271,11 +276,32 @@
     g.seed_ptr = ptr(seed_ptr)
     g.store_policy = _chain_store_policy()
     g.drop_masks = ptr(masks)
-    _maybe_timed(stream, "gemm_bf16", _chain_flops(R, N, H, taps, seg),
+    flops, extra = _chain_flops(R, N, H, taps, seg), []
+    if tail is not None:
+        wt, tb, Y, cst = tail
+        k1 = len(wt)
+        if taps != 3 or not (1 <= k1 <= nat.RES_TAIL_MAX):
+            raise nat.NativeError(f"res_chain_fwd: the tail needs taps == 3 and 1..{nat.RES_TAIL_MAX} matrices")
+        if Y.dtype != torch.bfloat16 or tuple(Y.shape) != (N, k1 * H) or not Y.is_contiguous():
+            raise nat.NativeError(f"res_chain_fwd: tail Y must be a contiguous ({N}, {k1 * H}) bfloat16 tensor")
+        if tb.dtype != torch.float32 or tb.numel() != H or not tb.is_contiguous():
+            raise nat.NativeError("res_chain_fwd: tail bias must be (H,) float32")
+        if cst is not None and (cst.dtype != torch.float64 or cst.numel() < 2 * H or not cst.is_contiguous()):
+            raise nat.NativeError("res_chain_fwd: tail colstats must be (2 H,) float64")
+        for w in wt:
+            if w.dtype != torch.bfloat16 or w.numel() != H * H or not w.is_contiguous():
+                raise nat.NativeError("res_chain_fwd: tail matrices must be packed (H, H) bfloat16 copies")
+        g.tail_k1 = k1
+        for j in range(k1):
+            g.tail_w[j] = ptr(wt[j])
+        g.tail_bias, g.tail_y, g.tail_colstats = ptr(tb), ptr(Y), ptr(cst)
+        flops += 2.0 * N * k1 * H * H
+        extra = [Y, tb] + list(wt)
+    _maybe_timed(stream, "gemm_bf16", flops,
                  lambda sp: call("aw_res_chain_fwd", ctypes.byref(g), sp),
                  lambda: (f"res_chain_fwd_kernel<{int(taps)}>",
                           _nbytes([a0, x0, masks] + list(w1) + list(w2) + list(b1) + list(b2) + list(dh) + list(a1) +
-                                  list(dx)[:-1] + list(a))))
+                                  list(dx)[:-1] + list(a) + extra)))
 
 
 def res_chain_bwd(gx, gxo, w1t, w2t, dh, x0, dx, gh, gxo_out, drop_p=0.0, masks=None, taps=1, seg=16, stream=None):
@@ -301,20 +327,26 @@
                                   list(gxo_out))))
 
 
-def res_pack_weights(src, fwd=None, bwd=None, taps=1, stream=None):
+def res_pack_weights(src, fwd=None, bwd=None, taps=1, stream=None, job_taps=None):
     n = len(src)
     fwd = fwd if fwd is not None else [None] * n
     bwd = bwd if bwd is not None else [None] * n
-    if len(fwd) != n or len(bwd) != n:
+    jt = [int(taps)] * n if job_taps is None else [int(v) for v in job_taps]
+    if len(fwd) != n or len(bwd) != n or len(jt) != n:
         raise nat.NativeError("res_pack_weights: list lengths differ")
-    for t in list(src) + [t for t in fwd + bwd if t is not None]:
-        if t.dtype != torch.bfloat16 or t.numel() != 512 * 512 * taps or not t.is_contiguous():
-            raise nat.NativeError(f"res_pack_weights: need contiguous 512 x {512 * taps} bfloat16 tensors")
+    for i in range(n):
+        for t in (src[i], fwd[i], bwd[i]):
+            if t is not None and (t.dtype != torch.bfloat16 or t.numel() != 512 * 512 * jt[i] or not t.is_contiguous()):
+                raise nat.NativeError(f"res_pack_weights: need contiguous 512 x {512 * jt[i]} bfloat16 tensors")
     for c0 in range(0, n, nat.RES_PACK_MAX):
         sl = slice(c0, c0 + nat.RES_PACK_MAX)
         m = len(src[sl])
         arr = lambda ts: (ctypes.c_void_p * m)(*[ptr(t) for t in ts])
-        call("aw_res_pack_weights", arr(src[sl]), arr(fwd[sl]), arr(bwd[sl]), m, int(taps), stream_ptr(stream))
+        if job_taps is None:
+            call("aw_res_pack_weights", arr(src[sl]), arr(fwd[sl]), arr(bwd[sl]), m, int(taps), stream_ptr(stream))
+        else:
+            call("aw_res_pack_weights_mixed", arr(src[sl]), arr(fwd[sl]), arr(bwd[sl]), (ctypes.c_int * m)(*jt[sl]), m,
+                 int(taps), stream_ptr(stream))
 
 
 def vq_forward(z2d, E, zq, idx, counts, sqerr, stream=None, zq_copy=None, count_groups=1):
diff --git a/vq-vae-transformer-arc-welding_amd/arcweld/resstack.py b/vq-vae-transformer-arc-welding_amd/arcweld/resstack.py
--- a/vq-vae-transformer-arc-welding_amd/arcweld/resstack.py
+++ b/vq-vae-transformer-arc-welding_amd/arcweld/resstack.py
@@ -132,7 +132,7 @@
     return gx, gxo
 
 
-def _chain_fwd(sv, weights, biases, RT, save):
+def _chain_fwd(sv, weights, biases, RT, save, tail=None):
     geo = sv.geo
     R, H, taps, T = len(biases), geo.H, geo.taps, sv.T
     x0, a0 = sv.xs[0], sv.a0s[0]
@@ -144,14 +144,23 @@
     sv.a0s += [e(T) for _ in range(R)]
     wsrc = [w for r in range(R) for w in weights[r]]
     pk = [torch.empty(H, geo.Kd, device=dev, dtype=T) for _ in wsrc]
-    K.res_pack_weights(wsrc, pk, None, taps=taps)
+    ktail = None
+    if tail is not None:
+        Wt, tb, Y, cst = tail
+        k1 = Wt.shape[0] // H
+        tsrc = [Wt[j * H:(j + 1) * H] for j in range(k1)]
+        tpk = [torch.empty(H, H, device=dev, dtype=T) for _ in tsrc]
+        K.res_pack_weights(wsrc + tsrc, pk + tpk, None, taps=taps, job_taps=[taps] * len(wsrc) + [1] * k1)
+        ktail = (tpk, tb, Y, cst)
+    else:
+        K.res_pack_weights(wsrc, pk, None, taps=taps)
     if save:
         sv.pk_bwd = wsrc
         if sv.p_drop > 0 and R > 1:
             sv.masks = K.res_dropout_masks_empty(N, R, dev)
     K.res_chain_fwd(a0, x0, pk[0::2], pk[1::2], [b1 for b1, _ in biases], [b2 for _, b2 in biases], sv.hs, sv.a1s,
                     sv.xs[1:], sv.a0s[1:], drop=(sv.p_drop, sv.seeds), seed_ptr=sv.ctr, masks=sv.masks, taps=taps,
-                    seg=geo.S)
+                    seg=geo.S, tail=ktail)
 
 
 def _chain_bwd(sv, gx, gxo, grads):
@@ -174,15 +183,17 @@
 
 
 def forward(geo, x0, a0, weights, biases, bns=None, *, T, RT, p_drop=0.0, seeds=None, ctr=None, training=False,
-            chain=False, last_operand_only=True, in_place=False, save=True):
+            chain=False, last_operand_only=True, in_place=False, save=True, tail=None):
     R, H, Kd = len(biases), geo.H, geo.Kd
     N, dev = a0.shape[0], a0.device
     seeds = [0] * R if seeds is None else seeds
     route = "bn" if bns is not None else "chain" if chain else "conv"
     sv = Saved(geo, route, T, p_drop, seeds, ctr, training, x0, a0)
     e = lambda dt: torch.empty(N, H, device=dev, dtype=dt)
+    if tail is not None and (route != "chain" or geo.taps != 3):
+        raise ValueError("resstack.forward: the ConvT tail runs only inside the decoder chain")
     if route == "chain":
-        _chain_fwd(sv, weights, biases, RT, save)
+        _chain_fwd(sv, weights, biases, RT, save, tail)
         return sv.xs[R], sv.a0s[R], sv
     x, a, h, a1 = x0, a0, None, None
     for r in range(R):
diff --git a/vq-vae-transformer-arc-welding_amd/arcweld/vqvae.py b/vq-vae-transformer-arc-welding_amd/arcweld/vqvae.py
--- a/vq-vae-transformer-arc-welding_amd/arcweld/vqvae.py
+++ b/vq-vae-transformer-arc-welding_amd/arcweld/vqvae.py
@@ -181,17 +181,20 @@
 
     y0, ya0 = e(N, H, dt=RT), e(N, H, dt=T)
     K.gemm(zq_T, Wd0, N, H, D, bias=pr["dec0"].bias, C=y0, C2=ya0, c2_mode=1)
-    _, yR_T, sv.dec = resstack.forward(resstack.Geometry(3, H, S), y0, ya0, dec_w, _biases(pr["dec"]), pr["dec_bn"],
-                                       seeds=[_mix(seed, 200 + r) for r in range(R)],
-                                       chain=K.res_chain_ok(H, R, T, RT, 3, S, "DEC"), **stack)
-    if R == 0:
-        yR_T = _operand(y0, T)
-
-    bn = pr["bn"]
     bf_y = T != F32 and K.head_bf16_ok(H) and os.environ.get("ARCWELD_HEAD_BF16", "1") == "1"
     Y = e(N, k1 * H, dt=T if bf_y else F32)
     colstats = acc["colstats"] if training else None
-    K.gemm(yR_T, Wt1, N, k1 * H, H, bias=pr["t1"].bias, bias_mod=H, C=Y, colstats=colstats, stats_mod=H)
+    dec_chain = K.res_chain_ok(H, R, T, RT, 3, S, "DEC") and pr["dec_bn"] is None
+    convt_tail = dec_chain and bf_y and k1 <= nat.RES_TAIL_MAX and K.convt_tail_ok()
+    _, yR_T, sv.dec = resstack.forward(resstack.Geometry(3, H, S), y0, ya0, dec_w, _biases(pr["dec"]), pr["dec_bn"],
+                                       seeds=[_mix(seed, 200 + r) for r in range(R)], chain=dec_chain,
+                                       tail=(Wt1, pr["t1"].bias, Y, colstats) if convt_tail else None, **stack)
+    if R == 0:
+        yR_T = _operand(y0, T)
+
+    bn = pr["bn"]
+    if not convt_tail:
+        K.gemm(yR_T, Wt1, N, k1 * H, H, bias=pr["t1"].bias, bias_mod=H, C=Y, colstats=colstats, stats_mod=H)
     stats = e(4 * H)
     K.bn_finalize(colstats, N * k1, H, bn.weight, bn.bias, bn.running_mean, bn.running_var,
                   bn.num_batches_tracked if training else None, bn.eps,
diff --git a/vq-vae-transformer-arc-welding_amd/csrc/gemm_core.h b/vq-vae-transformer-arc-welding_amd/csrc/gemm_core.h
--- a/vq-vae-transformer-arc-welding_amd/csrc/gemm_core.h
+++ b/vq-vae-transformer-arc-welding_amd/csrc/gemm_core.h
@@ -1,4 +1,5 @@
 #pragma once
+#include <type_traits>
 #include "common.h"
 
 #pragma clang diagnostic ignored "-Winline-asm"
@@ -639,7 +640,9 @@
   const int c4 = (tid & 31) * 4, r0 = tid >> 5;
   const int col = n0 + c4;
   const bool vec = GEN ? (P.vec && col + 4 <= N) : (col < N);
-  float bias[4], csum[4] = {0.f, 0.f, 0.f, 0.f}, csq[4] = {0.f, 0.f, 0.f, 0.f};
+  using stat_t = std::conditional_t<GEN, float, double>;
+  float bias[4];
+  stat_t csum[4] = {0, 0, 0, 0}, csq[4] = {0, 0, 0, 0};
 #pragma unroll
   for (int e = 0; e < 4; ++e) {
     const int c = col + e;
@@ -722,8 +725,9 @@
           else if (c2m == 3) y = x * ds2[e];
           w[e] = y;
           if (f_stats && col + e < N) {
-            csum[e] += x;
-            csq[e] += x * x;
+            const stat_t xs = (stat_t)x;
+            csum[e] += xs;
+            csq[e] += xs * xs;
           }
         }
         if (FASTGELU && c2m == 1 && !f_tanh) aw_gelu4(v, w);
@@ -767,7 +771,7 @@
   AW_STAMP(4);
   if (f_stats) {
     __syncthreads();
-    float* red = Cs;
+    stat_t* red = reinterpret_cast<stat_t*>(Cs);
 #pragma unroll
     for (int e = 0; e < 4; ++e) {
       red[(r0 * 2 + 0) * 128 + c4 + e] = csum[e];
@@ -775,7 +779,7 @@
     }
     __syncthreads();
     if (tid < 128 && n0 + tid < N) {
-      float a = 0.f, b = 0.f;
+      stat_t a = 0, b = 0;
 #pragma unroll
       for (int g = 0; g < NR; ++g) {
         a += red[(g * 2 + 0) * 128 + tid];
diff --git a/vq-vae-transformer-arc-welding_amd/csrc/reschain.hip b/vq-vae-transformer-arc-welding_amd/csrc/reschain.hip
--- a/vq-vae-transformer-arc-welding_amd/csrc/reschain.hip
+++ b/vq-vae-transformer-arc-welding_amd/csrc/reschain.hip
@@ -23,12 +23,14 @@
   static constexpr int FLAGS = SCR + 8 * EC_SCR;
   static constexpr int BIAS = FLAGS + 64;
   static constexpr int LDS = BIAS + 8 * 256;
+  static constexpr int TBIAS = LDS;
+  static constexpr int LDS_TAIL = TBIAS + 8 * 256;
   static constexpr uint32_t WBYTES = (uint32_t)EC_H * EC_H * 2 * TAPS;
   static constexpr int WWAVE = 4 * KS * 1024;
   static constexpr uint64_t KEYS = TAPS == 1 ? 0xfe76dc54ba329810ull : 0xf53ac739685ace10ull;
   __device__ static int key(int u) { return u < 0 ? 15 : u > 15 ? 0 : (int)((KEYS >> (4 * u)) & 15); }
 };
-static_assert(EcGeo<3>::LDS <= 160 * 1024, "decoder chain LDS");
+static_assert(EcGeo<3>::LDS_TAIL <= 160 * 1024, "decoder chain LDS");
 
 typedef __amdgpu_buffer_rsrc_t rsrc_t;
 __device__ __forceinline__ rsrc_t ec_rsrc(const void* p, uint32_t nbytes) {
@@ -146,6 +148,44 @@
   for (int e = 0; e < 4; ++e) ds[e] = (b >> e) & 1u ? k : 0.f;
 }
 
+template <class G, int KS, bool MAYSKIP, typename Tail, typename Step>
+__device__ __forceinline__ void ec_conv_g(f32x4 (&acc)[4][4], uint4 (&wf)[2][4], char* smem,
+                                          const int (&rb)[G::KS / 16], int io, rsrc_t rc, rsrc_t rn, bool has_next,
+                                          int wl, int wln, int nks, int w, int target, Tail tail, Step step) {
+  constexpr int T = G::KS / 16, T0 = KS == G::KS ? 0 : T / 2;
+  static_assert(KS == G::KS || KS == 16, "all taps or the centre tap");
+#pragma unroll
+  for (int i = 0; i < 4; ++i)
+#pragma unroll
+    for (int j = 0; j < 4; ++j) acc[i][j] = f32x4{0.f, 0.f, 0.f, 0.f};
+  int rbi[T];
+#pragma unroll
+  for (int t = 0; t < T; ++t) rbi[t] = rb[t] + io;
+#pragma unroll
+  for (int s = 0; s < KS; ++s) {
+    const int t = T0 + (s >> 4), kk = s & 15;
+    if (s < 16 && (kk & 1) == 0 && (kk >> 1) != w && (!MAYSKIP || target >= 0)) ec_wait<G>(smem, kk >> 1, target);
+    uint4 bf[4];
+#pragma unroll
+    for (int j = 0; j < 4; ++j) bf[j] = ec_lds_r16(smem, (rbi[t] ^ (64 * (kk & 3))) + (kk >> 2) * 256 + j * G::JS);
+#pragma unroll
+    for (int i = 0; i < 4; ++i)
+#pragma unroll
+      for (int j = 0; j < 4; ++j)
+        acc[i][j] = __builtin_amdgcn_mfma_f32_16x16x32_bf16(__builtin_bit_cast(bf16x8, wf[s & 1][i]),
+                                                            __builtin_bit_cast(bf16x8, bf[j]), acc[i][j], 0, 0, 0);
+    if (s + 2 < KS) {
+#pragma unroll
+      for (int i = 0; i < 4; ++i) wf[s & 1][i] = ec_wload(rc, wl, (i * KS + s + 2) * 1024);
+    } else if (has_next) {
+#pragma unroll
+      for (int i = 0; i < 4; ++i) wf[s & 1][i] = ec_wload(rn, wln, (i * nks + s + 2 - KS) * 1024);
+    }
+    step(s);
+    if (s == KS - 1) tail();
+    __builtin_amdgcn_sched_barrier(0);
+  }
+}
 template <class G, typename Tail, typename Step>
 __device__ __forceinline__ void ec_conv(f32x4 (&acc)[4][4], uint4 (&wf)[2][4], char* smem, const int (&rb)[G::KS / 16],
                                         int io, rsrc_t rc, rsrc_t rn, bool has_next, int wl, int w, int target,
@@ -244,14 +284,22 @@
   for (int q = 0; q < 2; ++q) ec_store16<WT>(r, S.gs, 8192 * (2 * j + q), ec_lds_r16(smem, S.srq(q)));
 }
 
+template <class G, bool WT>
+__device__ __forceinline__ void ec_store_scratch_at(const char* smem, int j, const EcStore<G>& S, rsrc_t r,
+                                                    uint32_t gs, int st8, int co) {
+#pragma unroll
+  for (int q = 0; q < 2; ++q) ec_store16<WT>(r, gs, st8 * (2 * j + q) + co, ec_lds_r16(smem, S.srq(q)));
+}
+
 template <class G> __device__ __forceinline__ void ec_init(char* smem, int tid) {
   if (tid < 8) *ec_flag<G>(smem, tid) = 0;
 }
 
-template <int TAPS, bool DROP, bool WT>
+template <int TAPS, bool DROP, bool WT, bool TAIL>
 __global__ __launch_bounds__(EC_NTH) void res_chain_fwd_kernel(aw_res_chain_fwd_args P) {
   using G = EcGeo<TAPS>;
-  __shared__ __attribute__((aligned(16))) char smem[G::LDS];
+  static_assert(!TAIL || TAPS == 3, "the ConvT tail follows the decoder chain");
+  __shared__ __attribute__((aligned(16))) char smem[TAIL ? G::LDS_TAIL : G::LDS];
   const int tid = threadIdx.x;
   const int64_t row0 = (int64_t)blockIdx.x * EC_ROWS;
   const EcLane<G, 1> L(tid);
@@ -259,6 +307,7 @@
   const int R = P.R, NC = 2 * R;
 
   ec_init<G>(smem, tid);
+  if constexpr (TAIL) *reinterpret_cast<float*>(smem + G::TBIAS + 4 * tid) = P.tail_bias[tid];
   ec_load_image<G>(smem, P.a0, row0, nbytes, tid);
   u32x2 xr[4][4];
   ec_load_frags(xr, ec_rsrc(P.x0, nbytes), ec_frag_off(row0, L.li, L.w, L.g));
@@ -281,8 +330,10 @@
     const int r = c >> 1;
     const bool second = (c & 1) != 0;
     const rsrc_t rc = ec_rsrc(second ? P.w2[r] : P.w1[r], G::WBYTES);
-    const bool has_next = c + 1 < NC;
-    const rsrc_t rn = ec_rsrc(has_next ? (second ? P.w1[r + 1] : P.w2[r]) : nullptr, G::WBYTES);
+    const bool tail_next = TAIL && c + 1 == NC;
+    const bool has_next = TAIL || c + 1 < NC;
+    const rsrc_t rn = ec_rsrc(tail_next ? P.tail_w[0] : has_next ? (second ? P.w1[r + 1] : P.w2[r]) : nullptr,
+                              tail_next ? EcGeo<1>::WBYTES : G::WBYTES);
     const int io = (c & 1) * G::IMG, no = ((c + 1) & 1) * G::IMG;
     f32x4 acc[4][4];
     const float bias_l = (second ? P.b2[r] : P.b1[r])[64 * L.w + L.lane];
@@ -295,7 +346,12 @@
       *reinterpret_cast<float*>(smem + G::BIAS + 256 * L.w + 4 * L.lane) = bias_l;
       if (DROP && second) ec_store8(rmask, (uint32_t)(ec_keep_idx(r, tid) * 8), u32x2{kb[0], kb[1]});
     };
-    ec_conv<G>(acc, wf, smem, L.rb, io, rc, rn, has_next, L.wl, L.w, c, park, hash);
+    if constexpr (TAIL)
+      ec_conv_g<G, G::KS, false>(acc, wf, smem, L.rb, io, rc, rn, true, L.wl,
+                                 tail_next ? L.w * EcGeo<1>::WWAVE + L.lane * 16 : L.wl, tail_next ? 16 : G::KS, L.w, c,
+                                 park, hash);
+    else
+      ec_conv<G>(acc, wf, smem, L.rb, io, rc, rn, has_next, L.wl, L.w, c, park, hash);
     const u32x2 keep = {kb[0], kb[1]};
     int nwb[4];
 #pragma unroll
@@ -365,8 +421,82 @@
             ec_lds_w8(smem, nwb[i] + G::JS * j, xr[i][j]);
             ec_frag_fence(4 * i + j);
           }
+        if constexpr (TAIL) ec_publish<G>(smem, L.w, L.lane, c + 1);
       }
       ec_store_slice<G, WT>(smem, no, S, ec_rsrc(P.a[r], nbytes));
+    }
+  }
+
+  if constexpr (TAIL) {
+    using G1 = EcGeo<1>;
+    const int k1 = P.tail_k1;
+    const int wl1 = L.w * G1::WWAVE + L.lane * 16;
+    const EcStore<G> S(tid, row0);
+    const rsrc_t ry = ec_rsrc(P.tail_y, (uint32_t)(P.N * k1 * EC_ROWB));
+    const uint32_t ygs = (uint32_t)(((row0 + (L.lane >> 3)) * k1 * EC_H + 64 * L.w + 8 * (L.lane & 7)) * 2);
+    const int st8 = 8 * k1 * EC_ROWB;
+    const int64_t left = P.N - row0;
+    const int ngrp = left >= EC_ROWS ? 4 : (int)(left >> 4);
+    double cs[4][4], cq[4][4];
+#pragma unroll
+    for (int i = 0; i < 4; ++i)
+#pragma unroll
+      for (int e = 0; e < 4; ++e) cs[i][e] = cq[i][e] = 0.;
+    for (int jt = 0; jt < k1; ++jt) {
+      const bool more = jt + 1 < k1;
+      const rsrc_t rc = ec_rsrc(P.tail_w[jt], G1::WBYTES);
+      const rsrc_t rn = ec_rsrc(more ? P.tail_w[jt + 1] : nullptr, G1::WBYTES);
+      f32x4 acc[4][4];
+      ec_conv_g<G, 16, true>(acc, wf, smem, L.rb, 0, rc, rn, more, wl1, wl1, 16, L.w, jt == 0 ? NC : -1, [] {},
+                             [](int) {});
+#pragma unroll
+      for (int j = 0; j < 4; ++j) {
+        if (j < ngrp) {
+#pragma unroll
+          for (int i = 0; i < 4; ++i) {
+            const float4 b4 = *reinterpret_cast<const float4*>(smem + G::TBIAS + 256 * L.w + 64 * i + 16 * L.g);
+            const float bv[4] = {b4.x, b4.y, b4.z, b4.w};
+            float v[4];
+#pragma unroll
+            for (int e = 0; e < 4; ++e) {
+              v[e] = acc[i][j][e] + bv[e];
+              const double vd = (double)v[e];
+              cs[i][e] += vd;
+              cq[i][e] += vd * vd;
+            }
+            ec_lds_w8(smem, S.sw[i], ec_pack(v));
+            ec_frag_fence(4 * j + i);
+          }
+          ec_store_scratch_at<G, WT>(smem, j, S, ry, ygs, st8, jt * EC_ROWB);
+        }
+        __builtin_amdgcn_sched_barrier(0);
+      }
+    }
+    if (P.tail_colstats) {
+#pragma unroll
+      for (int i = 0; i < 4; ++i)
+#pragma unroll
+        for (int e = 0; e < 4; ++e)
+#pragma unroll
+          for (int m = 1; m < 16; m <<= 1) {
+            cs[i][e] += __shfl_xor(cs[i][e], m);
+            cq[i][e] += __shfl_xor(cq[i][e], m);
+          }
+      double* red = reinterpret_cast<double*>(smem + G::SCR + L.w * EC_SCR);
+      asm volatile("s_waitcnt lgkmcnt(0)" ::: "memory");
+      if (L.li == 0) {
+#pragma unroll
+        for (int i = 0; i < 4; ++i)
+#pragma unroll
+          for (int e = 0; e < 4; ++e) {
+            red[16 * i + 4 * L.g + e] = cs[i][e];
+            red[64 + 16 * i + 4 * L.g + e] = cq[i][e];
+          }
+      }
+      asm volatile("s_waitcnt lgkmcnt(0)" ::: "memory");
+      const double a = red[L.lane], b = red[64 + L.lane];
+      atomicAdd(P.tail_colstats + 64 * L.w + L.lane, a);
+      atomicAdd(P.tail_colstats + EC_H + 64 * L.w + L.lane, b);
     }
   }
 }
@@ -499,9 +629,30 @@
   const void* src[AW_RES_PACK_MAX];
   void* fwd[AW_RES_PACK_MAX];
   void* bwd[AW_RES_PACK_MAX];
+  uint32_t one_tap;
 };
 
 constexpr int PK_PITCH1 = 128 + 16;
+template <int TAPS>
+__device__ __forceinline__ void res_pack_fwd(const char* __restrict__ W, uint4* __restrict__ out, char* t, int x,
+                                             int nx, int tid) {
+  constexpr int RB = EC_ROWB * TAPS, PITCH0 = RB + 16, KB = 16 * TAPS;
+  for (int mb = x; mb < EC_H / 16; mb += nx) {
+#pragma unroll
+    for (int q = 0; q < 4 * TAPS; ++q) {
+      const int c = tid + 256 * q, row = c / (64 * TAPS), kc = c % (64 * TAPS);
+      *reinterpret_cast<uint4*>(t + row * PITCH0 + kc * 16) =
+          *reinterpret_cast<const uint4*>(W + (size_t)(16 * mb + row) * RB + kc * 16);
+    }
+    __syncthreads();
+#pragma unroll
+    for (int q = 0; q < 4 * TAPS; ++q) {
+      const int o = tid + 256 * q, st = o >> 6, l = o & 63;
+      out[(size_t)mb * 64 * KB + o] = *reinterpret_cast<const uint4*>(t + (l & 15) * PITCH0 + (4 * st + (l >> 4)) * 16);
+    }
+    __syncthreads();
+  }
+}
 template <int TAPS>
 __global__ __launch_bounds__(256) void res_pack_kernel(PackJobs J) {
   constexpr int RB = EC_ROWB * TAPS, PITCH0 = RB + 16, KB = 16 * TAPS;
@@ -509,27 +660,15 @@
   __shared__ __attribute__((aligned(16))) char t[SZ];
   const int x = blockIdx.x, job = blockIdx.y, tid = threadIdx.x;
   const char* __restrict__ W = reinterpret_cast<const char*>(J.src[job]);
+  const bool one_tap = TAPS > 1 && ((J.one_tap >> job) & 1u);
   if (blockIdx.z == 0) {
     uint4* __restrict__ out = reinterpret_cast<uint4*>(J.fwd[job]);
     if (!out) return;
-    for (int mb = x; mb < EC_H / 16; mb += gridDim.x) {
-#pragma unroll
-      for (int q = 0; q < 4 * TAPS; ++q) {
-        const int c = tid + 256 * q, row = c / (64 * TAPS), kc = c % (64 * TAPS);
-        *reinterpret_cast<uint4*>(t + row * PITCH0 + kc * 16) =
-            *reinterpret_cast<const uint4*>(W + (size_t)(16 * mb + row) * RB + kc * 16);
-      }
-      __syncthreads();
-#pragma unroll
-      for (int q = 0; q < 4 * TAPS; ++q) {
-        const int o = tid + 256 * q, st = o >> 6, l = o & 63;
-        out[(size_t)mb * 64 * KB + o] = *reinterpret_cast<const uint4*>(t + (l & 15) * PITCH0 + (4 * st + (l >> 4)) * 16);
-      }
-      __syncthreads();
-    }
+    if (one_tap) res_pack_fwd<1>(W, out, t, x, (int)gridDim.x, tid);
+    else res_pack_fwd<TAPS>(W, out, t, x, (int)gridDim.x, tid);
   } else {
     uint4* __restrict__ out = reinterpret_cast<uint4*>(J.bwd[job]);
-    if (!out) return;
+    if (!out || one_tap) return;
     const int tap = x >> 3, b = x & 7;
 #pragma unroll
     for (int q = 0; q < 16; ++q) {
@@ -569,12 +708,12 @@
 
 bool aligned16(const void* p) { return ((uintptr_t)p & 15) == 0; }
 
-template <int TAPS>
+template <int TAPS, bool TAIL>
 void launch_fwd(const aw_res_chain_fwd_args* a, bool drop, bool wt, dim3 grid, hipStream_t s) {
-  if (drop && wt) hipLaunchKernelGGL((res_chain_fwd_kernel<TAPS, true, true>), grid, dim3(EC_NTH), 0, s, *a);
-  else if (drop) hipLaunchKernelGGL((res_chain_fwd_kernel<TAPS, true, false>), grid, dim3(EC_NTH), 0, s, *a);
-  else if (wt) hipLaunchKernelGGL((res_chain_fwd_kernel<TAPS, false, true>), grid, dim3(EC_NTH), 0, s, *a);
-  else hipLaunchKernelGGL((res_chain_fwd_kernel<TAPS, false, false>), grid, dim3(EC_NTH), 0, s, *a);
+  if (drop && wt) hipLaunchKernelGGL((res_chain_fwd_kernel<TAPS, true, true, TAIL>), grid, dim3(EC_NTH), 0, s, *a);
+  else if (drop) hipLaunchKernelGGL((res_chain_fwd_kernel<TAPS, true, false, TAIL>), grid, dim3(EC_NTH), 0, s, *a);
+  else if (wt) hipLaunchKernelGGL((res_chain_fwd_kernel<TAPS, false, true, TAIL>), grid, dim3(EC_NTH), 0, s, *a);
+  else hipLaunchKernelGGL((res_chain_fwd_kernel<TAPS, false, false, TAIL>), grid, dim3(EC_NTH), 0, s, *a);
 }
 template <int TAPS>
 void launch_bwd(const aw_res_chain_bwd_args* a, bool drop, bool wt, dim3 grid, hipStream_t s) {
@@ -607,11 +746,23 @@
                "aw_res_chain_fwd: block %d saved outputs unaligned", r);
   }
   AW_REQUIRE(aligned16(a->drop_masks), "aw_res_chain_fwd: drop_masks unaligned");
+  if (a->tail_k1 == 0) {
+    AW_REQUIRE(!a->tail_bias && !a->tail_y && !a->tail_colstats, "aw_res_chain_fwd: tail fields without tail_k1");
+  } else {
+    AW_REQUIRE(a->taps == 3 && a->tail_k1 >= 1 && a->tail_k1 <= AW_RES_TAIL_MAX,
+               "aw_res_chain_fwd: the tail needs taps == 3 and tail_k1 in 1..%d (got %d)", AW_RES_TAIL_MAX, a->tail_k1);
+    AW_REQUIRE((a->N + EC_ROWS) * a->tail_k1 * EC_ROWB < (1ll << 31), "aw_res_chain_fwd: N * tail_k1 out of range");
+    AW_REQUIRE(a->tail_y && aligned16(a->tail_y) && a->tail_bias && ((uintptr_t)a->tail_colstats & 7) == 0,
+               "aw_res_chain_fwd: tail_y / tail_bias missing or unaligned");
+    for (int j = 0; j < a->tail_k1; ++j)
+      AW_REQUIRE(a->tail_w[j] && aligned16(a->tail_w[j]), "aw_res_chain_fwd: tail matrix %d missing or unaligned", j);
+  }
   hipStream_t s = (hipStream_t)stream;
   const dim3 grid((unsigned)((a->N + EC_ROWS - 1) / EC_ROWS));
   const bool drop = a->drop_p > 0.f, wt = a->store_policy == AW_STORE_WT;
-  if (a->taps == 3) launch_fwd<3>(a, drop, wt, grid, s);
-  else launch_fwd<1>(a, drop, wt, grid, s);
+  if (a->tail_k1) launch_fwd<3, true>(a, drop, wt, grid, s);
+  else if (a->taps == 3) launch_fwd<3, false>(a, drop, wt, grid, s);
+  else launch_fwd<1, false>(a, drop, wt, grid, s);
   return aw::check_launch("aw_res_chain_fwd");
 }
 
@@ -639,6 +790,11 @@
 
 extern "C" int aw_res_pack_weights(const void* const* src, void* const* fwd, void* const* bwd, int n, int taps,
                                    void* stream) {
+  return aw_res_pack_weights_mixed(src, fwd, bwd, nullptr, n, taps, stream);
+}
+
+extern "C" int aw_res_pack_weights_mixed(const void* const* src, void* const* fwd, void* const* bwd,
+                                         const int* job_taps, int n, int taps, void* stream) {
   AW_REQUIRE(src && fwd && bwd && n >= 0 && n <= AW_RES_PACK_MAX && (taps == 1 || taps == 3),
              "aw_res_pack_weights: bad args (n must be 0..%d, taps 1 or 3)", AW_RES_PACK_MAX);
   if (n == 0) return AW_OK;
@@ -649,6 +805,11 @@
     J.src[i] = src[i];
     J.fwd[i] = fwd[i];
     J.bwd[i] = bwd[i];
+    if (job_taps && job_taps[i] != taps) {
+      AW_REQUIRE(job_taps[i] == 1 && fwd[i] && !bwd[i], "aw_res_pack_weights: job %d: a job of %d taps in a launch of "
+                 "%d (only 1-tap forward copies may differ)", i, job_taps[i], taps);
+      J.one_tap |= 1u << i;
+    }
   }
   const dim3 grid(8 * taps, n, 2);
   if (taps == 3) hipLaunchKernelGGL(res_pack_kernel<3>, grid, dim3(256), 0, (hipStream_t)stream, J);
```

After: 438,600 windows/s (median of 6 runs). +1.4%, better.
